# MrOlm/inStrain

Hardware: AMD Instinct MI355X
Metric: Gbp profiled/s (higher is better)
Workload: dtype u32

## Files before the change

### include/instrain_amd.h

```cpp
#ifndef INSTRAIN_AMD_H
#define INSTRAIN_AMD_H

#include <stdint.h>

#ifdef __cplusplus
extern "C" {
#endif

#define ISX_OK 0
#define ISX_ERR_ARG (-1)
#define ISX_ERR_HIP (-2)
#define ISX_ERR_CAPACITY (-3)
#define ISX_ERR_MM_RANGE (-4)
#define ISX_ERR_IO (-5)
#define ISX_ERR_STATE (-6)

#define ISX_ABI_VERSION 5


typedef struct isx_ctx isx_ctx;
typedef struct isx_batch isx_batch;
typedef struct isx_bam isx_bam;
struct isx_bam_params_s;
struct isx_bam_info_s;
// ... 250 lines not shown
    int32_t want_counts;
    int32_t ring_kib;
    int32_t stage_async;
    int32_t lean_output;
    int64_t max_segs;
} isx_pipe_params;

typedef struct {
    uint32_t gpos;
    float clon_rarefied;
} isx_rare;

typedef struct {
    uint32_t gpos;
    uint32_t coverage;
} isx_sat;

typedef struct {
    int64_t ticket;
    int64_t n_pos, n_obs;
    isx_sizes sizes;
    const uint16_t *coverage16;
    const float *clon;
    const isx_rare *rare;
    int64_t n_rare, n_saturated;
    const uint32_t *counts;
    const float *clon_rarefied;
    const isx_snv *snv;
    isx_batch *batch;
    float encode_ms;
    float h2d_ms, kernel_ms, d2h_ms;
    float collect_wait_ms;
    int32_t record_bytes;
    int32_t encode_passes;
    int64_t h2d_bytes, d2h_bytes;
    const isx_ld *ld;
    const uint8_t *coverage8;
    const isx_rare *clon_sparse;
    int64_t n_clon;
    const isx_sat *saturated;
    const uint8_t *coverage4;
    const uint16_t *cov_rows;
    const uint32_t *cov_row_window;
    int64_t n_cov_rows;
    int32_t cov_window, pad_cov;
    const void *lev_mask;
    const void *lev_cov;
    const uint32_t *lev_win_off;
    const isx_rare *lev_clon, *lev_rare;
    const isx_sat *lev_sat;
    int64_t n_lev, n_lev_clon, n_lev_rare, n_lev_sat;
    int32_t lev_mask_bytes, lev_cov_bytes, lev_window, n_lev_windows, lev_min_cov, pad_lev;
    uint64_t rows_checksum;
} isx_pipe_result;

int isx_levels_expand(const isx_pipe_result *r, int32_t host_threads, uint32_t *gpos, uint32_t *mm_cov, float *clon, float *clon_rarefied);

int isx_pipe_create(isx_ctx *ctx, const isx_params *params, const isx_pipe_params *pp, isx_pipe **out);
void isx_pipe_destroy(isx_pipe *p);
int isx_pipe_submit(isx_pipe *p, int64_t n_pos, const uint8_t *ref, int32_t n_splits, const int64_t *split_bounds,
                    int64_t n_obs, const isx_obs *obs, const uint32_t *pair, int64_t *ticket);
int isx_pipe_submit_bam(isx_pipe *p, isx_bam *bam, const struct isx_bam_params_s *bp, const int32_t *refs, int32_t n_refs,
                        const uint8_t *ref, int32_t n_splits, const int64_t *split_bounds, struct isx_bam_info_s *info,
                        int64_t *ticket);
int isx_pipe_collect(isx_pipe *p, int64_t ticket, isx_pipe_result *out);
int isx_pipe_release(isx_pipe *p, int64_t ticket);
int isx_pipe_fetch_entries(isx_pipe *p, int64_t ticket, isx_entry *out);
int isx_pipe_fetch_entries_shrunk(isx_pipe *p, int64_t ticket, uint32_t *gpos, uint32_t *mm_cov, float *clon, float *clon_rarefied);


#define ISX_SEG_BASES 150
#define ISX_SEG_WORDS 15
#define ISX_SEG_SKIP_WORD 0x24924924u
#define ISX_DREC_WORDS 8
#define ISX_DREC_EXC 6
#define ISX_DREC_EXC_FULL 3
#define ISX_DREC_DUAL 0x80000000u
#define ISX_DREC_NO_EXC 0x3FFFFFFFu

typedef struct {
    int64_t n_seg;
    const uint32_t *gpos;
    const uint8_t *len;
    const uint8_t *mm;
    const uint32_t *pair;
    const uint32_t *bases;
} isx_segs;

int isx_batch_create_reads(isx_ctx *ctx, const isx_params *params, int64_t n_pos, const uint8_t *ref, int32_t n_splits,
                           const int64_t *split_bounds, const isx_segs *segs, isx_batch **out);
int isx_pipe_submit_reads(isx_pipe *p, int64_t n_pos, const uint8_t *ref, int32_t n_splits, const int64_t *split_bounds,
                          const isx_segs *segs, int64_t *ticket);

typedef struct isx_wire isx_wire;
int isx_pipe_stage_reads(isx_pipe *p, int64_t n_pos, const uint8_t *ref, int32_t n_splits, const int64_t *split_bounds,
                         const isx_segs *segs, isx_wire **out);
int isx_pipe_submit_wire(isx_pipe *p, const isx_wire *wire, int64_t *ticket);
int64_t isx_wire_bytes(const isx_wire *wire);
void isx_wire_free(isx_wire *wire);
int isx_wire_keep_reference(isx_pipe *p, isx_wire *wire);

#define ISX_PLANE_WORDS 8
typedef struct {
    int64_t n_seg;
    const uint32_t *gpos;
    const uint8_t *len;
    const uint32_t *pair;
    const uint64_t *planes;
    const uint8_t *mm;
} isx_read_planes;

typedef struct {
    const uint8_t *plane2;
    const uint8_t *nplane;
    uint64_t key;
} isx_ref_planes;

int isx_pack_ref_planes(const uint8_t *ref, int64_t n_pos, int32_t host_threads, uint8_t *plane2, uint8_t *nplane, int32_t *has_n);
int isx_planes_from_segs(const isx_segs *segs, int32_t host_threads, uint64_t *planes);
int isx_pack_read_planes(int64_t n_reads, const int64_t *ref_start, const int64_t *clip_lo, const int64_t *clip_hi,
                         const uint32_t *cigar, const int64_t *cigar_off, const char *seq, const uint8_t *qual, const int64_t *seq_off,
                         const uint32_t *pair, int32_t min_base_quality, int64_t cap_seg, uint32_t *seg_gpos,
                         uint8_t *seg_len, uint32_t *seg_pair, uint64_t *seg_planes, int64_t *n_seg);
int isx_pipe_submit_planes(isx_pipe *p, int64_t n_pos, const isx_ref_planes *ref, int32_t n_splits, const int64_t *split_bounds,
                           const isx_read_planes *reads, int64_t *ticket);
int isx_pipe_stage_planes(isx_pipe *p, int64_t n_pos, const isx_ref_planes *ref, int32_t n_splits, const int64_t *split_bounds,
                          const isx_read_planes *reads, isx_wire **out);
int isx_pipe_set_reference_budget(isx_pipe *p, int64_t mib);
int isx_host_register(const void *ptr, int64_t bytes);
int isx_host_unregister(const void *ptr);
int isx_encode_planes(const isx_read_planes *reads, const isx_ref_planes *ref, int64_t n_pos, int32_t host_threads, int32_t slack_groups,
                      int64_t cap_rec, int64_t ring_records, uint32_t *rec, uint32_t *gbase, int64_t *n_rec, int64_t *need_slack);
int isx_encode_planes_mm(const isx_read_planes *reads, const isx_ref_planes *ref, int64_t n_pos, int32_t n_mm_bins, int32_t host_threads, int32_t slack_groups,
                         int64_t cap_rec, int64_t ring_records, uint32_t *rec, uint32_t *gbase, int64_t *n_rec, int64_t *need_slack);

int isx_count_read_segs(int64_t n_reads, const uint32_t *cigar, const int64_t *cigar_off, const int64_t *ref_start,
                        const int64_t *clip_lo, const int64_t *clip_hi, int64_t *n_seg);
int isx_pack_reads(int64_t n_reads, const int64_t *ref_start, const int64_t *clip_lo, const int64_t *clip_hi,
                   const uint32_t *cigar, const int64_t *cigar_off, const char *seq, const uint8_t *qual, const int64_t *seq_off,
                   const uint8_t *mm, const uint32_t *pair, int32_t min_base_quality, int64_t cap_seg, uint32_t *seg_gpos,
                   uint8_t *seg_len, uint8_t *seg_mm, uint32_t *seg_pair, uint32_t *seg_bases, int64_t *n_seg);

int isx_encode_segs(const isx_segs *segs, int64_t n_pos, int32_t n_mm_bins, int32_t host_threads, int64_t cap_rec, uint32_t *rec,
                    uint32_t *gbase, uint32_t *pair_out, int64_t *n_rec);
int64_t isx_seg_records_needed(const uint32_t *gpos, int64_t n_seg, int32_t host_threads);
int isx_encode_segs_ring(const isx_segs *segs, int64_t n_pos, int32_t n_mm_bins, int32_t host_threads, int64_t cap_rec, int64_t ring_records,
                         uint32_t *rec, uint32_t *gbase, uint32_t *pair_out, int64_t *n_rec);

int isx_encode_delta(const isx_segs *segs, const uint8_t *ref, int64_t n_pos, int32_t n_mm_bins, int32_t host_threads, int32_t slack_groups,
                     int64_t cap_rec, int64_t ring_records, uint32_t *rec, uint32_t *gbase, uint32_t *pair_out, int64_t *n_rec, int64_t *need_slack);
int64_t isx_delta_records_needed(const uint32_t *gpos, int64_t n_seg, int32_t host_threads, int32_t slack_groups);

int isx_encode_obs(const isx_obs *obs, const uint32_t *pair, int64_t n_obs, int64_t n_pos, int32_t record_bytes,
                   int32_t host_threads, double slack, int64_t cap_rec, void *rec, uint32_t *gbase, uint32_t *pair_out,
                   int64_t *n_rec, int32_t *passes);
int isx_encode_obs_ring(const isx_obs *obs, const uint32_t *pair, int64_t n_obs, int64_t n_pos, int32_t record_bytes,
                        int32_t host_threads, double slack, int64_t cap_rec, int64_t ring_records, void *rec,
                        uint32_t *gbase, uint32_t *pair_out, int64_t *n_rec, int32_t *passes);

typedef struct {
    int64_t in_off;
    int32_t in_len;
    int32_t out_len;
    int64_t out_off;
} isx_bgzf_block;
int isx_bgzf_index(const uint8_t *image, int64_t n_bytes, int64_t cap_blocks, isx_bgzf_block *blocks, int64_t *n_blocks, int64_t *out_bytes);
int isx_bgzf_inflate_device(isx_ctx *ctx, const uint8_t *image, int64_t n_bytes, const isx_bgzf_block *blocks, int64_t n_blocks,
                            uint8_t *out, int64_t out_bytes, float *kernel_ms);
int isx_bgzf_inflate_host(const uint8_t *image, int64_t n_bytes, const isx_bgzf_block *blocks, int64_t n_blocks, uint8_t *out, int64_t out_bytes);
int isx_bgzf_inflate_fast(const uint8_t *image, int64_t n_bytes, const isx_bgzf_block *blocks, int64_t n_blocks, uint8_t *out, int64_t out_bytes);

typedef struct isx_bam_params_s {
    double min_read_ani;
    int32_t min_mapq;
    double max_insert_relative;
    int32_t min_insert;
    int32_t min_base_quality;
    int32_t skip_mm;
    int32_t window_length;
    int32_t pairing_filter;
} isx_bam_params;

typedef struct isx_bam_info_s {
    int32_t n_refs;
    int32_t n_splits;
    int64_t n_reads;
    int64_t n_pos;
// ... 48 lines not shown
```

### instrain_amd/_lib.py

```python
import ctypes as C
import os

import numpy as np

_HERE = os.path.dirname(os.path.abspath(__file__))
LIB_PATH = os.path.join(_HERE, "libinstrain_amd.so")
if os.environ.get("ISX_LIB"):
    LIB_PATH = os.path.abspath(os.environ["ISX_LIB"])

BGZF_BLOCK_DT = np.dtype([("in_off", np.int64), ("in_len", np.int32), ("out_len", np.int32), ("out_off", np.int64)])
OBS_DT = np.dtype([("gpos", "<u4"), ("mm", "<u2"), ("base", "u1"), ("flags", "u1")])
ENTRY_DT = np.dtype([("gpos", "<u4"), ("mm", "<u2"), ("flags", "<u2"), ("cnt", "<u4", (4,)), ("clon", "<f4"),
                     ("clon_rarefied", "<f4")])
SNV_DT = np.dtype([("gpos", "<u4"), ("mm", "<u2"), ("con_base", "u1"), ("var_base", "u1"),
                   ("allele_count", "u1"), ("cls", "u1"), ("cryptic", "u1"), ("ref_base", "u1"),
                   ("cnt", "<u4", (4,))])
LD_DT = np.dtype([("gpos_a", "<u4"), ("gpos_b", "<u4"), ("mm", "<u2"), ("allele_A", "u1"), ("allele_a", "u1"),
                  ("allele_B", "u1"), ("allele_b", "u1"), ("pad", "<u2"), ("total", "<u4"), ("countAB", "<u4"),
                  ("countAb", "<u4"), ("countaB", "<u4"), ("countab", "<u4"), ("pad2", "<u4"),
                  ("r2", "<f8"), ("d_prime", "<f8"), ("r2_normalized", "<f8"), ("d_prime_normalized", "<f8")])
AO_DT = np.dtype([("pair", "<u4"), ("gpos", "<u4"), ("order", "<u4"), ("mm", "<u2"), ("base", "u1"), ("pad", "u1")])
assert AO_DT.itemsize == 16
assert OBS_DT.itemsize == 8 and ENTRY_DT.itemsize == 32 and SNV_DT.itemsize == 28 and LD_DT.itemsize == 72

# ... 19 lines not shown


class Segs(C.Structure):
    _fields_ = [("n_seg", C.c_int64), ("gpos", C.c_void_p), ("len", C.c_void_p), ("mm", C.c_void_p), ("pair", C.c_void_p),
                ("bases", C.c_void_p)]


PLANE_WORDS = 8
LAYOUT_MM_ENTRIES = 16
LAYOUT_MM_DELTA_RECORDS = 32
ABI_VERSION = 5


class ReadPlanes(C.Structure):
    _fields_ = [("n_seg", C.c_int64), ("gpos", C.c_void_p), ("len", C.c_void_p), ("pair", C.c_void_p), ("planes", C.c_void_p), ("mm", C.c_void_p)]


class RefPlanes(C.Structure):
    _fields_ = [("plane2", C.c_void_p), ("nplane", C.c_void_p), ("key", C.c_uint64)]


RARE_DT = np.dtype([("gpos", "<u4"), ("clon_rarefied", "<f4")])
CLON_DT = np.dtype([("gpos", "<u4"), ("clon", "<f4")])
SAT_DT = np.dtype([("gpos", "<u4"), ("coverage", "<u4")])


class Sizes(C.Structure):
    _fields_ = [(n, C.c_int64) for n in ("n_entries", "n_snv", "n_sites", "n_allele_obs", "n_increments",
                                         "n_edges", "n_ld")]


class Timings(C.Structure):
    _fields_ = [(n, C.c_float) for n in ("pileup_ms", "sites_ms", "allele_ms", "group_ms", "incr_ms", "ld_ms",
                                         "total_ms")] + \
               [(n, C.c_int32) for n in ("pileup_blocks", "pileup_threads", "pileup_lds_bytes", "pileup_window")] + \
               [("mfma_ms", C.c_float), ("dense_tiles", C.c_int32), ("dense_macs", C.c_int64), ("dense_bytes", C.c_int64),
                ("record_bytes", C.c_int32), ("pad", C.c_int32)]


class PipeResult(C.Structure):
    _fields_ = [("ticket", C.c_int64), ("n_pos", C.c_int64), ("n_obs", C.c_int64), ("sizes", Sizes),
                ("coverage16", C.c_void_p), ("clon", C.c_void_p), ("rare", C.c_void_p), ("n_rare", C.c_int64),
                ("n_saturated", C.c_int64), ("counts", C.c_void_p), ("clon_rarefied", C.c_void_p), ("snv", C.c_void_p),
                ("batch", C.c_void_p),
                ("encode_ms", C.c_float), ("h2d_ms", C.c_float), ("kernel_ms", C.c_float), ("d2h_ms", C.c_float),
                ("collect_wait_ms", C.c_float), ("record_bytes", C.c_int32), ("encode_passes", C.c_int32),
                ("h2d_bytes", C.c_int64), ("d2h_bytes", C.c_int64), ("ld", C.c_void_p),
                ("coverage8", C.c_void_p), ("clon_sparse", C.c_void_p), ("n_clon", C.c_int64), ("saturated", C.c_void_p),
                ("coverage4", C.c_void_p), ("cov_rows", C.c_void_p), ("cov_row_window", C.c_void_p), ("n_cov_rows", C.c_int64),
                ("cov_window", C.c_int32), ("pad_cov", C.c_int32),
                ("lev_mask", C.c_void_p), ("lev_cov", C.c_void_p), ("lev_win_off", C.c_void_p), ("lev_clon", C.c_void_p), ("lev_rare", C.c_void_p),
                ("lev_sat", C.c_void_p), ("n_lev", C.c_int64), ("n_lev_clon", C.c_int64), ("n_lev_rare", C.c_int64), ("n_lev_sat", C.c_int64),
                ("lev_mask_bytes", C.c_int32), ("lev_cov_bytes", C.c_int32), ("lev_window", C.c_int32), ("n_lev_windows", C.c_int32),
                ("lev_min_cov", C.c_int32), ("pad_lev", C.c_int32), ("rows_checksum", C.c_uint64)]


class BamParams(C.Structure):
    _fields_ = [("min_read_ani", C.c_double), ("min_mapq", C.c_int32), ("max_insert_relative", C.c_double),
                ("min_insert", C.c_int32), ("min_base_quality", C.c_int32), ("skip_mm", C.c_int32),
                ("window_length", C.c_int32), ("pairing_filter", C.c_int32)]


PAIRING_FILTERS = {"paired_only": 0, "non_discordant": 1, "all_reads": 2}


class BamInfo(C.Structure):
    _fields_ = [("n_refs", C.c_int32), ("n_splits", C.c_int32), ("n_reads", C.c_int64), ("n_pos", C.c_int64),
                ("n_obs", C.c_int64), ("n_pairs", C.c_int64), ("unfiltered_pairs", C.c_int64),
                ("filtered_pairs", C.c_int64), ("filtered_bases", C.c_int64), ("median_insert", C.c_double),
                ("max_mm", C.c_int32), ("pad", C.c_int32), ("unfiltered_reads", C.c_int64),
                ("unfiltered_singletons", C.c_int64), ("filtered_singletons", C.c_int64), ("n_segs", C.c_int64)]


SCAFFOLD_LEVEL_DT = np.dtype([("nonzero", "<i8"), ("sum_cov", "<u8"), ("sumsq_cov", "<u8"), ("median_cov", "<f8"),
                              ("counted", "<i8"), ("sum_clon", "<f8"), ("median_clon", "<f8"),
                              ("counted_rarefied", "<i8"), ("sum_clon_rarefied", "<f8"),
                              ("median_clon_rarefied", "<f8"), ("mm", "<i4"), ("present", "<i4")])
assert SCAFFOLD_LEVEL_DT.itemsize == 88
GENOME_LEVEL_DT = np.dtype([("n", "<i8"), ("sum_cov", "<u8"), ("sumsq_cov", "<u8"), ("median_cov", "<f8"), ("mm", "<i4"), ("pad", "<i4")])
assert GENOME_LEVEL_DT.itemsize == 40
GENOME_COV_DT = np.dtype([("n", "<i8"), ("sum_cov", "<u8"), ("sumsq_cov", "<u8"), ("max_cov", "<u4"), ("pad", "<u4")])
SNV_LEVEL_DT = np.dtype([(n, "<u4") for n in ("divergent", "sns", "snv", "con", "pop")])
LD_LEVEL_DT = np.dtype([("n", "<i8"), ("n_r2", "<i8"), ("n_dprime", "<i8"), ("sum_distance", "<i8"), ("sum_r2", "<f8"), ("sum_dprime", "<f8")])
assert GENOME_COV_DT.itemsize == 32 and SNV_LEVEL_DT.itemsize == 20 and LD_LEVEL_DT.itemsize == 48


COMPARE_LEVEL_DT = np.dtype([("both", "<i8"), ("either", "<i8"), ("mm", "<i4"), ("present_a", "<i4"),
                             ("present_b", "<i4"), ("pad", "<i4"), ("consensus_snps", "<i8"), ("population_snps", "<i8")])
assert COMPARE_LEVEL_DT.itemsize == 48
COMPARE_SNP_DT = np.dtype([("gpos", "<u4"), ("mm", "<u2"), ("consensus_snp", "u1"), ("population_snp", "u1"),
                           ("has_a", "u1"), ("has_b", "u1"), ("con_a", "u1"), ("ref_a", "u1"), ("var_a", "u1"),
                           ("con_b", "u1"), ("ref_b", "u1"), ("var_b", "u1"), ("cnt_a", "<u4", (4,)), ("cnt_b", "<u4", (4,))])
assert COMPARE_SNP_DT.itemsize == 48


GENE_DT = np.dtype([("start", "<i8"), ("end", "<i8"), ("seq_off", "<i8"), ("strand", "<i4"), ("pad", "<i4")])
GENE_COV_DT = np.dtype([("sum_cov", "<u8"), ("nonzero", "<u4"), ("counted", "<u4"), ("sum_clon", "<f8")])
GENE_SNV_COUNT_DT = np.dtype([(n, "<u4") for n in ("divergent", "sns", "sns_n", "sns_s", "snv", "snv_n", "snv_s")])
GENE_MUTATION_DT = np.dtype([("gene", "<i4"), ("k", "<i4"), ("type", "u1"), ("aa_old", "u1"), ("aa_new", "u1"), ("n_genes", "u1"),
                             ("pad", "<u4")])
assert GENE_DT.itemsize == 32 and GENE_COV_DT.itemsize == 24 and GENE_SNV_COUNT_DT.itemsize == 28 and GENE_MUTATION_DT.itemsize == 16
GENE_LEVEL_PRESENT, GENE_COV_ANY, GENE_CLON_ANY = 1, 2, 4


ERR_CAPACITY = -3


class IsxError(RuntimeError):
    def __init__(self, code, msg):
        super().__init__("libinstrain_amd error %d: %s" % (code, msg))
        self.code = code


SYMBOLS = ["isx_last_error", "isx_abi_version", "isx_ctx_create", "isx_ctx_destroy", "isx_ctx_reserve_cus", "isx_set_null_model",
           "isx_batch_create", "isx_batch_create_reads", "isx_batch_destroy", "isx_batch_run", "isx_batch_launch", "isx_batch_wait", "isx_batch_sizes", "isx_batch_timings",
           "isx_batch_fetch_entries", "isx_batch_fetch_dense", "isx_batch_fetch_snv", "isx_batch_fetch_ld", "isx_batch_fetch_allele_obs",
           "isx_batch_summarize", "isx_batch_summarize_genomes", "isx_batch_genome_coverage", "isx_snv_level_counts", "isx_ld_level_sums", "isx_compare_coverage", "isx_compare_scaffolds", "isx_compare_fetch_snps",
           "isx_genes_create", "isx_genes_destroy", "isx_genes_sites", "isx_batch_profile_genes", "isx_genes_profile_snvs",
           "isx_pipe_create", "isx_pipe_destroy", "isx_pipe_submit", "isx_pipe_submit_reads", "isx_pipe_stage_reads", "isx_pipe_submit_wire", "isx_wire_bytes", "isx_wire_free", "isx_wire_keep_reference", "isx_pipe_submit_bam", "isx_encode_segs", "isx_encode_segs_ring", "isx_seg_records_needed", "isx_encode_delta", "isx_delta_records_needed", "isx_count_read_segs", "isx_pack_reads", "isx_pipe_collect", "isx_pipe_release", "isx_pipe_fetch_entries", "isx_pipe_fetch_entries_shrunk", "isx_levels_expand", "isx_encode_obs", "isx_encode_obs_ring",
           "isx_pack_ref_planes", "isx_planes_from_segs", "isx_pack_read_planes", "isx_pipe_submit_planes", "isx_pipe_stage_planes", "isx_encode_planes", "isx_encode_planes_mm", "isx_pipe_set_reference_budget", "isx_host_register", "isx_host_unregister",
           "isx_bgzf_index", "isx_bgzf_inflate_device", "isx_bgzf_inflate_host", "isx_bgzf_inflate_fast",
           "isx_bam_open", "isx_bam_close", "isx_bam_close_wait", "isx_bam_set_threads", "isx_bam_ref", "isx_bam_set_priority_reads", "isx_bam_scan", "isx_bam_scan_part",
           "isx_bam_insert_sizes", "isx_bam_set_wanted_refs", "isx_bam_pair_keys", "isx_bam_set_cross_names", "isx_bam_filter_insert_sizes", "isx_bam_filter", "isx_bam_set_r2m", "isx_bam_r2m", "isx_bam_drop_names", "isx_bam_batch_pair_names", "isx_bam_set_mm_cap", "isx_bam_mm_levels", "isx_bam_set_mm_levels", "isx_bam_ref_counts",
           "isx_bam_expand_refs", "isx_bam_segment_refs", "isx_bam_copy_segs", "isx_bam_copy_read_planes", "isx_bam_expand_region", "isx_bam_expand", "isx_bam_copy", "isx_bam_view"]

_lib = None


def load():
    global _lib
    if _lib is not None:
        return _lib
    if not os.path.exists(LIB_PATH):
        raise IsxError(-2, "%s not built: run `python -c 'import __graft_entry__ as g; g.build()'` "
                           "(hipcc --offload-arch=gfx950)" % LIB_PATH)
    lib = C.CDLL(LIB_PATH)
    vp, i32, i64 = C.c_void_p, C.c_int32, C.c_int64
    lib.isx_last_error.restype = C.c_char_p
    lib.isx_abi_version.restype = C.c_int
    if lib.isx_abi_version() != ABI_VERSION:
        raise IsxError(-6, "%s has ABI version %d, this package binds version %d: rebuild it (python -c 'import __graft_entry__ as g; g.build()')"
                       % (LIB_PATH, lib.isx_abi_version(), ABI_VERSION))
    lib.isx_ctx_create.argtypes = [C.c_int, C.POINTER(vp)]
    lib.isx_ctx_destroy.argtypes = [vp]
    lib.isx_ctx_reserve_cus.argtypes = [vp, C.c_int]
    lib.isx_bgzf_index.argtypes = [vp, i64, i64, vp, C.POINTER(i64), C.POINTER(i64)]
    lib.isx_bgzf_inflate_device.argtypes = [vp, vp, i64, vp, i64, vp, i64, C.POINTER(C.c_float)]
    lib.isx_bgzf_inflate_host.argtypes = [vp, i64, vp, i64, vp, i64]
    lib.isx_bgzf_inflate_fast.argtypes = [vp, i64, vp, i64, vp, i64]
    lib.isx_ctx_destroy.restype = None
    lib.isx_set_null_model.argtypes = [vp, vp, i64, i32]
    lib.isx_batch_create.argtypes = [vp, C.POINTER(Params), i64, vp, i32, vp, i64, vp, vp, C.POINTER(vp)]
    lib.isx_batch_create_reads.argtypes = [vp, C.POINTER(Params), i64, vp, i32, vp, C.POINTER(Segs), C.POINTER(vp)]
    lib.isx_pipe_submit_reads.argtypes = [vp, i64, vp, i32, vp, C.POINTER(Segs), C.POINTER(i64)]
    lib.isx_pipe_stage_reads.argtypes = [vp, i64, vp, i32, vp, C.POINTER(Segs), C.POINTER(vp)]
    lib.isx_pipe_submit_wire.argtypes = [vp, vp, C.POINTER(i64)]
    lib.isx_wire_bytes.argtypes = [vp]
    lib.isx_wire_bytes.restype = i64
    lib.isx_wire_free.argtypes = [vp]
    lib.isx_wire_keep_reference.argtypes = [vp, vp]
    lib.isx_wire_free.restype = None
    lib.isx_encode_segs.argtypes = [C.POINTER(Segs), i64, i32, i32, i64, vp, vp, vp, C.POINTER(i64)]
    lib.isx_encode_segs_ring.argtypes = [C.POINTER(Segs), i64, i32, i32, i64, i64, vp, vp, vp, C.POINTER(i64)]
    lib.isx_encode_delta.argtypes = [C.POINTER(Segs), vp, i64, i32, i32, i32, i64, i64, vp, vp, vp, C.POINTER(i64), C.POINTER(i64)]
    lib.isx_delta_records_needed.argtypes = [vp, i64, i32, i32]
    lib.isx_delta_records_needed.restype = i64
    lib.isx_seg_records_needed.argtypes = [vp, i64, i32]
    lib.isx_seg_records_needed.restype = i64
    lib.isx_count_read_segs.argtypes = [i64, vp, vp, vp, vp, vp, C.POINTER(i64)]
    lib.isx_pack_reads.argtypes = [i64, vp, vp, vp, vp, vp, vp, vp, vp, vp, vp, i32, i64, vp, vp, vp, vp, vp, C.POINTER(i64)]
    lib.isx_batch_destroy.argtypes = [vp]
    lib.isx_batch_destroy.restype = None
    lib.isx_batch_run.argtypes = [vp]
# ... 18 lines not shown
    lib.isx_genes_sites.argtypes = [vp, vp, C.POINTER(C.c_float)]
    lib.isx_batch_profile_genes.argtypes = [vp, vp, i32, vp, vp, vp, vp, vp, C.POINTER(C.c_float)]
    lib.isx_genes_profile_snvs.argtypes = [vp, i32, vp, vp, vp, i64, vp, i32, vp, vp, C.POINTER(C.c_float)]
    lib.isx_pipe_create.argtypes = [vp, C.POINTER(Params), C.POINTER(PipeParams), C.POINTER(vp)]
    lib.isx_pipe_destroy.argtypes = [vp]
    lib.isx_pipe_destroy.restype = None
    lib.isx_pipe_submit.argtypes = [vp, i64, vp, i32, vp, i64, vp, vp, C.POINTER(i64)]
    lib.isx_pipe_submit_bam.argtypes = [vp, vp, C.POINTER(BamParams), vp, i32, vp, i32, vp, C.POINTER(BamInfo), C.POINTER(i64)]
    lib.isx_pipe_collect.argtypes = [vp, i64, C.POINTER(PipeResult)]
    lib.isx_pipe_release.argtypes = [vp, i64]
    lib.isx_pipe_fetch_entries.argtypes = [vp, i64, vp]
    lib.isx_pipe_fetch_entries_shrunk.argtypes = [vp, i64, vp, vp, vp, vp]
    lib.isx_levels_expand.argtypes = [C.POINTER(PipeResult), i32, vp, vp, vp, vp]
    lib.isx_encode_obs.argtypes = [vp, vp, i64, i64, i32, i32, C.c_double, i64, vp, vp, vp, C.POINTER(i64), C.POINTER(i32)]
    lib.isx_encode_obs_ring.argtypes = [vp, vp, i64, i64, i32, i32, C.c_double, i64, i64, vp, vp, vp, C.POINTER(i64), C.POINTER(i32)]
    lib.isx_bam_open.argtypes = [C.c_char_p, C.POINTER(vp)]
    lib.isx_bam_close.argtypes = [vp]
    lib.isx_bam_close.restype = None
    lib.isx_bam_close_wait.argtypes = [vp]
    lib.isx_bam_close_wait.restype = None
    lib.isx_bam_expand.argtypes = [vp, C.POINTER(BamParams), C.POINTER(BamInfo)]
    lib.isx_bam_set_threads.argtypes = [vp, i32]
    lib.isx_bam_set_priority_reads.argtypes = [vp, i64, C.c_char_p, vp]
    lib.isx_bam_scan.argtypes = [vp, C.POINTER(BamInfo)]
    lib.isx_bam_scan_part.argtypes = [vp, i32, i32, C.POINTER(BamInfo)]
    lib.isx_bam_set_wanted_refs.argtypes = [vp, vp, i32]
    lib.isx_bam_insert_sizes.argtypes = [vp, vp, i64, C.POINTER(i64)]
    lib.isx_bam_filter_insert_sizes.argtypes = [vp, vp, i64, C.POINTER(i64)]
    lib.isx_bam_pair_keys.argtypes = [vp, vp, vp, vp, vp, i64, C.POINTER(i64)]
    lib.isx_bam_set_cross_names.argtypes = [vp, i64, vp, vp, vp]
    lib.isx_bam_filter.argtypes = [vp, C.POINTER(BamParams), C.c_double, C.POINTER(BamInfo)]
    lib.isx_bam_set_r2m.argtypes = [vp, i32, i64, C.c_char_p, vp, vp]
    lib.isx_bam_drop_names.argtypes = [vp]
    lib.isx_bam_r2m.argtypes = [vp, i32, C.POINTER(i64), C.POINTER(i64), vp, vp, vp]
    lib.isx_bam_batch_pair_names.argtypes = [vp, C.POINTER(i64), C.POINTER(i64), vp, vp]
    lib.isx_bam_set_mm_cap.argtypes = [vp, i32]
    lib.isx_bam_mm_levels.argtypes = [vp, vp, i32, vp]
    lib.isx_bam_set_mm_levels.argtypes = [vp, vp, i32]
    lib.isx_bam_ref_counts.argtypes = [vp, vp, vp]
    lib.isx_bam_expand_region.argtypes = [vp, C.POINTER(BamParams), i32, i64, i64, C.POINTER(BamInfo)]
    lib.isx_bam_expand_refs.argtypes = [vp, C.POINTER(BamParams), vp, i32, C.POINTER(BamInfo)]
    lib.isx_bam_segment_refs.argtypes = [vp, C.POINTER(BamParams), vp, i32, C.POINTER(BamInfo), C.POINTER(i64)]
    lib.isx_bam_copy_segs.argtypes = [vp, vp, vp, vp, vp, vp, vp, vp]
    lib.isx_bam_copy_read_planes.argtypes = [vp, vp]
    lib.isx_pack_ref_planes.argtypes = [vp, i64, i32, vp, vp, C.POINTER(i32)]
    lib.isx_planes_from_segs.argtypes = [C.POINTER(Segs), i32, vp]
    lib.isx_pack_read_planes.argtypes = [i64, vp, vp, vp, vp, vp, vp, vp, vp, vp, i32, i64, vp, vp, vp, vp, C.POINTER(i64)]
    lib.isx_pipe_submit_planes.argtypes = [vp, i64, C.POINTER(RefPlanes), i32, vp, C.POINTER(ReadPlanes), C.POINTER(i64)]
    lib.isx_pipe_set_reference_budget.argtypes = [vp, i64]
    lib.isx_host_register.argtypes = [vp, i64]
    lib.isx_host_unregister.argtypes = [vp]
    lib.isx_pipe_stage_planes.argtypes = [vp, i64, C.POINTER(RefPlanes), i32, vp, C.POINTER(ReadPlanes), C.POINTER(vp)]
    lib.isx_encode_planes.argtypes = [C.POINTER(ReadPlanes), C.POINTER(RefPlanes), i64, i32, i32, i64, i64, vp, vp, C.POINTER(i64), C.POINTER(i64)]
    lib.isx_encode_planes_mm.argtypes = [C.POINTER(ReadPlanes), C.POINTER(RefPlanes), i64, i32, i32, i32, i64, i64, vp, vp, C.POINTER(i64), C.POINTER(i64)]
    lib.isx_bam_ref.argtypes = [vp, i32, C.POINTER(C.c_char_p), C.POINTER(i64), C.POINTER(i64)]
    lib.isx_bam_copy.argtypes = [vp, vp, vp, vp, vp]
    lib.isx_bam_view.argtypes = [vp, C.POINTER(vp), C.POINTER(vp)]
    _lib = lib
    return lib


def check(rc):
    if rc != 0:
        raise IsxError(rc, load().isx_last_error().decode(errors="replace"))
```

### instrain_amd/csrc/isx_internal.h

```cpp
#pragma once
#include <hip/hip_runtime.h>
#include <stdint.h>
#include <string>

#include "../../include/instrain_amd.h"

#define ISX_PAD32 0x0700FFFFu
#define ISX_GROUP16 512
#define ISX_GROUP 256
#define ISX_CHUNK 1024
#define ISX_DENSE_PAD 8
#define ISX_SEG_GROUP 16
#define ISX_SEG_PAD 32
#define ISX_SEG_LM 16
#define ISX_PK16_MAX_W 3264
#define ISX_PAD 2048
#define ISX_SENTINEL 0xFFFFFFFFu
#define ISX_TAIL_BYTES 65536
#define ISX_TAIL_GROUPS 256

void isx_set_error(const std::string &msg);

hipError_t isx_dev_malloc(void **p, size_t bytes);
void isx_dev_free(void *p);
// ... 140 lines not shown
    int32_t stripe;
    int32_t pad, lm;
    double min_freq;
    uint4 *counts;
    float *clon;
    float *clon_r;
    uint16_t *cov16;
    uint8_t *cov8;
    uint8_t *cov4;
    uint16_t *cov_rows;
    uint32_t *cov_row_win;
    uint32_t cap_cov_rows;
    uint2 *sat;
    uint32_t cap_sat, sat_thr;
    uint2 *clon_list;
    uint32_t cap_clon;
    uint2 *rare;
    uint32_t cap_rare;
    int32_t min_cov_r;
    uint32_t seed_lo, seed_hi;
    isx_entry *entries;
    uint32_t slab;
    uint32_t cap_ovf;
    uint64_t ovf0;
    uint32_t *win_nent;
    uint32_t *win_site_base, *win_site_cnt;
    isx_slev *slev;
    uint32_t cap_slev;
    isx_snv *snv;
    uint32_t cap_snv;
    isx_site *sites;
    uint32_t cap_sites;
    isx_ao *ao;
    uint32_t cap_ao;
    int32_t enable_linkage;
    uint32_t *win_rec;
    uint32_t *cursors;
    uint32_t *flags;
    uint32_t base[CUR_N];
    uint32_t *host_state;
    const uint32_t *pub_cursors;
    uint32_t *pub_host_state;
    uint32_t pub_epoch;
    void *lev_mask;
    void *lev_cov;
    uint32_t *lev_win_off;
    uint32_t cap_lev;
    int32_t lev_mask_bytes, lev_cov_bytes;
};

void launch_pileup(const PileupArgs &a, int block, size_t lds, int grid, int packed, hipStream_t s, hipEvent_t ev_start,
                   hipEvent_t ev_stop);
void launch_publish_state(const PileupArgs &a, uint32_t epoch, hipStream_t s);
void launch_win_order(const uint32_t *win_rec, uint32_t *win_out, int n_win, int W, const isx_snv *snv_raw, isx_snv *snv, const isx_site *sites_raw,
                      isx_site *sites, const uint2 *clon_raw, uint2 *clon, const uint2 *rare_raw, uint2 *rare, uint32_t *scan_state, uint32_t epoch, hipStream_t s);
void launch_extract_gpos(const uint2 *rec, const uint32_t *rec32, const uint32_t *gbase, uint32_t *gpos, uint16_t *gpos16,
                         const uint32_t *base16, uint32_t base16_records, uint64_t n_rec, hipStream_t s);
size_t pileup_lds_bytes(int W, int M, int qcap, int rqcap, int linkage, int packed, int block, int segs, int *stage_off, int *dlt_off = nullptr);

struct LinkageBuffers;
```

### instrain_amd/csrc/isx_pipe.hip

```cpp
#include <atomic>
#include <algorithm>
#include <chrono>
#include <cmath>
#include <condition_variable>
#include <cstring>
#include <deque>
#include <mutex>
#include <memory>
#include <string>
#include <thread>
#include <vector>

#include "bam_front.h"
#include "isx_batch.h"
#include "obs_encode.h"
#include "seg_encode.h"
#include "isx_summary.h"
#include <unordered_map>

namespace {

constexpr size_t ALIGN = 256;
inline size_t up(size_t v, size_t a = ALIGN) { return (v + a - 1) / a * a; }

// ... 10 lines not shown
    return ISX_OK;
}

void host_block_free(void *p, bool pinned)
{
    if (!p) return;
    if (pinned) isx_pin_free(p); else free(p);
}

static const bool pipe_timing = getenv("ISX_PIPE_TIMING") != nullptr;
#define H2D(p, s) ((s).h2d ? (s).h2d : (p)->s_h2d)
struct Slot {
    isx_batch *b = nullptr;
    hipStream_t h2d = nullptr;
    uint8_t *h_in = nullptr, *d_in = nullptr;
    size_t in_bytes = 0;
    size_t off_bounds = 0, off_win = 0, off_ref = 0, off_gbase = 0, off_ridx = 0, off_rec = 0;
    size_t off_pairs = 0;
    isxenc::PairRun *h_runs = nullptr;
    bool runs_pinned = true;
    uint2 *d_runs = nullptr;
    size_t cap_runs = 0;
    hipEvent_t ev_ring[2] = {nullptr, nullptr};
    bool ring_busy[2] = {false, false};
    uint8_t *h_out = nullptr;
    uint8_t *h_small = nullptr;
    size_t small_bytes = 0;
    bool out_pinned = true;
    size_t out_bytes = 0, o_counts = 0, o_clon = 0, o_clonr = 0, o_snv = 0, o_cov16 = 0, o_rare = 0;
    bool rare_dense = false;
    bool cov8 = false, clon_sparse = false;
    bool cov4 = false;
    size_t cov_rows_off = 0;
    int cov_window = 0;
    std::vector<uint32_t> cov_row_win;
    std::vector<isx_sat> sat_rows;
    bool sat_complete = true;
    void *sort_temp = nullptr;
    size_t sort_temp_bytes = 0;
    std::vector<float> clonr_big;
    std::vector<isx_rare> rare_big;
    std::vector<uint32_t> cmin, cmax, dir_pmax, dir_smin;
    std::vector<uint8_t> cany;
    std::vector<uint2> win;
    size_t o_lmask = 0, o_lwin = 0, o_lcov = 0, o_lclon = 0, o_lrare = 0;
    size_t lcov_room = 0, lclon_room = 0, lrare_room = 0;
    std::vector<uint8_t> lcov_big;
    std::vector<isx_rare> lclon_big, lrare_big;
    std::vector<isx_snv> snv_big;
    std::vector<isx_ld> ld_rows;
    uint64_t rows_checksum = 0;
    hipEvent_t ev_h2d0 = nullptr, ev_h2d1 = nullptr, ev_pass = nullptr, ev_d2h0 = nullptr, ev_d2h1 = nullptr;
    hipEvent_t ev_h2da = nullptr, ev_h2db = nullptr;
    bool h2d_split = false;
    int64_t ticket = -1;
    BamBatch *dead_batch = nullptr;
    bool ref_has_n = false;
    int state = 0;
    int rc = 0;
    std::string err;
    float finish_wait_ms = 0.f;
    float encode_ms = 0.f;
    int encode_passes = 0;
    int64_t h2d_bytes = 0, d2h_bytes = 0;
    uint16_t *d_gpos16 = nullptr;
};

static uint64_t bytes_checksum(const void *p, size_t bytes, uint64_t seed)
{
    const uint8_t *b = static_cast<const uint8_t *>(p);
    uint64_t a[4] = {seed ^ 0x9E3779B97F4A7C15ull, seed + 0xC2B2AE3D27D4EB4Full, seed ^ 0x165667B19E3779F9ull, seed + 0x27D4EB2F165667C5ull};
    const size_t n8 = bytes / 8;
    size_t i = 0;
    for (; i + 4 <= n8; i += 4) {
        uint64_t w[4];
        memcpy(w, b + 8 * i, 32);
        for (int k = 0; k < 4; k++) a[k] = a[k] * 0x100000001B3ull + w[k];
    }
    uint64_t h = (uint64_t)bytes;
    for (; i < n8; i++) { uint64_t w; memcpy(&w, b + 8 * i, 8); h = h * 0x100000001B3ull + w; }
    for (size_t j = n8 * 8; j < bytes; j++) h = h * 0x100000001B3ull + b[j];
    for (int k = 0; k < 4; k++) { h ^= a[k]; h *= 0xFF51AFD7ED558CCDull; h ^= h >> 33; }
    return h;
}

static inline size_t ref2_bytes(int64_t n_pos) { return (((size_t)n_pos + 3) / 4 + 15) & ~(size_t)15; }
static inline size_t refn_bytes(int64_t n_pos) { return (((size_t)n_pos + 7) / 8 + 15) & ~(size_t)15; }

static bool copy_ref_planes(isxenc::HostPool &pool, const isx_ref_planes *rp, int64_t n_pos, uint8_t *plane2, uint8_t *nplane)
{
    const size_t b2 = ((size_t)n_pos + 3) / 4, bn = ((size_t)n_pos + 7) / 8;
    const size_t piece = (size_t)1 << 20;
    const int t2 = (int)((b2 + piece - 1) / piece), tn = rp->nplane ? (int)((bn + piece - 1) / piece) : 0;
    std::atomic<int> any{0};
    pool.run(t2 + tn, [&](int t) {
        if (t < t2) { const size_t a = (size_t)t * piece; memcpy(plane2 + a, rp->plane2 + a, std::min(piece, b2 - a)); return; }
        const size_t a = (size_t)(t - t2) * piece, n = std::min(piece, bn - a);
        const uint8_t *src = rp->nplane + a;
        uint8_t acc = 0;
        for (size_t i = 0; i < n; i++) acc |= src[i];
        memcpy(nplane + a, src, n);
        if (acc) any.store(1, std::memory_order_relaxed);
    });
    return any.load() != 0;
}

static bool plane_any(isxenc::HostPool &pool, const uint8_t *pl, size_t bytes)
{
    const size_t piece = (size_t)1 << 20;
    const int nt = (int)((bytes + piece - 1) / piece);
    std::atomic<int> any{0};
    pool.run(nt, [&](int t) {
        const size_t a = (size_t)t * piece, n = std::min(piece, bytes - a);
        uint64_t acc = 0;
        size_t i = 0;
        for (; i + 8 <= n; i += 8) { uint64_t v; memcpy(&v, pl + a + i, 8); acc |= v; }
        for (; i < n; i++) acc |= pl[a + i];
        if (acc) any.store(1, std::memory_order_relaxed);
// ... 10 lines not shown
    for (size_t k = 0; k < n_s; k++) {
        uint64_t w;
        memcpy(&w, plane2 + 8 * (k * step), 8);
        h = (h ^ w) * 0x100000001B3ull;
        h ^= h >> 29;
    }
    return h;
}

int cgroup_cpus()
{
    if (FILE *f = fopen("/sys/fs/cgroup/cpu.max", "r")) {
        char q[64] = {0};
        long period = 0;
        const int n = fscanf(f, "%63s %ld", q, &period);
        fclose(f);
        if (n == 2 && period > 0 && strcmp(q, "max") != 0) return (int)std::max<long>(1, atol(q) / period);
    }
    return 0;
}

int gpu_numa_node(int device)
{
    char bus[64] = {0};
    if (hipDeviceGetPCIBusId(bus, sizeof bus, device) != hipSuccess) return -1;
    std::string id(bus);
    std::transform(id.begin(), id.end(), id.begin(), [](unsigned char ch) { return (char)std::tolower(ch); });
    int node = -1;
    if (FILE *f = fopen(("/sys/bus/pci/devices/" + id + "/numa_node").c_str(), "r")) {
        if (fscanf(f, "%d", &node) != 1) node = -1;
        fclose(f);
    }
    return node;
}

}

struct isx_pipe {
    isx_ctx *ctx = nullptr;
    isx_params prm{};
    isx_pipe_params pp{};
    std::unique_ptr<isxenc::HostPool> pool;
    std::vector<Slot> slots;
    hipStream_t s_h2d = nullptr, s_d2h = nullptr;
    hipStream_t s_h2d2 = nullptr;
    hipStream_t s_fin = nullptr;
    hipStream_t s_fin2 = nullptr;
    int64_t next_ticket = 0;
    int64_t cap_rec = 0;
    int64_t ring_half = 0;
    int rb = 2;
    bool segs = false;
    bool drec = false;
    int64_t dslack = 1;
    uint32_t G = ISX_GROUP16;
    size_t snv_prefix = 0;
    size_t rare_prefix = 0, cap_rare = 0;
    double slack = 0.0;
    std::thread finisher;
    std::thread finisher2;
    std::vector<std::thread> more_finishers;
    std::vector<hipStream_t> extra_fin;
    std::mutex bounce_mu;
    std::mutex mu;
    std::condition_variable cv_work, cv_done;
    std::deque<int64_t> work;
    bool stop = false;
    std::mutex launch_mu;
    uint8_t *bounce[2] = {nullptr, nullptr};
    hipEvent_t bounce_ev[2] = {nullptr, nullptr};
    size_t bounce_bytes = 0;
    std::unique_ptr<isxenc::HostPool> fin_pool;
    struct StageJob {
        int64_t ticket, n_pos;
        const uint8_t *ref;
        std::vector<int64_t> bounds;
        isx_segs segs;
        bool planes = false;
        isx_read_planes reads{};
        isx_ref_planes rp{};
    };
    struct RefEntry { uint8_t *d = nullptr; size_t bytes = 0; int64_t n_pos = 0; bool has_n = false; hipEvent_t ready = nullptr; uint64_t sum = 0; };
    std::unordered_map<uint64_t, RefEntry> ref_cache;
    size_t ref_cache_bytes = 0;
    std::atomic<size_t> ref_cache_budget{(size_t)4096 << 20};
    std::thread stager;
    std::deque<StageJob> stage_q;
    std::condition_variable cv_stage;
    int64_t next_promise = 0;
    bool stage_stop = false;
};

static int bounce_d2h(isx_pipe *p, void *hdst, const void *dsrc, size_t bytes, hipStream_t st)
{
    if (!bytes) return ISX_OK;
    std::lock_guard<std::mutex> bounce_lk(p->bounce_mu);
    const size_t piece = p->bounce_bytes;
    const size_t n_pieces = (bytes + piece - 1) / piece;
    auto issue = [&](size_t k) -> hipError_t {
        const size_t off = k * piece, len = std::min(piece, bytes - off);
        hipError_t e = isx_copy_to_host(p->bounce[k & 1], static_cast<const uint8_t *>(dsrc) + off, len, st);
        return e == hipSuccess ? hipEventRecord(p->bounce_ev[k & 1], st) : e;
    };
    HIP_TRY(issue(0));
    for (size_t k = 0; k < n_pieces; k++) {
        if (k + 1 < n_pieces) HIP_TRY(issue(k + 1));
        HIP_TRY(isx_wait_event(p->bounce_ev[k & 1]));
        const size_t off = k * piece, len = std::min(piece, bytes - off);
        const size_t sub = (size_t)1 << 20;
        const uint8_t *src = p->bounce[k & 1];
        uint8_t *dst = static_cast<uint8_t *>(hdst) + off;
        p->fin_pool->run((int)((len + sub - 1) / sub), [&](int t) {
            const size_t a = (size_t)t * sub;
            memcpy(dst + a, src + a, std::min(sub, len - a));
        });
    }
    return ISX_OK;
}

static void pipe_free(isx_pipe *p)
{
    if (!p) return;
    if (p->stager.joinable()) {
        { std::lock_guard<std::mutex> lk(p->mu); p->stage_stop = true; }
        p->cv_stage.notify_all();
        p->stager.join();
    }
    if (p->finisher.joinable()) {
        { std::lock_guard<std::mutex> lk(p->mu); p->stop = true; }
        p->cv_work.notify_all();
        p->finisher.join();
        if (p->finisher2.joinable()) p->finisher2.join();
        for (auto &t : p->more_finishers) if (t.joinable()) t.join();
    }
    (void)hipSetDevice(p->ctx->device);
    if (p->s_h2d) (void)isx_wait_stream(p->s_h2d);
    if (p->s_h2d2) (void)isx_wait_stream(p->s_h2d2);
    if (p->s_d2h) (void)isx_wait_stream(p->s_d2h);
    if (p->s_fin) (void)isx_wait_stream(p->s_fin);
    if (p->s_fin2) (void)isx_wait_stream(p->s_fin2);
    for (hipStream_t st : p->extra_fin) (void)isx_wait_stream(st);
    for (int i = 0; i < 2; i++) if (p->ctx->pstream[i]) (void)isx_wait_stream(p->ctx->pstream[i]);
    const double t_f0 = now_ms();
    double t_batch = 0, t_dev = 0, t_pin = 0;
    for (Slot &s : p->slots) {
        double t_x = now_ms();
        if (s.b) {
            isx_batch *b = s.b;
            b->d_seg = nullptr; b->d_drec = nullptr;
            b->d_rec = nullptr; b->d_rec32 = nullptr; b->d_rec16 = nullptr; b->d_gbase = nullptr; b->d_pair = nullptr;
            b->d_pair_runs = nullptr; b->d_run_index = nullptr;
            b->d_gpos = nullptr; b->d_gpos16 = nullptr; b->d_cbase = nullptr; b->d_ref = nullptr; b->d_win = nullptr;
            b->d_bounds = nullptr;
            isx_batch_destroy(b);
        }
        t_batch += now_ms() - t_x; t_x = now_ms();
        if (s.sort_temp) isx_dev_free(s.sort_temp);
        if (s.d_gpos16) isx_dev_free(s.d_gpos16);
        if (s.d_in) isx_dev_free(s.d_in);
        if (s.d_runs) isx_dev_free(s.d_runs);
        t_dev += now_ms() - t_x; t_x = now_ms();
        if (s.h_in) isx_pin_free(s.h_in);
        host_block_free(s.h_runs, s.runs_pinned);
        for (hipEvent_t e : s.ev_ring) if (e) (void)hipEventDestroy(e);
        host_block_free(s.h_out, s.out_pinned);
        if (s.h_small) isx_pin_free(s.h_small);
        t_pin += now_ms() - t_x;
        for (hipEvent_t e : {s.ev_h2d0, s.ev_h2d1, s.ev_pass, s.ev_d2h0, s.ev_d2h1, s.ev_h2da, s.ev_h2db}) if (e) (void)hipEventDestroy(e);
    }
    if (pipe_timing)
        fprintf(stderr, "[isx_pipe_destroy] device tables %.1f ms, device arena %.1f ms, pinned staging %.1f ms, total %.1f ms\n", t_batch, t_dev, t_pin, now_ms() - t_f0);
    for (auto &kv : p->ref_cache) { if (kv.second.d) isx_dev_free(kv.second.d); if (kv.second.ready) (void)hipEventDestroy(kv.second.ready); }
    for (int i = 0; i < 2; i++) {
        if (p->bounce[i]) isx_pin_free(p->bounce[i]);
        if (p->bounce_ev[i]) (void)hipEventDestroy(p->bounce_ev[i]);
    }
    if (p->s_h2d) (void)hipStreamDestroy(p->s_h2d);
    if (p->s_h2d2) (void)hipStreamDestroy(p->s_h2d2);
    if (p->s_d2h) (void)hipStreamDestroy(p->s_d2h);
    if (p->s_fin) (void)hipStreamDestroy(p->s_fin);
    if (p->s_fin2) (void)hipStreamDestroy(p->s_fin2);
    for (hipStream_t st : p->extra_fin) (void)hipStreamDestroy(st);
    delete p;
}

static int slot_batch_create(isx_pipe *p, Slot &s, int index)
{
    isx_ctx *c = p->ctx;
    const isx_params *prm = &p->prm;
    const double t_s0 = now_ms();
    isx_batch *b = new isx_batch();
    s.b = b;
    b->ctx = c; b->prm = *prm; b->M = prm->n_mm_bins;
    b->ps = getenv("ISX_ONE_PASS_QUEUE") ? 0 : (index & 1);
    b->cap_pos = p->pp.max_pos; b->cap_obs = p->pp.max_obs; b->arena = true; b->ref_packed = 2;
    b->n_pos = p->pp.max_pos; b->n_obs = p->pp.max_obs;
    b->segs = p->segs; b->drec = p->drec;
    b->lean = p->pp.lean_output != 0 && !p->pp.want_counts;
    b->lev_sparse = b->M > 1 && b->M <= 32 && p->segs && !p->pp.want_counts && !(prm->layout & ISX_LAYOUT_MM_ENTRIES);
    b->spin_us = (p->pp.host_threads > 0 && p->pp.host_threads < 8) ? 200 : 2000;
    const bool dense = b->M == 1;
    batch_pick_block(b);
    const int64_t cap_pos = p->pp.max_pos;
    for (auto &e : b->ev) HIP_TRY(hipEventCreate(&e));
    for (auto &e : b->ev_sum) HIP_TRY(hipEventCreate(&e));
    HIP_TRY(isx_dev_malloc(reinterpret_cast<void **>(&b->d_cursors), (CUR_N + 4) * sizeof(uint32_t)));
    b->d_flags = b->d_cursors + CUR_N;
    HIP_TRY(hipHostMalloc(&b->h_state, (CUR_N + 8) * sizeof(uint32_t), hipHostMallocMapped | hipHostMallocCoherent));
    memset(b->h_state, 0, (CUR_N + 8) * sizeof(uint32_t));
    HIP_TRY(hipHostGetDevicePointer(reinterpret_cast<void **>(&b->d_host_state), b->h_state, 0));
    HIP_TRY(hipMemset(b->d_cursors, 0, (CUR_N + 4) * sizeof(uint32_t)));
    {
        std::vector<uint16_t> thr = build_thresholds(c->h_lut, c->fallback, prm->min_freq);
        HIP_TRY(isx_dev_malloc(reinterpret_cast<void **>(&b->d_thr), thr.size() * sizeof(uint16_t)));
        HIP_TRY(hipMemcpy(b->d_thr, thr.data(), thr.size() * sizeof(uint16_t), hipMemcpyHostToDevice));
    }
    const uint64_t npm = (uint64_t)cap_pos * b->M;
    const uint64_t cap_obs = (uint64_t)std::max<int64_t>(p->pp.max_obs, 1);
    if (dense) {
        if (p->pp.want_counts) HIP_TRY(isx_dev_malloc(reinterpret_cast<void **>(&b->d_counts), (size_t)cap_pos * sizeof(uint4)));
        else {
// ... 25 lines not shown
            b->cap_entries = b->cap_lev;
            HIP_TRY(isx_dev_malloc(reinterpret_cast<void **>(&b->d_entries), b->cap_entries * sizeof(isx_entry)));
        }
        b->cap_clon = (size_t)cap_pos / 4 + 65536;
        HIP_TRY(isx_dev_malloc(reinterpret_cast<void **>(&b->d_clon_list), b->cap_clon * sizeof(uint2)));
        b->cap_sat = (size_t)cap_pos / 16 + 65536;
        HIP_TRY(isx_dev_malloc(reinterpret_cast<void **>(&b->d_sat), b->cap_sat * sizeof(uint2)));
        if (prm->rarefied_coverage > 0) {
            b->cap_rare = p->cap_rare;
            HIP_TRY(isx_dev_malloc(reinterpret_cast<void **>(&b->d_rare), b->cap_rare * sizeof(uint2)));
        }
    } else {
        b->slab_region = (size_t)(cap_pos + 2 * b->block) * (size_t)std::min(b->M, 4);
        const size_t ovf = b->M <= 4 ? 16 : (size_t)std::max<uint64_t>(1u << 20, std::min<uint64_t>(cap_obs, npm) / 4);
        if (b->slab_region + ovf >= 0xFFFFFFFFull) { isx_set_error("mm path: more than 2^32 entry slots in one batch"); return ISX_ERR_ARG; }
        b->cap_entries = b->slab_region + ovf;
        HIP_TRY(isx_dev_malloc(reinterpret_cast<void **>(&b->d_entries), b->cap_entries * sizeof(isx_entry)));
        HIP_TRY(isx_dev_malloc(reinterpret_cast<void **>(&b->d_win_nent), ((size_t)cap_pos / 64 + 2) * sizeof(uint32_t)));
    }
    b->cap_snv = (size_t)std::min<uint64_t>(npm, std::max<uint64_t>((uint64_t)cap_pos / 2, 1u << 20));
    b->cap_sites = (size_t)std::min<uint64_t>((uint64_t)cap_pos, std::max<uint64_t>((uint64_t)cap_pos / 4, 1u << 20));
    b->cap_ao = (size_t)std::max<uint64_t>(1, std::min<uint64_t>(cap_obs, std::max<uint64_t>(cap_obs / 4, 1u << 20)));
    HIP_TRY(isx_dev_malloc(reinterpret_cast<void **>(&b->d_snv), b->cap_snv * sizeof(isx_snv)));
    HIP_TRY(isx_dev_malloc(reinterpret_cast<void **>(&b->d_sites), b->cap_sites * sizeof(isx_site)));
    if (prm->enable_linkage) HIP_TRY(isx_dev_malloc(reinterpret_cast<void **>(&b->d_ao), b->cap_ao * sizeof(isx_ao)));
    if (!dense) {
        b->cap_slev = b->cap_sites * (size_t)std::min(b->M, 8);
        HIP_TRY(isx_dev_malloc(reinterpret_cast<void **>(&b->d_slev), b->cap_slev * sizeof(isx_slev)));
    }
    size_t o = 0;
    s.off_bounds = o; o = up(o + (size_t)(p->pp.max_splits + 1) * sizeof(int64_t));
    s.off_win = o; o = up(o + ((size_t)cap_pos / 64 + 2) * sizeof(uint2));
    s.off_ref = o; o = up(o + ref2_bytes(cap_pos) + refn_bytes(cap_pos));
    s.off_gbase = o; o = up(o + ((size_t)(p->cap_rec / p->G) + ISX_TAIL_GROUPS) * sizeof(uint32_t));
    s.off_ridx = o; if (prm->enable_linkage && !p->segs) o = up(o + ((size_t)p->cap_rec / ISX_CHUNK + 2) * sizeof(uint32_t));
    s.off_pairs = o; if (prm->enable_linkage && p->segs && !p->drec) o = up(o + (size_t)p->cap_rec * sizeof(uint32_t));
    s.off_rec = o;
    s.in_bytes = up(o + (size_t)p->cap_rec * p->rb + ISX_TAIL_BYTES);
    const size_t host_bytes = p->ring_half ? up(o + 2 * (size_t)p->ring_half * p->rb) : s.in_bytes;
    const double t_a0 = now_ms();
    HIP_TRY(isx_pin_malloc(reinterpret_cast<void **>(&s.h_in), host_bytes));
    const double t_a1 = now_ms();
    HIP_TRY(isx_dev_malloc(reinterpret_cast<void **>(&s.d_in), s.in_bytes));
    if (pipe_timing)
        fprintf(stderr, "[isx_pipe_create] slot %d: device tables %.1f ms, pinned input %.1f MB %.1f ms, device arena %.1f MB %.1f ms\n", index,
                t_a0 - t_s0, host_bytes / 1e6, t_a1 - t_a0, s.in_bytes / 1e6, now_ms() - t_a1);
    if (prm->enable_linkage && !p->segs) {
        s.cap_runs = (size_t)p->cap_rec / 64 + 4096;
        s.runs_pinned = p->pp.depth > 1;
        { const int hrc = host_block_alloc(reinterpret_cast<void **>(&s.h_runs), s.cap_runs * sizeof(isxenc::PairRun), s.runs_pinned); if (hrc != ISX_OK) return hrc; }
        HIP_TRY(isx_dev_malloc(reinterpret_cast<void **>(&s.d_runs), s.cap_runs * sizeof(uint2)));
    }
    if (p->ring_half) for (hipEvent_t &e : s.ev_ring) HIP_TRY(hipEventCreateWithFlags(&e, hipEventDisableTiming));
    if (prm->enable_linkage && p->rb == 4) HIP_TRY(isx_dev_malloc(reinterpret_cast<void **>(&s.d_gpos16), (size_t)p->cap_rec * sizeof(uint16_t)));
    o = 0;
    s.o_snv = o; o = up(o + p->snv_prefix * sizeof(isx_snv));
    s.o_rare = o; if (dense && prm->rarefied_coverage > 0) o = up(o + p->rare_prefix * sizeof(isx_rare));
    s.small_bytes = o;
    HIP_TRY(isx_pin_malloc(reinterpret_cast<void **>(&s.h_small), std::max<size_t>(s.small_bytes, 1)));
    o = 0;
    if (dense) {
        s.o_cov16 = o; o = up(o + (size_t)cap_pos * 2);
        s.o_clon = o; o = up(o + (size_t)cap_pos * 4);
        if (p->pp.want_counts) {
            s.o_counts = o; o = up(o + (size_t)cap_pos * 16);
            s.o_clonr = o; if (prm->rarefied_coverage > 0) o = up(o + (size_t)cap_pos * 4);
        }
    }
    if (b->lev_sparse) {
        s.o_lmask = o; o = up(o + (size_t)cap_pos * b->lev_mask_bytes);
        s.o_lwin = o; o = up(o + ((size_t)cap_pos / 64 + 2) * sizeof(uint32_t));
        s.lcov_room = (size_t)cap_pos * (size_t)std::min(b->M, 4);
        s.o_lcov = o; o = up(o + s.lcov_room);
        s.lclon_room = (size_t)cap_pos;
        s.o_lclon = o; o = up(o + s.lclon_room);
        s.lrare_room = prm->rarefied_coverage > 0 ? (size_t)cap_pos / 2 : 0;
        s.o_lrare = o; o = up(o + s.lrare_room);
    }
    s.out_bytes = o;
    const double t_o0 = now_ms();
    s.out_pinned = s.out_bytes <= ((size_t)64 << 20) || p->pp.depth > 2;
    { const int hrc = host_block_alloc(reinterpret_cast<void **>(&s.h_out), s.out_bytes, s.out_pinned); if (hrc != ISX_OK) return hrc; }
    if (pipe_timing) fprintf(stderr, "[isx_pipe_create] slot %d: %s results %.1f MB %.1f ms\n", index, s.out_pinned ? "pinned" : "pageable", s.out_bytes / 1e6, now_ms() - t_o0);
    for (hipEvent_t *e : {&s.ev_h2d0, &s.ev_h2d1, &s.ev_pass, &s.ev_d2h0, &s.ev_d2h1, &s.ev_h2da, &s.ev_h2db}) HIP_TRY(hipEventCreate(e));
    const size_t n_chunks = (size_t)(p->cap_rec / (p->segs ? (int64_t)p->G : (int64_t)ISX_CHUNK)) + 2;
    s.cmin.resize(n_chunks); s.cmax.resize(n_chunks); s.cany.resize(n_chunks);
    return ISX_OK;
}

static int finish_slot(isx_pipe *p, Slot &s, hipStream_t sfin)
{
    isx_ctx *c = p->ctx;
    isx_batch *b = s.b;
    const bool dense = b->M == 1;
    const double t0 = now_ms();
    HIP_TRY(isx_wait_event(s.ev_d2h1));
    s.finish_wait_ms = (float)(now_ms() - t0);
    const double t_c0 = now_ms();
    double t_fin = 0, t_rare = 0;
    hipStream_t ps = c->pstream[b->ps];
    bool redo = false;
    for (int attempt = 0;; attempt++) {
        uint32_t cf = 0;
        int rc = finish_pass_sizes(b, &cf, sfin);
        if (rc != ISX_OK) return rc;
        const bool cov8_overflow = !cf && dense && b->sparse_out && b->cov8_out && !b->nib_pass && (size_t)b->n_sat > b->cap_sat;
        const bool nib_overflow = !cf && dense && b->nib_pass &&
                                  ((size_t)b->n_pos / 2 + 128 + (size_t)b->n_cov_rows * (size_t)b->W * 2 > (size_t)b->n_pos * 2 ||
                                   ((size_t)b->n_cov_rows + 1) * (size_t)b->W > (size_t)(b->cap_pos ? b->cap_pos : b->n_pos));
        const bool clon_overflow = !cf && dense && b->sparse_out && b->lean && !b->clon_dense &&
                                   ((size_t)b->n_clon > b->cap_clon || (size_t)b->n_clon * 2 > (size_t)b->n_pos);
        const bool rare_overflow = !cf && dense && p->prm.rarefied_coverage > 0 && !b->rare_dense &&
                                   ((size_t)b->n_rare > p->cap_rare || (size_t)b->n_rare * 8 > (size_t)b->n_pos);
        const bool lev_overflow = !cf && b->lev_sparse && ((size_t)b->n_clon > b->cap_clon || (size_t)b->n_sat > b->cap_sat ||
                                                           (p->prm.rarefied_coverage > 0 && (size_t)b->n_rare > b->cap_rare));
        if (!cf && !cov8_overflow && !clon_overflow && !nib_overflow && !rare_overflow && !lev_overflow) break;
        if (attempt == 7) { isx_set_error("output tables still too small after 8 growth steps"); return ISX_ERR_CAPACITY; }
        if (cov8_overflow) b->cov8_out = false;
        if (nib_overflow) b->nib_out = false;
        if (clon_overflow) b->clon_dense = true;
        if (rare_overflow) b->rare_dense = true;
        if (cf && (rc = batch_grow_tables(b, cf)) != ISX_OK) return rc;
        if (lev_overflow) {
            auto regrow_list = [&](uint2 **lp, size_t *cap, size_t need) -> int {
                if (need <= *cap) return ISX_OK;
                HIP_TRY(isx_wait_stream(ps));
                if (*lp) isx_dev_free(*lp);
                *lp = nullptr;
                const size_t want = need + need / 4 + 65536;
                HIP_TRY(isx_dev_malloc(reinterpret_cast<void **>(lp), want * sizeof(uint2)));
                *cap = want;
                return ISX_OK;
            };
            if ((rc = regrow_list(&b->d_clon_list, &b->cap_clon, b->n_clon)) != ISX_OK) return rc;
            if ((rc = regrow_list(&b->d_sat, &b->cap_sat, b->n_sat)) != ISX_OK) return rc;
            if (p->prm.rarefied_coverage > 0 && (rc = regrow_list(&b->d_rare, &b->cap_rare, b->n_rare)) != ISX_OK) return rc;
        }
// ... 125 lines not shown
            }
            if (!b->ordered) std::sort(rr, rr + n_rare, [](const isx_rare &x, const isx_rare &y) { return x.gpos < y.gpos; });
        }
    }
    t_rare = now_ms();
    const size_t n_snv = (size_t)b->sizes.n_snv;
    isx_snv *rows = reinterpret_cast<isx_snv *>(s.h_small + s.o_snv);
    if (n_snv > p->snv_prefix || redo) {
        if (n_snv > p->snv_prefix) { s.snv_big.resize(n_snv); rows = s.snv_big.data(); }
        { const int prc = pull(rows, b->d_snv, n_snv * sizeof(isx_snv)); if (prc != ISX_OK) return prc; }
    }
    if (!b->ordered) std::sort(rows, rows + n_snv, [](const isx_snv &x, const isx_snv &y) { return x.gpos != y.gpos ? x.gpos < y.gpos : x.mm < y.mm; });
    if (p->prm.enable_linkage) {
        s.ld_rows.resize((size_t)b->sizes.n_ld);
        if (!s.ld_rows.empty() && b->ld_host && s.ld_rows.size() <= b->n_ld_host) memcpy(s.ld_rows.data(), b->ld_host, s.ld_rows.size() * sizeof(isx_ld));
        else if (!s.ld_rows.empty()) { const int rc = pull(s.ld_rows.data(), b->L.ld.p, s.ld_rows.size() * sizeof(isx_ld)); if (rc != ISX_OK) return rc; }
    }
    s.rows_checksum = bytes_checksum(s.ld_rows.data(), p->prm.enable_linkage ? s.ld_rows.size() * sizeof(isx_ld) : 0, bytes_checksum(rows, n_snv * sizeof(isx_snv), 0));
    if (pipe_timing)
        fprintf(stderr, "[isx_pipe finisher] wait %.2f ms, finish (sizes, linkage) %.2f ms [device: sites %.2f allele %.2f group %.2f incr %.2f ld %.2f; %lld ao, %lld incr, %lld ld], clonTR list (%u) %.2f ms, snv rows (%zu) %.2f ms\n",
                s.finish_wait_ms, t_fin - t_c0, b->tim.sites_ms, b->tim.allele_ms, b->tim.group_ms, b->tim.incr_ms, b->tim.ld_ms,
                (long long)b->sizes.n_allele_obs, (long long)b->sizes.n_increments, (long long)b->sizes.n_ld, b->n_rare, t_rare - t_fin, n_snv, now_ms() - t_rare);
    return ISX_OK;
}

static void finisher_main(isx_pipe *p, hipStream_t sfin)
{
    (void)hipSetDevice(p->ctx->device);
    for (;;) {
        int64_t ticket;
        {
            std::unique_lock<std::mutex> lk(p->mu);
            p->cv_work.wait(lk, [&] { return p->stop || !p->work.empty(); });
            if (p->work.empty()) return;
            ticket = p->work.front();
            p->work.pop_front();
        }
        Slot &s = p->slots[(size_t)(ticket % (int64_t)p->slots.size())];
        const int rc = finish_slot(p, s, sfin);
        std::string err = rc == ISX_OK ? std::string() : std::string(isx_last_error());
        BamBatch *dead = nullptr;
        {
            std::lock_guard<std::mutex> lk(p->mu);
            s.rc = rc; s.err.swap(err);
            dead = s.dead_batch; s.dead_batch = nullptr;
            s.state = 2;
        }
        p->cv_done.notify_all();
        if (dead) bam_batch_retire(dead);
    }
}

static int submit_segs_common(isx_pipe *p, int64_t n_pos, const uint8_t *ref, int32_t n_splits, const int64_t *split_bounds,
                              isxenc::SegJob &J, int64_t *ticket, const isx_ref_planes *rp = nullptr);

static void stager_main(isx_pipe *p)
{
    for (;;) {
        isx_pipe::StageJob job;
        {
            std::unique_lock<std::mutex> lk(p->mu);
            p->cv_stage.wait(lk, [&] { return p->stage_stop || !p->stage_q.empty(); });
            if (p->stage_q.empty()) return;
            job = std::move(p->stage_q.front());
            p->stage_q.pop_front();
        }
        isxenc::SegJob J;
        if (job.planes) { J.in2 = job.reads; J.n_seg = job.reads.n_seg; }
        else { J.in = job.segs; J.n_seg = job.segs.n_seg; }
        int64_t got = -1;
        const int rc = submit_segs_common(p, job.n_pos, job.ref, (int32_t)job.bounds.size() - 1, job.bounds.data(), J, &got, job.planes ? &job.rp : nullptr);
        if (rc != ISX_OK) {
            Slot &s = p->slots[(size_t)(job.ticket % (int64_t)p->slots.size())];
            std::string err(isx_last_error());
            std::lock_guard<std::mutex> lk(p->mu);
            s.ticket = job.ticket; s.rc = rc; s.err.swap(err); s.state = 2;
            p->next_ticket = job.ticket + 1;
        }
        p->cv_done.notify_all();
    }
}

static void drain_stager(isx_pipe *p)
{
    if (!p->stager.joinable()) return;
    std::unique_lock<std::mutex> lk(p->mu);
    p->cv_done.wait(lk, [&] { return p->next_ticket == p->next_promise; });
}

extern "C" {

int isx_pipe_create(isx_ctx *c, const isx_params *prm, const isx_pipe_params *pp, isx_pipe **out)
{
    if (!c || !prm || !pp || !out) { isx_set_error("isx_pipe_create: bad argument"); return ISX_ERR_ARG; }
    *out = nullptr;
    if (!c->d_lut) { isx_set_error("isx_pipe_create: call isx_set_null_model first"); return ISX_ERR_STATE; }
    if (prm->n_mm_bins < 1 || prm->n_mm_bins > 128) { isx_set_error("n_mm_bins must be in [1, 128]"); return ISX_ERR_ARG; }
    if (pp->max_pos <= 0 || pp->max_obs < 0 || pp->max_splits <= 0 || pp->depth < 1 || pp->depth > 64 || pp->max_segs < 0) {
        isx_set_error("isx_pipe_create: max_pos > 0, max_obs >= 0, max_segs >= 0, max_splits > 0, 1 <= depth <= 64");
        return ISX_ERR_ARG;
    }
    if (pp->max_segs > 0 && prm->linkage_mode == 2) { isx_set_error("isx_pipe_create: the dense MFMA linkage path takes observation batches only"); return ISX_ERR_ARG; }
    if (pp->max_pos >= (int64_t)0xFFFF0000ll) { isx_set_error("flat position space must be < 2^32 - 65536"); return ISX_ERR_ARG; }
    if (prm->window && (prm->window < 64 || (prm->window & 63) || prm->window > 8192)) { isx_set_error("window must be a multiple of 64 in [64, 8192]"); return ISX_ERR_ARG; }
    if (prm->layout & ISX_LAYOUT_WIDE_RECORDS) { isx_set_error("a pipe streams 2- / 4-byte records only"); return ISX_ERR_ARG; }
    HIP_TRY(hipSetDevice(c->device));
    isx_pipe *p = new isx_pipe();
    p->ctx = c; p->prm = *prm; p->pp = *pp;
    p->segs = pp->max_segs > 0;
    p->drec = p->segs && !(prm->layout & ISX_LAYOUT_SEG64_RECORDS) && (prm->n_mm_bins == 1 || (prm->layout & ISX_LAYOUT_MM_DELTA_RECORDS));
    p->rb = p->segs ? (p->drec ? 32 : 64) : ((prm->n_mm_bins == 1 && !(prm->layout & ISX_LAYOUT_NO_SHORT_RECORDS)) ? 2 : 4);
    p->G = p->segs ? (p->drec ? ISX_DREC_GROUP : ISX_SEG_GROUP) : (p->rb == 2 ? ISX_GROUP16 : ISX_GROUP);
    const double js = pp->jump_slack > 0 ? pp->jump_slack : 0.25;
    if (p->segs) {
        if (p->pp.max_obs == 0) p->pp.max_obs = pp->max_segs * ISX_SEG_BASES;
        const uint64_t G = p->G;
        const uint64_t groups = (uint64_t)(pp->max_segs + G - 1) / G + (uint64_t)pp->max_segs / 4096 * (p->drec ? 3 : 1) + (uint64_t)pp->max_pos / 65536 +
                                (uint64_t)pp->max_splits + 64 + (uint64_t)((double)pp->max_segs / G * js * (p->drec ? 1.0 : 0.25));
        p->cap_rec = (int64_t)(groups * G);
        if ((uint64_t)p->cap_rec >= (1ull << 26)) { delete p; isx_set_error("more than 2^26 segment records in one batch (4 GiB of records)"); return ISX_ERR_ARG; }
        const size_t rec_bytes = (size_t)p->cap_rec * (size_t)p->rb;
        size_t ring = 0;
        if (pp->ring_kib > 0) ring = (size_t)pp->ring_kib << 10;
        else if (pp->ring_kib == 0 && rec_bytes > ((size_t)(pp->depth == 1 ? 96 : 256) << 20)) ring = (size_t)64 << 20;
        if (ring && ring < rec_bytes) {
            p->ring_half = (int64_t)(ring / 2 / (size_t)p->rb) / (int64_t)p->G * (int64_t)p->G;
            if (p->ring_half * p->rb < (4096 + 16 * ISX_SEG_GROUP) * 64) { delete p; isx_set_error("isx_pipe_create: ring_kib too small for a read-level pipe (at least 1024)"); return ISX_ERR_ARG; }
        }
    } else {
        const uint64_t want = (uint64_t)((double)pp->max_obs * (1.0 + js)) + 4 * ISX_PAD;
        p->cap_rec = (int64_t)((want + ISX_PAD - 1) / ISX_PAD * ISX_PAD);
        if ((uint64_t)p->cap_rec >= 0xFFFFFFFFull) { delete p; isx_set_error("more than 2^32 records in one batch"); return ISX_ERR_ARG; }
    }
    if (!p->segs) {
        const size_t rec_bytes = (size_t)p->cap_rec * p->rb;
        size_t ring = 0;
        if (pp->ring_kib > 0) ring = (size_t)pp->ring_kib << 10;
        else if (pp->ring_kib == 0 && pp->depth == 1 && rec_bytes > ((size_t)128 << 20)) ring = (size_t)64 << 20;
        else if (pp->ring_kib == 0 && rec_bytes > ((size_t)512 << 20)) ring = (size_t)256 << 20;
        if (ring && ring < rec_bytes) {
            p->ring_half = (int64_t)(ring / 2 / p->rb) / ISX_PAD * ISX_PAD;
            if (p->ring_half < 2 * ISX_PAD) { delete p; isx_set_error("isx_pipe_create: ring_kib too small (at least 32)"); return ISX_ERR_ARG; }
        }
    }
    p->snv_prefix = (size_t)std::min<int64_t>(std::max<int64_t>(pp->max_pos / 64, 1 << 16), 1 << 22);
    p->cap_rare = (size_t)std::max<int64_t>(pp->max_pos, 1 << 16);
    p->rare_prefix = (size_t)std::max<int64_t>(pp->max_pos / 16, 1 << 16);
    int nt = pp->host_threads;
    if (nt <= 0) {
        const int q = cgroup_cpus();
        nt = q > 0 ? q : (int)std::thread::hardware_concurrency();
        nt = std::max(1, std::min(nt, 32));
    }
    c->n_pipes++;
    const double t_c0 = now_ms();
    p->pool.reset(new isxenc::HostPool(nt, gpu_numa_node(c->device), pp->pin_threads != 0));
    const double t_c1 = now_ms();
    int rc = ISX_OK;
    hipError_t e;
    if ((e = isx_side_stream_create(c, &p->s_h2d)) != hipSuccess ||
        (e = isx_side_stream_create(c, &p->s_fin)) != hipSuccess ||
        (e = isx_side_stream_create(c, &p->s_fin2)) != hipSuccess ||
        (e = isx_side_stream_create(c, &p->s_d2h)) != hipSuccess) {
        isx_set_error(std::string("isx_pipe_create: ") + hipGetErrorString(e));
        pipe_free(p);
        return ISX_ERR_HIP;
    }
    p->slots.resize((size_t)pp->depth);
    {
        const char *e2 = getenv("ISX_PIPE_H2D_STREAMS");
        if (e2 && atoi(e2) >= 2 && pp->depth >= 2 && isx_side_stream_create(c, &p->s_h2d2) != hipSuccess) { p->s_h2d2 = nullptr; (void)hipGetLastError(); }
    }
    for (int i = 0; i < pp->depth && rc == ISX_OK; i++) {
        rc = slot_batch_create(p, p->slots[(size_t)i], i);
        if ((i & 1) && p->s_h2d2) p->slots[(size_t)i].h2d = p->s_h2d2;
    }
    if (rc != ISX_OK) { pipe_free(p); return rc; }
    if (!p->slots[0].out_pinned) {
        p->bounce_bytes = (size_t)16 << 20;
        for (int i = 0; i < 2 && rc == ISX_OK; i++) {
            if (isx_pin_malloc(reinterpret_cast<void **>(&p->bounce[i]), p->bounce_bytes) != hipSuccess ||
                hipEventCreateWithFlags(&p->bounce_ev[i], hipEventDisableTiming) != hipSuccess) rc = ISX_ERR_HIP;
        }
        if (rc != ISX_OK) { isx_set_error("isx_pipe_create: bounce buffers"); pipe_free(p); return rc; }
        p->fin_pool.reset(new isxenc::HostPool(std::max(1, std::min(nt, 6)), -1, false));
    }
    p->finisher = std::thread(finisher_main, p, p->s_fin);
    if (pp->depth >= 2) p->finisher2 = std::thread(finisher_main, p, p->s_fin2);
    {
        int want = pp->depth >= 4 ? 4 : 2;
        if (const char *e = getenv("ISX_PIPE_FINISHERS")) want = std::max(1, atoi(e));
        want = std::min(want, pp->depth);
        for (int i = 2; i < want; i++) {
            hipStream_t st = nullptr;
            if (isx_side_stream_create(c, &st) != hipSuccess) break;
            p->extra_fin.push_back(st);
            p->more_finishers.emplace_back(finisher_main, p, st);
        }
    }
    if (pipe_timing)
        fprintf(stderr, "[isx_pipe_create] thread pool %.1f ms, %d slot(s) %.1f ms\n", t_c1 - t_c0, pp->depth, now_ms() - t_c1);
    if (pp->stage_async && p->segs) p->stager = std::thread(stager_main, p);
    *out = p;
    return ISX_OK;
}

void isx_pipe_destroy(isx_pipe *p) { pipe_free(p); }

static int enqueue_pass_impl(isx_pipe *p, Slot &s, int64_t n_pos, int64_t *ticket);

static int enqueue_pass(isx_pipe *p, Slot &s, int64_t n_pos, int64_t *ticket)
{
    const int rc = enqueue_pass_impl(p, s, n_pos, ticket);
    if (rc != ISX_OK) {
        const std::string why(isx_last_error());
        (void)isx_wait_stream(H2D(p, s));
        (void)isx_wait_stream(p->ctx->pstream[s.b->ps]);
        (void)isx_wait_stream(p->s_d2h);
        isx_set_error(why);
    }
    return rc;
}

static int enqueue_pass_impl(isx_pipe *p, Slot &s, int64_t n_pos, int64_t *ticket)
{
    isx_ctx *c = p->ctx;
    isx_batch *b = s.b;
    const bool dense = b->M == 1, linkage = p->prm.enable_linkage != 0;
    hipStream_t ps = c->pstream[b->ps];
    int rc = ISX_OK;
    std::unique_lock<std::mutex> launch_lk(p->launch_mu);
    HIP_TRY(hipStreamWaitEvent(ps, s.ev_h2d1, 0));
    if (dense && p->prm.rarefied_coverage > 0 && b->rare_dense)
        HIP_TRY(hipMemsetD32Async(reinterpret_cast<hipDeviceptr_t>(b->d_clon_r), 0x7FC00000, (size_t)n_pos, ps));
    if (linkage && p->rb == 4)
        launch_extract_gpos(nullptr, b->d_rec32, b->d_gbase, nullptr, b->d_gpos16, b->d_gbase, ISX_GROUP, b->n_rec, ps);
    if ((rc = launch_pass(b)) != ISX_OK) return rc;
    {
        PileupArgs pa{};
        pa.cursors = b->d_cursors; pa.host_state = b->d_host_state;
        launch_publish_state(pa, b->epoch, ps);
        b->publish_enqueued = true;
        if (c->unpublished[b->ps] == b) c->unpublished[b->ps] = nullptr;
    }
    HIP_TRY(hipEventRecord(s.ev_pass, ps));

    HIP_TRY(hipStreamWaitEvent(p->s_d2h, s.ev_pass, 0));
    HIP_TRY(hipEventRecord(s.ev_d2h0, p->s_d2h));
    const size_t snv_rows = std::min(p->snv_prefix, b->cap_snv);
    HIP_TRY(isx_copy_rows_to_host(s.h_small + s.o_snv, b->d_snv, b->d_cursors + CUR_SNV, b->base[CUR_SNV], (uint32_t)sizeof(isx_snv), snv_rows, p->s_d2h));
    s.d2h_bytes = 0;
    if (dense) {
        if (p->prm.rarefied_coverage > 0) {
            const size_t n = std::min(p->rare_prefix, std::min(p->cap_rare, (size_t)n_pos));
// ... 182 lines not shown
static int stage_reference(isx_pipe *p, Slot &s, int64_t n_pos, const uint8_t *ref, const isx_ref_planes *rp, isxenc::SegJob &J, RefStage *out)
{
    const bool ring = p->ring_half > 0;
    const double t_r = now_ms();
    const size_t b2 = ((size_t)n_pos + 3) / 4, bn = ((size_t)n_pos + 7) / 8;
    hipStream_t st = H2D(p, s);

    const auto hit = rp && rp->key ? p->ref_cache.find(rp->key) : p->ref_cache.end();
    if (hit != p->ref_cache.end()) {
        const isx_pipe::RefEntry &e = hit->second;
        if (e.n_pos != n_pos || e.has_n != (rp->nplane != nullptr && e.has_n) || e.sum != ref_plane_checksum(rp->plane2, n_pos)) {
            isx_set_error("isx_pipe_submit_planes: the reference key stands for other planes (positions / non-ACGT plane / content differ)");
            return ISX_ERR_ARG;
        }
        s.ref_has_n = e.has_n;
        J.ref2 = rp->plane2; J.refn = e.has_n ? rp->nplane : nullptr;
        out->resident = e.d;
        HIP_TRY(hipStreamWaitEvent(st, e.ready, 0));
        if (!ring) HIP_TRY(hipEventRecord(s.ev_h2d0, st));
        HIP_TRY(hipEventRecord(s.ev_h2da, st));
        out->early = true;
        out->host_ms = now_ms() - t_r;
        return ISX_OK;
    }

    const bool first_trip = rp && rp->key && p->ref_cache_budget.load(std::memory_order_relaxed) > 0;
    if (rp && !first_trip && isx_host_is_registered(rp->plane2, b2) && (!rp->nplane || isx_host_is_registered(rp->nplane, bn))) {
        const bool any_n = rp->nplane && plane_any(*p->pool, rp->nplane, bn);
        s.ref_has_n = any_n;
        J.ref2 = rp->plane2; J.refn = any_n ? rp->nplane : nullptr;
        out->host_ms = now_ms() - t_r;
        if (!ring) HIP_TRY(hipEventRecord(s.ev_h2d0, st));
        HIP_TRY(hipMemcpyAsync(s.d_in + s.off_ref, rp->plane2, b2, hipMemcpyHostToDevice, st));
        if (any_n) HIP_TRY(hipMemcpyAsync(s.d_in + s.off_ref + ref2_bytes(n_pos), rp->nplane, bn, hipMemcpyHostToDevice, st));
        if (!ring) HIP_TRY(hipEventRecord(s.ev_h2da, st));
        out->early = true;
        return ISX_OK;
    }

    uint8_t *h2 = s.h_in + s.off_ref, *hn = h2 + ref2_bytes(n_pos);
    s.ref_has_n = rp ? copy_ref_planes(*p->pool, rp, n_pos, h2, hn) : isxenc::pack_ref_planes(*p->pool, ref, n_pos, h2, hn);
    J.ref2 = h2; J.refn = s.ref_has_n ? hn : nullptr;
    out->host_ms = now_ms() - t_r;
    static const bool late_dma = getenv("ISX_PIPE_LATE_DMA") != nullptr;
    if (late_dma) return ISX_OK;
    if (!ring) HIP_TRY(hipEventRecord(s.ev_h2d0, st));
    HIP_TRY(hipMemcpyAsync(s.d_in + s.off_ref, h2, ref2_bytes(n_pos) + (s.ref_has_n ? refn_bytes(n_pos) : 0), hipMemcpyHostToDevice, st));
    if (!ring) HIP_TRY(hipEventRecord(s.ev_h2da, st));
    out->early = true;
    if (rp && rp->key) ref_cache_insert(p, s, rp, n_pos);
    return ISX_OK;
}

static int submit_common(isx_pipe *p, int64_t n_pos, const uint8_t *ref, int32_t n_splits, const int64_t *split_bounds,
                         int64_t n_obs, isxenc::EncodeJob &J, int64_t *ticket)
{
    static const char who[] = "isx_pipe_submit";
    int rc;
    if ((rc = check_capacity(p, who, n_pos, n_obs, p->pp.max_obs, n_splits)) != ISX_OK) return rc;
    if ((rc = check_split_bounds(n_pos, n_splits, split_bounds)) != ISX_OK) return rc;
    Slot *slot = nullptr;
    if ((rc = slot_acquire(p, who, &slot)) != ISX_OK) return rc;
    Slot &s = *slot;
    isx_batch *b = s.b;
    const bool linkage = p->prm.enable_linkage != 0;

    const double t0 = now_ms();
    const bool ring = p->ring_half > 0;
    uint8_t *d_rec = s.d_in + s.off_rec;
    RingFeed feed;
    J.n_obs = n_obs; J.n_pos = n_pos; J.record_bytes = p->rb;
    J.rec = s.h_in + s.off_rec; J.gbase = reinterpret_cast<uint32_t *>(s.h_in + s.off_gbase);
    J.pair_out = nullptr;
    J.cmin = s.cmin.data(); J.cmax = s.cmax.data(); J.cany = s.cany.data();
    J.cap_rec = p->cap_rec;
    if ((rc = ring_feed_install(p, s, feed, J.ring_groups, J.wave_begin, J.wave_flush)) != ISX_OK) return rc;
    int erc = 0;
    for (int attempt = 0;; attempt++) {
        if (linkage) {
            J.runs_out = s.h_runs; J.cap_runs = s.cap_runs;
            J.run_index_out = reinterpret_cast<uint32_t *>(s.h_in + s.off_ridx);
        }
        J.slack = p->slack;
        feed.bytes = 0;
        erc = isxenc::encode_obs(*p->pool, J);
        if (erc != isxenc::ENC_OK || !linkage || J.n_runs <= s.cap_runs || attempt == 1) break;
        HIP_TRY(isx_wait_stream(H2D(p, s)));
        host_block_free(s.h_runs, s.runs_pinned); s.h_runs = nullptr;
        isx_dev_free(s.d_runs); s.d_runs = nullptr;
        s.cap_runs = J.n_runs + J.n_runs / 4 + 4096;
        { const int hrc = host_block_alloc(reinterpret_cast<void **>(&s.h_runs), s.cap_runs * sizeof(isxenc::PairRun), s.runs_pinned); if (hrc != ISX_OK) return hrc; }
        HIP_TRY(isx_dev_malloc(reinterpret_cast<void **>(&s.d_runs), s.cap_runs * sizeof(uint2)));
    }
    const double t_enc = now_ms();
    if (feed.err != hipSuccess) { isx_set_error(std::string("isx_pipe_submit: staging ring: ") + hipGetErrorString(feed.err)); return ISX_ERR_HIP; }
    if (erc == isxenc::ENC_CAPACITY) { isx_set_error("isx_pipe_submit: the stream jumps too often for the pipe's record capacity (raise jump_slack)"); return ISX_ERR_CAPACITY; }
    if (erc == isxenc::ENC_MM_RANGE) { isx_set_error("an observation has mm >= 256"); return ISX_ERR_MM_RANGE; }
    if (erc == isxenc::ENC_BAD_POS) { isx_set_error("observation gpos >= n_pos"); return ISX_ERR_ARG; }
    if (linkage) {
        if (J.n_runs > s.cap_runs) { isx_set_error("isx_pipe_submit: internal: pair-id run table did not fit after growing it"); return ISX_ERR_STATE; }
        b->n_runs = (uint32_t)J.n_runs;
    }
    if (J.passes > 1 && J.n_groups_in > 0)
        p->slack = std::max(p->slack, 1.25 * ((double)J.n_groups_real / (double)J.n_groups_in - 1.0) + 0.01);
    s.ref_has_n = isxenc::pack_ref_planes(*p->pool, ref, n_pos, s.h_in + s.off_ref, s.h_in + s.off_ref + ref2_bytes(n_pos));
    memcpy(s.h_in + s.off_bounds, split_bounds, (size_t)(n_splits + 1) * sizeof(int64_t));

    b->n_pos = n_pos; b->n_obs = n_obs; b->n_splits = n_splits; b->n_rec = (uint64_t)J.n_rec;
    b->n_pairs = (uint64_t)J.max_pair + 1;
    if ((rc = slot_choose_windows(p, s, ISX_CHUNK, false)) != ISX_OK) return rc;
    if ((rc = slot_shape_pass(p, s)) != ISX_OK) return rc;
    slot_bind_inputs(p, s, nullptr);
    s.encode_ms = (float)(now_ms() - t0);
    s.encode_passes = J.passes;
    if (pipe_timing)
        fprintf(stderr, "[isx_pipe_submit] records %.2f ms (%d pass), reference + bounds + windows %.2f ms; %lld obs, %lld runs\n",
                t_enc - t0, J.passes, now_ms() - t_enc, (long long)n_obs, (long long)J.n_runs);

    if (!ring) HIP_TRY(hipEventRecord(s.ev_h2d0, H2D(p, s)));
    const size_t ref_bytes = ref2_bytes(n_pos) + (s.ref_has_n ? refn_bytes(n_pos) : 0);
    const size_t head = (size_t)(n_splits + 1) * sizeof(int64_t) + s.win.size() * sizeof(uint2) + ref_bytes;
    memset(s.h_in + s.off_gbase + (size_t)(b->n_rec / p->G) * sizeof(uint32_t), 0, ISX_TAIL_GROUPS * sizeof(uint32_t));
    const size_t gb_bytes = ((size_t)(b->n_rec / p->G) + ISX_TAIL_GROUPS) * sizeof(uint32_t), rec_bytes = (size_t)b->n_rec * p->rb + ISX_TAIL_BYTES;
    HIP_TRY(hipMemcpyAsync(s.d_in + s.off_bounds, s.h_in + s.off_bounds, (size_t)(n_splits + 1) * sizeof(int64_t), hipMemcpyHostToDevice, H2D(p, s)));
    HIP_TRY(hipMemcpyAsync(s.d_in + s.off_win, s.h_in + s.off_win, s.win.size() * sizeof(uint2), hipMemcpyHostToDevice, H2D(p, s)));
    HIP_TRY(hipMemcpyAsync(s.d_in + s.off_ref, s.h_in + s.off_ref, ref_bytes, hipMemcpyHostToDevice, H2D(p, s)));
    HIP_TRY(hipMemcpyAsync(s.d_in + s.off_gbase, s.h_in + s.off_gbase, gb_bytes, hipMemcpyHostToDevice, H2D(p, s)));
    if (ring) {
        if (p->rb == 2) HIP_TRY(hipMemsetD8Async(reinterpret_cast<hipDeviceptr_t>(d_rec + (size_t)b->n_rec * 2), 0xFF, ISX_TAIL_BYTES, H2D(p, s)));
        else HIP_TRY(hipMemsetD32Async(reinterpret_cast<hipDeviceptr_t>(d_rec + (size_t)b->n_rec * 4), (int)ISX_PAD32, ISX_TAIL_BYTES / 4, H2D(p, s)));
        if (feed.bytes != (size_t)b->n_rec * p->rb) { isx_set_error("internal: the staging ring did not carry the whole stream"); return ISX_ERR_STATE; }
    } else {
        if (p->rb == 2) memset(s.h_in + s.off_rec + (size_t)b->n_rec * 2, 0xFF, ISX_TAIL_BYTES);
        else std::fill_n(reinterpret_cast<uint32_t *>(s.h_in + s.off_rec + (size_t)b->n_rec * 4), ISX_TAIL_BYTES / 4, (uint32_t)ISX_PAD32);
        HIP_TRY(hipMemcpyAsync(d_rec, s.h_in + s.off_rec, rec_bytes, hipMemcpyHostToDevice, H2D(p, s)));
    }
    s.h2d_bytes = (int64_t)(head + gb_bytes + rec_bytes);
    if (linkage) {
        const size_t rb = (size_t)b->n_runs * sizeof(isxenc::PairRun), ib = (size_t)(b->n_rec / ISX_CHUNK) * sizeof(uint32_t);
        HIP_TRY(hipMemcpyAsync(s.d_runs, s.h_runs, rb, hipMemcpyHostToDevice, H2D(p, s)));
        HIP_TRY(hipMemcpyAsync(s.d_in + s.off_ridx, s.h_in + s.off_ridx, ib, hipMemcpyHostToDevice, H2D(p, s)));
        s.h2d_bytes += (int64_t)(rb + ib);
    }
    HIP_TRY(hipEventRecord(s.ev_h2d1, H2D(p, s)));
    s.h2d_split = false;

    return enqueue_pass(p, s, n_pos, ticket);
}

static int encode_reads(isx_pipe *p, Slot &s, isxenc::SegJob &J, bool planes_in, RingFeed &feed)
{
    s.encode_passes = 1;
    if (!p->drec) return isxenc::encode_segs(*p->pool, J);
    std::vector<int64_t> exact;
    for (int attempt = 0;; attempt++) {
        J.slack_groups = p->dslack;
        J.task_groups = exact.empty() ? nullptr : exact.data();
        feed.bytes = 0;
        const int erc = planes_in ? isxenc::encode_planes(*p->pool, J) : isxenc::encode_delta(*p->pool, J);
        if (erc != isxenc::SEG_CAPACITY || J.need_slack <= p->dslack || attempt != 0) return erc;
        exact = J.task_need;
        int64_t tot = 0;
        for (int64_t v : exact) tot += v;
        const int64_t n_t = (int64_t)exact.size(), base_tot = J.n_rec / ISX_DREC_GROUP - n_t * p->dslack;
        p->dslack = std::max<int64_t>(p->dslack, 1 + (tot - base_tot + n_t - 1) / std::max<int64_t>(n_t, 1));
        s.encode_passes = 2;
    }
}

static int submit_segs_common(isx_pipe *p, int64_t n_pos, const uint8_t *ref, int32_t n_splits, const int64_t *split_bounds,
                              isxenc::SegJob &J, int64_t *ticket, const isx_ref_planes *rp)
{
    static const char who[] = "isx_pipe_submit_reads";
    const bool planes_in = J.in2.planes != nullptr || (bool)J.produce_planes || (J.n_seg == 0 && rp != nullptr);
    int rc;
    if ((rc = check_capacity(p, who, n_pos, J.n_seg, p->pp.max_segs, n_splits)) != ISX_OK) return rc;
    if ((rc = check_split_bounds(n_pos, n_splits, split_bounds)) != ISX_OK) return rc;
    Slot *slot = nullptr;
    if ((rc = slot_acquire(p, who, &slot)) != ISX_OK) return rc;
    Slot &s = *slot;
    isx_batch *b = s.b;
    const bool linkage = p->prm.enable_linkage != 0;

    const double t0 = now_ms();
    J.n_pos = n_pos; J.n_mm_bins = b->M;
    J.rec = reinterpret_cast<uint32_t *>(s.h_in + s.off_rec);
    J.gbase = reinterpret_cast<uint32_t *>(s.h_in + s.off_gbase);
    J.pair_out = linkage && !p->drec ? reinterpret_cast<uint32_t *>(s.h_in + s.off_pairs) : nullptr;
    J.cmin = s.cmin.data(); J.cmax = s.cmax.data(); J.cany = s.cany.data();
    J.cap_rec = p->cap_rec;
    const bool ring = p->ring_half > 0;
    RingFeed feed;
    if ((rc = ring_feed_install(p, s, feed, J.ring_groups, J.wave_begin, J.wave_flush)) != ISX_OK) return rc;
    RefStage rs;
    if (planes_in) {
        if (!p->drec) { isx_set_error("bit-plane reads need a pipe whose batches travel as reference-delta records (one mm bin, or ISX_LAYOUT_MM_DELTA_RECORDS)"); return ISX_ERR_STATE; }
        if ((rc = stage_reference(p, s, n_pos, ref, rp, J, &rs)) != ISX_OK) return rc;
    }
    if (p->drec) J.ref = ref;
    const int erc = encode_reads(p, s, J, planes_in, feed);
    const double t_enc = now_ms();
    if (feed.err != hipSuccess) { isx_set_error(std::string("isx_pipe_submit_reads: staging ring: ") + hipGetErrorString(feed.err)); return ISX_ERR_HIP; }
    if ((rc = seg_status_error(erc, "isx_pipe_submit_reads: the stream jumps too often for the pipe's record capacity (raise jump_slack)", ISX_ERR_CAPACITY)) != ISX_OK) return rc;
    if (J.n_bases > p->pp.max_obs) { isx_set_error("isx_pipe_submit_reads: more bases than the pipe's max_obs"); return ISX_ERR_CAPACITY; }
    bool early_rec = false;
    if (rs.early && !ring) {
        const size_t gb_bytes0 = (size_t)(J.n_rec / (int64_t)p->G) * sizeof(uint32_t), rec_bytes0 = (size_t)J.n_rec * (size_t)p->rb;
        HIP_TRY(hipEventRecord(s.ev_h2db, H2D(p, s)));
        if (s.off_pairs == s.off_rec && s.off_ridx == s.off_rec && s.off_rec - s.off_gbase < ((size_t)2 << 20)) {
            HIP_TRY(hipMemcpyAsync(s.d_in + s.off_gbase, s.h_in + s.off_gbase, (s.off_rec - s.off_gbase) + rec_bytes0, hipMemcpyHostToDevice, H2D(p, s)));
        } else {
            HIP_TRY(hipMemcpyAsync(s.d_in + s.off_gbase, s.h_in + s.off_gbase, gb_bytes0, hipMemcpyHostToDevice, H2D(p, s)));
            HIP_TRY(hipMemcpyAsync(s.d_in + s.off_rec, s.h_in + s.off_rec, rec_bytes0, hipMemcpyHostToDevice, H2D(p, s)));
        }
        early_rec = true;
    }
    if (!planes_in) s.ref_has_n = isxenc::pack_ref_planes(*p->pool, ref, n_pos, s.h_in + s.off_ref, s.h_in + s.off_ref + ref2_bytes(n_pos));
    const double t_ref = now_ms();
    memcpy(s.h_in + s.off_bounds, split_bounds, (size_t)(n_splits + 1) * sizeof(int64_t));

    b->n_pos = n_pos; b->n_obs = J.n_bases; b->n_splits = n_splits; b->n_rec = (uint64_t)J.n_rec;
    b->n_pairs = (uint64_t)J.max_pair + 1;
    if ((rc = slot_choose_windows(p, s, p->G, true)) != ISX_OK) return rc;
    if ((rc = slot_shape_pass(p, s)) != ISX_OK) return rc;
    slot_bind_inputs(p, s, rs.resident);
    s.encode_ms = (float)(now_ms() - t0);
    if (pipe_timing)
        fprintf(stderr, "[isx_pipe_submit_reads] records %.2f ms, reference %.2f ms, bounds + windows %.2f ms; %lld segments, %lld records%s\n",
                t_enc - t0 - rs.host_ms, t_ref - t_enc + rs.host_ms, now_ms() - t_ref, (long long)J.n_seg, (long long)J.n_rec, planes_in ? " (bit planes)" : "");
    const double t_q0 = now_ms();

    if (!ring && !rs.early) HIP_TRY(hipEventRecord(s.ev_h2d0, H2D(p, s)));
    const size_t ref_bytes = ref2_bytes(n_pos) + (s.ref_has_n ? refn_bytes(n_pos) : 0);
    const size_t head = (size_t)(n_splits + 1) * sizeof(int64_t) + s.win.size() * sizeof(uint2) + ref_bytes;
    const size_t gb_bytes = (size_t)(b->n_rec / p->G) * sizeof(uint32_t), rec_bytes = (size_t)b->n_rec * (size_t)p->rb;
    if (s.off_win - s.off_bounds < ((size_t)1 << 20)) {
        HIP_TRY(hipMemcpyAsync(s.d_in + s.off_bounds, s.h_in + s.off_bounds, (s.off_win - s.off_bounds) + s.win.size() * sizeof(uint2), hipMemcpyHostToDevice, H2D(p, s)));
    } else {
        HIP_TRY(hipMemcpyAsync(s.d_in + s.off_bounds, s.h_in + s.off_bounds, (size_t)(n_splits + 1) * sizeof(int64_t), hipMemcpyHostToDevice, H2D(p, s)));
        HIP_TRY(hipMemcpyAsync(s.d_in + s.off_win, s.h_in + s.off_win, s.win.size() * sizeof(uint2), hipMemcpyHostToDevice, H2D(p, s)));
    }
    if (!rs.early) HIP_TRY(hipMemcpyAsync(s.d_in + s.off_ref, s.h_in + s.off_ref, ref_bytes, hipMemcpyHostToDevice, H2D(p, s)));
    if (!early_rec) HIP_TRY(hipMemcpyAsync(s.d_in + s.off_gbase, s.h_in + s.off_gbase, gb_bytes, hipMemcpyHostToDevice, H2D(p, s)));
    if (ring) { if (feed.bytes != rec_bytes) { isx_set_error("internal: the staging ring did not carry the whole stream"); return ISX_ERR_STATE; } }
    else if (!early_rec) HIP_TRY(hipMemcpyAsync(s.d_in + s.off_rec, s.h_in + s.off_rec, rec_bytes, hipMemcpyHostToDevice, H2D(p, s)));
    s.h2d_bytes = (int64_t)(head + gb_bytes + rec_bytes) - (rs.resident ? (int64_t)ref_bytes : 0);
    if (linkage && !p->drec) {
        HIP_TRY(hipMemcpyAsync(s.d_in + s.off_pairs, s.h_in + s.off_pairs, (size_t)b->n_rec * sizeof(uint32_t), hipMemcpyHostToDevice, H2D(p, s)));
        s.h2d_bytes += (int64_t)b->n_rec * 4;
    }
    HIP_TRY(hipEventRecord(s.ev_h2d1, H2D(p, s)));
    s.h2d_split = early_rec;
    const double t_q1 = now_ms();
    rc = enqueue_pass(p, s, n_pos, ticket);
    if (pipe_timing) fprintf(stderr, "[isx_pipe_submit_reads] copy-in queue %.2f ms, pass + copy-out queue %.2f ms\n", t_q1 - t_q0, now_ms() - t_q1);
    return rc;
}

struct isx_wire {
    isx_pipe *pipe = nullptr;
    uint8_t *h = nullptr;
    size_t bytes = 0;
    size_t o_bounds = 0, o_win = 0, o_ref = 0, o_gbase = 0, o_pairs = 0, o_rec = 0;
    size_t bounds_bytes = 0, win_bytes = 0, ref_bytes = 0, gbase_bytes = 0, pairs_bytes = 0, rec_bytes = 0;
    int64_t n_pos = 0, n_bases = 0, n_rec = 0, n_seg = 0;
    int32_t n_splits = 0;
    uint64_t n_pairs = 0;
    int W = 0, packed = 0;
    bool ref_has_n = false;
    float stage_ms = 0.f;
    int encode_passes = 1;
    uint8_t *d_ref = nullptr;
    int device = 0;
};

static int stage_common(isx_pipe *p, int64_t n_pos, const uint8_t *ref, const isx_ref_planes *rp, int32_t n_splits, const int64_t *split_bounds,
                        const isx_segs *segs, const isx_read_planes *reads, isx_wire **out)
{
    isx_segs as_segs{};
    if (reads) { as_segs.n_seg = reads->n_seg; as_segs.gpos = reads->gpos; as_segs.len = reads->len; as_segs.pair = reads->pair; segs = &as_segs; }
    *out = nullptr;
    if (!p->segs) { isx_set_error("isx_pipe_stage_reads: not a read-level pipe (isx_pipe_params.max_segs == 0)"); return ISX_ERR_STATE; }
    const bool linkage = p->prm.enable_linkage != 0;
    if (linkage && segs->n_seg && !segs->pair) { isx_set_error("linkage needs the pair array"); return ISX_ERR_ARG; }
    int rc;
    if ((rc = check_capacity(p, "isx_pipe_stage_reads", n_pos, segs->n_seg, p->pp.max_segs, n_splits)) != ISX_OK) return rc;
    if ((rc = check_split_bounds(n_pos, n_splits, split_bounds)) != ISX_OK) return rc;
    HIP_TRY(hipSetDevice(p->ctx->device));
    const double t0 = now_ms();
    std::unique_ptr<isx_wire, void (*)(isx_wire *)> w(new isx_wire(), isx_wire_free);
    w->pipe = p; w->n_pos = n_pos; w->n_splits = n_splits; w->n_seg = segs->n_seg;
    const isx_batch *b0 = p->slots[0].b;
    const int M = b0->M;
    const size_t G = p->G, rb = (size_t)p->rb;
    auto up = [](size_t v) { return (v + 255) & ~(size_t)255; };
    isxenc::SegJob J;
    std::vector<uint32_t> cmin, cmax;
    std::vector<uint8_t> cany;
    std::vector<int64_t> exact;
    for (int attempt = 0;; attempt++) {
        int64_t cap = p->drec ? isxenc::delta_groups_needed(*p->pool, segs->gpos, segs->n_seg, p->dslack) * ISX_DREC_GROUP
                              : isxenc::seg_groups_needed(*p->pool, segs->gpos, segs->n_seg) * ISX_SEG_GROUP;
        if (!exact.empty()) { cap = 0; for (int64_t v : exact) cap += std::max<int64_t>(v, 1) * ISX_DREC_GROUP; }
        if (cap > p->cap_rec) { isx_set_error("isx_pipe_stage_reads: the stream needs more records than the pipe's capacity (raise jump_slack)"); return ISX_ERR_CAPACITY; }
        const size_t n_groups = (size_t)cap / G;
        w->bounds_bytes = (size_t)(n_splits + 1) * sizeof(int64_t);
        w->ref_bytes = ref2_bytes(n_pos) + refn_bytes(n_pos);
        const size_t win_cap = ((size_t)n_pos / 64 + 2) * sizeof(uint2);
// ... 77 lines not shown
    return stage_common(p, n_pos, nullptr, ref, n_splits, split_bounds, nullptr, reads, out);
}

void isx_wire_free(isx_wire *w)
{
    if (!w) return;
    if (w->h) isx_pin_free(w->h);
    if (w->d_ref) { (void)hipSetDevice(w->device); isx_dev_free(w->d_ref); }
    delete w;
}

int isx_wire_keep_reference(isx_pipe *p, isx_wire *w)
{
    if (!p || !w || w->pipe != p) { isx_set_error("isx_wire_keep_reference: bad argument"); return ISX_ERR_ARG; }
    if (w->d_ref || !w->ref_bytes) return ISX_OK;
    isx_ctx *c = p->ctx;
    HIP_TRY(hipSetDevice(c->device));
    uint8_t *d = nullptr;
    HIP_TRY(isx_dev_malloc(reinterpret_cast<void **>(&d), w->ref_bytes + 64));
    const hipError_t e = hipMemcpy(d, w->h + w->o_ref, w->ref_bytes, hipMemcpyHostToDevice);
    if (e != hipSuccess) { isx_dev_free(d); isx_set_error(std::string("isx_wire_keep_reference: ") + hipGetErrorString(e)); return ISX_ERR_HIP; }
    w->d_ref = d; w->device = c->device;
    return ISX_OK;
}

int64_t isx_wire_bytes(const isx_wire *w) { return w ? (int64_t)(w->bounds_bytes + w->win_bytes + (w->d_ref ? 0 : w->ref_bytes) + w->gbase_bytes + w->pairs_bytes + w->rec_bytes) : 0; }

int isx_pipe_submit_wire(isx_pipe *p, const isx_wire *w, int64_t *ticket)
{
    if (!p || !w || !ticket) { isx_set_error("isx_pipe_submit_wire: bad argument"); return ISX_ERR_ARG; }
    if (w->pipe != p) { isx_set_error("isx_pipe_submit_wire: the batch was staged for another pipe"); return ISX_ERR_ARG; }
    drain_stager(p);
    Slot *slot = nullptr;
    int rc = slot_acquire(p, "isx_pipe_submit_wire", &slot);
    if (rc != ISX_OK) return rc;
    Slot &s = *slot;
    isx_batch *b = s.b;
    const double t0 = now_ms();
    b->n_pos = w->n_pos; b->n_obs = w->n_bases; b->n_splits = w->n_splits; b->n_rec = (uint64_t)w->n_rec;
    b->n_pairs = w->n_pairs;
    s.ref_has_n = w->ref_has_n;
    b->packed = w->packed; b->W = w->W;
    b->n_win = (int)(w->win_bytes / sizeof(uint2));
    if ((rc = slot_shape_pass(p, s)) != ISX_OK) return rc;
    slot_bind_inputs(p, s, w->d_ref);
    HIP_TRY(hipEventRecord(s.ev_h2d0, H2D(p, s)));
    HIP_TRY(hipMemcpyAsync(s.d_in + s.off_bounds, w->h + w->o_bounds, w->bounds_bytes, hipMemcpyHostToDevice, H2D(p, s)));
    HIP_TRY(hipMemcpyAsync(s.d_in + s.off_win, w->h + w->o_win, w->win_bytes, hipMemcpyHostToDevice, H2D(p, s)));
    if (!w->d_ref) HIP_TRY(hipMemcpyAsync(s.d_in + s.off_ref, w->h + w->o_ref, w->ref_bytes, hipMemcpyHostToDevice, H2D(p, s)));
    HIP_TRY(hipMemcpyAsync(s.d_in + s.off_gbase, w->h + w->o_gbase, w->gbase_bytes, hipMemcpyHostToDevice, H2D(p, s)));
    if (w->pairs_bytes) HIP_TRY(hipMemcpyAsync(s.d_in + s.off_pairs, w->h + w->o_pairs, w->pairs_bytes, hipMemcpyHostToDevice, H2D(p, s)));
    HIP_TRY(hipMemcpyAsync(s.d_in + s.off_rec, w->h + w->o_rec, w->rec_bytes, hipMemcpyHostToDevice, H2D(p, s)));
    HIP_TRY(hipEventRecord(s.ev_h2d1, H2D(p, s)));
    s.h2d_split = false;
    s.h2d_bytes = isx_wire_bytes(w);
    s.encode_ms = (float)(now_ms() - t0);
    s.encode_passes = 0;
    return enqueue_pass(p, s, w->n_pos, ticket);
}

int isx_pipe_submit_reads(isx_pipe *p, int64_t n_pos, const uint8_t *ref, int32_t n_splits, const int64_t *split_bounds,
                          const isx_segs *segs, int64_t *ticket)
{
    if (!p || !ref || !split_bounds || !ticket || n_pos <= 0 || n_splits <= 0 || !segs || segs->n_seg < 0 ||
        (segs->n_seg && (!segs->gpos || !segs->len || !segs->bases))) {
        isx_set_error("isx_pipe_submit_reads: bad argument");
        return ISX_ERR_ARG;
    }
    if (!p->segs) { isx_set_error("isx_pipe_submit_reads: not a read-level pipe (isx_pipe_params.max_segs == 0)"); return ISX_ERR_STATE; }
    if (p->prm.enable_linkage && segs->n_seg && !segs->pair) { isx_set_error("linkage needs the pair array"); return ISX_ERR_ARG; }
    if (p->stager.joinable()) {
        isx_pipe::StageJob job;
        job.n_pos = n_pos; job.ref = ref; job.segs = *segs;
        if (!p->prm.enable_linkage) job.segs.pair = nullptr;
        job.bounds.assign(split_bounds, split_bounds + n_splits + 1);
        return queue_for_stager(p, std::move(job), "isx_pipe_submit_reads", ticket);
    }
    isxenc::SegJob J;
    J.in = *segs; J.n_seg = segs->n_seg;
    if (!p->prm.enable_linkage) J.in.pair = nullptr;
    return submit_segs_common(p, n_pos, ref, n_splits, split_bounds, J, ticket);
}

int isx_pipe_submit_planes(isx_pipe *p, int64_t n_pos, const isx_ref_planes *ref, int32_t n_splits, const int64_t *split_bounds,
                           const isx_read_planes *reads, int64_t *ticket)
{
    if (!p || !ref || !ref->plane2 || !split_bounds || !ticket || n_pos <= 0 || n_splits <= 0 || !reads || reads->n_seg < 0 ||
        (reads->n_seg && (!reads->gpos || !reads->len || !reads->planes))) {
        isx_set_error("isx_pipe_submit_planes: bad argument");
        return ISX_ERR_ARG;
    }
    if (!p->segs || !p->drec) { isx_set_error("isx_pipe_submit_planes: bit-plane reads need a read-level pipe (max_segs > 0) with one mm bin (n_mm_bins == 1) or ISX_LAYOUT_MM_DELTA_RECORDS"); return ISX_ERR_STATE; }
    if (p->prm.enable_linkage && reads->n_seg && !reads->pair) { isx_set_error("linkage needs the pair array"); return ISX_ERR_ARG; }
    if (p->stager.joinable()) {
        isx_pipe::StageJob job;
        job.n_pos = n_pos; job.ref = nullptr; job.planes = true; job.reads = *reads; job.rp = *ref;
        if (!p->prm.enable_linkage) job.reads.pair = nullptr;
        job.bounds.assign(split_bounds, split_bounds + n_splits + 1);
        return queue_for_stager(p, std::move(job), "isx_pipe_submit_planes", ticket);
    }
    isxenc::SegJob J;
    J.in2 = *reads; J.n_seg = reads->n_seg;
    if (!p->prm.enable_linkage) J.in2.pair = nullptr;
    return submit_segs_common(p, n_pos, nullptr, n_splits, split_bounds, J, ticket, ref);
}

int isx_pipe_set_reference_budget(isx_pipe *p, int64_t mib)
{
    if (!p) { isx_set_error("isx_pipe_set_reference_budget: bad argument"); return ISX_ERR_ARG; }
    p->ref_cache_budget.store(mib < 0 ? 0 : (size_t)(mib ? mib : 4096) << 20, std::memory_order_relaxed);
    return ISX_OK;
}

int isx_pipe_submit(isx_pipe *p, int64_t n_pos, const uint8_t *ref, int32_t n_splits, const int64_t *split_bounds,
                    int64_t n_obs, const isx_obs *obs, const uint32_t *pair, int64_t *ticket)
{
    if (!p || !ref || !split_bounds || !ticket || n_pos <= 0 || n_splits <= 0 || n_obs < 0 || (n_obs && !obs)) {
        isx_set_error("isx_pipe_submit: bad argument");
        return ISX_ERR_ARG;
    }
    if (p->prm.enable_linkage && n_obs && !pair) { isx_set_error("linkage needs the pair array"); return ISX_ERR_ARG; }
    if (p->segs) { isx_set_error("isx_pipe_submit: a read-level pipe takes isx_pipe_submit_reads / isx_pipe_submit_bam"); return ISX_ERR_STATE; }
    isxenc::EncodeJob J;
    J.obs = obs; J.pair = p->prm.enable_linkage ? pair : nullptr;
    static const isx_obs none{};
    if (!n_obs) J.obs = &none;
    return submit_common(p, n_pos, ref, n_splits, split_bounds, n_obs, J, ticket);
}

int isx_pipe_submit_bam(isx_pipe *p, isx_bam *bam, const struct isx_bam_params_s *bp, const int32_t *refs, int32_t n_refs,
                        const uint8_t *ref, int32_t n_splits, const int64_t *split_bounds, struct isx_bam_info_s *info, int64_t *ticket)
{
    if (!p || !bam || !bp || !refs || n_refs <= 0 || !ref || !ticket) { isx_set_error("isx_pipe_submit_bam: bad argument"); return ISX_ERR_ARG; }
    BamBatch *q = nullptr;
    const double t_in = now_ms();
    drain_stager(p);
    int rc = bam_batch_prepare(bam, bp, refs, n_refs, &q, 0, -1, p->segs);
    if (rc != ISX_OK) return rc;
    const double t_prep = now_ms();
    std::unique_ptr<BamBatch, void (*)(BamBatch *)> Q(q, bam_batch_free);
    const int64_t n_pos = bam_batch_n_pos(q), n_obs = p->segs ? bam_batch_seg_bases(q) : bam_batch_n_obs(q);
    const std::vector<int64_t> &own = bam_batch_bounds(q);
    if (!split_bounds) { split_bounds = own.data(); n_splits = (int32_t)own.size() - 1; }
    if (n_splits <= 0) { isx_set_error("isx_pipe_submit_bam: no splits"); return ISX_ERR_ARG; }
    if (info) bam_batch_info(q, n_refs, info);
    if (p->segs) {
        isxenc::SegJob J;
        J.n_seg = bam_batch_n_segs(q);
        J.gpos_all = bam_batch_seg_gpos(q);
        J.want_pairs = p->prm.enable_linkage != 0;
        if (p->drec && !getenv("ISX_BAM_SEG_WORDS")) J.produce_planes = [q](int64_t first, int64_t count, uint32_t *g, uint8_t *l, uint8_t *m, uint32_t *pr, uint64_t *pl) { bam_batch_emit_planes(q, first, count, g, l, m, pr, pl); };
        else J.produce = [q](int64_t first, int64_t count, uint32_t *g, uint8_t *l, uint8_t *m, uint32_t *pr, uint32_t *b) { bam_batch_emit_segs(q, first, count, g, l, m, pr, b); };
        rc = submit_segs_common(p, n_pos, ref, n_splits, split_bounds, J, ticket);
    } else {
        isxenc::EncodeJob J;
        J.obs = nullptr;
        J.want_pairs = p->prm.enable_linkage != 0;
        J.produce = [q](int64_t first, uint32_t count, isx_obs *o, uint32_t *pr) { bam_batch_emit(q, first, count, o, pr); };
        rc = submit_common(p, n_pos, ref, n_splits, split_bounds, n_obs, J, ticket);
    }
    const double t_sub = now_ms();
    if (rc == ISX_OK) {
        std::lock_guard<std::mutex> lk(p->mu);
        Slot &s = p->slots[(size_t)(*ticket % (int64_t)p->slots.size())];
        if (s.ticket == *ticket && s.state == 1) s.dead_batch = Q.release();
    }
    if (Q) bam_batch_retire(Q.release());
    if (pipe_timing)
        fprintf(stderr, "[isx_pipe_submit_bam] prepare %.1f ms, encode + enqueue %.1f ms, free %.1f ms\n", t_prep - t_in, t_sub - t_prep, now_ms() - t_sub);
    return rc;
}

int isx_pipe_collect(isx_pipe *p, int64_t ticket, isx_pipe_result *out)
{
    if (!p || !out || ticket < 0) { isx_set_error("isx_pipe_collect: bad argument"); return ISX_ERR_ARG; }
    Slot &s = p->slots[(size_t)(ticket % (int64_t)p->slots.size())];
    isx_ctx *c = p->ctx;
    isx_batch *b = s.b;
    const bool dense = b->M == 1;
    *out = isx_pipe_result{};
    {
        const double t0 = now_ms();
        std::unique_lock<std::mutex> lk(p->mu);
        if (ticket < p->next_promise) p->cv_done.wait(lk, [&] { return p->next_ticket > ticket; });
        if (s.ticket != ticket || s.state == 0) { isx_set_error("isx_pipe_collect: unknown or already released ticket"); return ISX_ERR_STATE; }
        p->cv_done.wait(lk, [&] { return s.state == 2; });
        out->collect_wait_ms = (float)(now_ms() - t0);
        if (s.rc != ISX_OK) { isx_set_error(s.err); return s.rc; }
    }
    HIP_TRY(hipSetDevice(c->device));
    out->ticket = ticket;
    out->n_pos = b->n_pos; out->n_obs = b->n_obs;
    out->sizes = b->sizes;
    out->snv = (size_t)b->sizes.n_snv > p->snv_prefix ? s.snv_big.data() : reinterpret_cast<const isx_snv *>(s.h_small + s.o_snv);
    if (dense) {
        if (s.cov4) {
            out->coverage4 = s.h_out + s.o_cov16;
            out->cov_rows = reinterpret_cast<const uint16_t *>(s.h_out + s.o_cov16 + s.cov_rows_off);
            out->cov_row_window = s.cov_row_win.data();
            out->n_cov_rows = (int64_t)s.cov_row_win.size();
            out->cov_window = s.cov_window;
        } else if (s.cov8) out->coverage8 = s.h_out + s.o_cov16;
        else out->coverage16 = reinterpret_cast<const uint16_t *>(s.h_out + s.o_cov16);
        if (s.clon_sparse) { out->clon_sparse = reinterpret_cast<const isx_rare *>(s.h_out + s.o_clon); out->n_clon = (int64_t)b->n_clon; }
        else out->clon = reinterpret_cast<const float *>(s.h_out + s.o_clon);
        out->n_saturated = b->n_sat;
        out->saturated = s.sat_complete ? s.sat_rows.data() : nullptr;
        if (p->prm.rarefied_coverage > 0) {
            out->n_rare = (int64_t)b->n_rare;
            if (!s.rare_dense) out->rare = s.rare_big.empty() ? reinterpret_cast<const isx_rare *>(s.h_small + s.o_rare) : s.rare_big.data();
            if (p->pp.want_counts) out->clon_rarefied = reinterpret_cast<const float *>(s.h_out + s.o_clonr);
            else if (s.rare_dense) out->clon_rarefied = s.clonr_big.data();
        }
        if (p->pp.want_counts) out->counts = reinterpret_cast<const uint32_t *>(s.h_out + s.o_counts);
    }
    if (b->lev_sparse) {
        out->lev_mask = s.h_out + s.o_lmask;
        out->lev_win_off = reinterpret_cast<const uint32_t *>(s.h_out + s.o_lwin);
        out->lev_cov = s.lcov_big.empty() ? s.h_out + s.o_lcov : s.lcov_big.data();
        out->lev_clon = s.lclon_big.empty() ? reinterpret_cast<const isx_rare *>(s.h_out + s.o_lclon) : s.lclon_big.data();
        out->lev_rare = s.lrare_big.empty() ? reinterpret_cast<const isx_rare *>(s.h_out + s.o_lrare) : s.lrare_big.data();
        out->lev_sat = s.sat_rows.data();
        out->n_lev = b->sizes.n_entries; out->n_lev_clon = (int64_t)b->n_clon; out->n_lev_sat = (int64_t)b->n_sat;
        out->n_lev_rare = p->prm.rarefied_coverage > 0 ? (int64_t)b->n_rare : 0;
        out->lev_mask_bytes = b->lev_mask_bytes; out->lev_cov_bytes = b->lev_cov_bytes;
        out->lev_window = b->W; out->n_lev_windows = b->n_win; out->lev_min_cov = p->prm.min_cov;
    }
    out->batch = b;
    out->encode_ms = s.encode_ms;
    out->encode_passes = s.encode_passes;
    out->record_bytes = p->rb;
    out->h2d_bytes = s.h2d_bytes; out->d2h_bytes = s.d2h_bytes;
    out->ld = p->prm.enable_linkage ? s.ld_rows.data() : nullptr;
    out->rows_checksum = s.rows_checksum;
    float ms = 0.f;
    if (s.h2d_split) {
        float m1 = 0.f, m2 = 0.f;
        if (hipEventElapsedTime(&m1, s.ev_h2d0, s.ev_h2da) == hipSuccess && hipEventElapsedTime(&m2, s.ev_h2db, s.ev_h2d1) == hipSuccess) out->h2d_ms = m1 + m2;
    } else if (hipEventElapsedTime(&ms, s.ev_h2d0, s.ev_h2d1) == hipSuccess) out->h2d_ms = ms;
    if (hipEventElapsedTime(&ms, s.ev_d2h0, s.ev_d2h1) == hipSuccess) out->d2h_ms = ms;
    isx_timings t{};
    if (isx_batch_timings(b, &t) == ISX_OK) out->kernel_ms = t.pileup_ms;
    return ISX_OK;
}

static int pipe_fetch_entries(isx_pipe *p, int64_t ticket, isx_entry *out, const EntrySoa *soa);

int isx_pipe_fetch_entries(isx_pipe *p, int64_t ticket, isx_entry *out)
{
    if (!out) { isx_set_error("isx_pipe_fetch_entries: bad argument"); return ISX_ERR_ARG; }
    return pipe_fetch_entries(p, ticket, out, nullptr);
}

int isx_pipe_fetch_entries_shrunk(isx_pipe *p, int64_t ticket, uint32_t *gpos, uint32_t *mm_cov, float *clon, float *clon_rarefied)
{
    if (!gpos || !mm_cov || !clon || !clon_rarefied) { isx_set_error("isx_pipe_fetch_entries_shrunk: bad argument"); return ISX_ERR_ARG; }
    const EntrySoa soa{gpos, mm_cov, clon, clon_rarefied};
    return pipe_fetch_entries(p, ticket, nullptr, &soa);
}

static int pipe_fetch_entries(isx_pipe *p, int64_t ticket, isx_entry *out, const EntrySoa *soa)
{
    if (!p || ticket < 0) { isx_set_error("isx_pipe_fetch_entries: bad argument"); return ISX_ERR_ARG; }
    Slot &s = p->slots[(size_t)(ticket % (int64_t)p->slots.size())];
    {
        std::lock_guard<std::mutex> lk(p->mu);
        if (s.ticket != ticket || s.state != 2 || s.rc != ISX_OK) { isx_set_error("isx_pipe_fetch_entries: collect the batch first"); return ISX_ERR_STATE; }
    }
    isx_batch *b = s.b;
    if (b->M == 1) { isx_set_error("n_mm_bins == 1: the dense tables come with isx_pipe_collect"); return ISX_ERR_STATE; }
    HIP_TRY(hipSetDevice(p->ctx->device));
    const size_t n = (size_t)b->sizes.n_entries;
    if (!n) return ISX_OK;
    if (b->lev_sparse && soa) {
        isx_pipe_result r;
        const int rc = isx_pipe_collect(p, ticket, &r);
        if (rc != ISX_OK) return rc;
        return isx_levels_expand(&r, std::max(1, std::min(p->pool ? p->pool->size() : 1, 16)), soa->gpos, soa->mm_cov, soa->clon, soa->clon_rarefied);
    }
    if (b->lev_sparse && !b->d_entries) {
        isx_set_error("isx_pipe_fetch_entries: a lean slot keeps no 32-byte entries (the levels come with isx_pipe_collect: isx_pipe_result.lev_*, isx_levels_expand)");
        return ISX_ERR_STATE;
    }
    const size_t region = p->ring_half ? 2 * (size_t)p->ring_half * p->rb : (size_t)p->cap_rec * p->rb;
    const size_t piece = std::min<size_t>((size_t)32 << 20, region / 2 / 4096 * 4096);
    if (piece < ((size_t)1 << 20))
        return fetch_entries_sorted(p->ctx->stream, b->d_entries, b->d_win_nent, (uint32_t)b->slab, entry_wins(b), b->n_ovf, n, out, nullptr, soa);
    uint8_t *bounce[2] = {s.h_in + s.off_rec, s.h_in + s.off_rec + piece};
    hipEvent_t ev[2] = {nullptr, nullptr};
    for (hipEvent_t &e : ev) HIP_TRY(hipEventCreateWithFlags(&e, hipEventDisableTiming));
    const EntryCopier copier = [&](const void *dsrc, void *hdst, size_t bytes, hipStream_t st) -> int {
// ... 89 lines not shown
```

### instrain_amd/csrc/seg_encode.cpp

```cpp
#include "seg_encode.h"

#include <immintrin.h>

#include <algorithm>
#include <atomic>
#include <cstdlib>
#include <cstring>
#include <string>
#include <vector>

void isx_set_error(const std::string &msg);

namespace isxenc {

namespace {

constexpr int64_t TASK = 4096;
constexpr uint32_t SPAN = 65535u;

inline int64_t count_groups(const uint32_t *gpos, int64_t a, int64_t e, int64_t group = ISX_SEG_GROUP)
{
    int64_t n = 0;
    for (int64_t i = a; i < e;) {
        uint32_t lo = gpos[i], hi = gpos[i];
// ... 650 lines not shown
                S.gpos.resize((size_t)TASK); S.pair.resize((size_t)TASK); S.len.resize((size_t)TASK); S.mm.resize((size_t)TASK);
                S.planes.resize((size_t)TASK * ISX_PLANE_WORDS + 8);
                S.pl = reinterpret_cast<uint64_t *>((reinterpret_cast<uintptr_t>(S.planes.data()) + 63) & ~(uintptr_t)63);
            }
            J.produce_planes(a, e - a, S.gpos.data(), S.len.data(), J.n_mm_bins > 1 ? S.mm.data() : nullptr, pairs ? S.pair.data() : nullptr, S.pl);
            gp = S.gpos.data() - a; ln = S.len.data() - a; pr = pairs ? S.pair.data() - a : nullptr;
            if (J.n_mm_bins > 1) mmv = S.mm.data() - a;
            pl = S.pl - (size_t)a * ISX_PLANE_WORDS;
        } else {
            gp = J.in2.gpos; ln = J.in2.len; pr = pairs ? J.in2.pair : nullptr; pl = J.in2.planes;
            if (J.n_mm_bins > 1) mmv = J.in2.mm;
        }
        PlaneTask K;
        K.a = a; K.e = e; K.gp = gp; K.ln = ln; K.mm = mmv; K.pr = pr; K.pl = pl; K.gpos_all = gpos_all;
        K.rec0 = RG ? J.rec + (size_t)((int64_t)half * RG) * group_words : J.rec;
        K.g0 = RG ? wave_g0 : 0; K.ga = g_at[(size_t)t]; K.ge = g_at[(size_t)t + 1]; K.fast_store = fast_store;
        if (variant == 2) planes_task_avx512(J, err, K);
        else if (variant == 1) planes_task_bmi2(J, err, K);
        else planes_task_portable(J, err, K);
        if (err.load(std::memory_order_relaxed) != SEG_OK) return;
        need_of[(size_t)t] = K.used;
        bases_of[(size_t)t] = K.nb; maxp_of[(size_t)t] = K.maxp; pieces_of[(size_t)t] = K.np;
    };
    if (!RG) pool.run(n_tasks, [&](int t) { run_task(t, 0, 0); });
    else {
        int half = 0;
        for (int t0 = 0; t0 < n_tasks && err.load() == SEG_OK;) {
            int t1 = t0 + 1;
            while (t1 < n_tasks && g_at[(size_t)t1 + 1] - g_at[(size_t)t0] <= RG) t1++;
            if (g_at[(size_t)t1] - g_at[(size_t)t0] > RG) return SEG_CAPACITY;
            J.wave_begin(half);
            const int64_t wg0 = g_at[(size_t)t0];
            pool.run(t1 - t0, [&](int k) { run_task(t0 + k, wg0, half); });
            if (err.load() == SEG_OK) J.wave_flush(half, wg0, g_at[(size_t)t1]);
            t0 = t1; half ^= 1;
        }
    }
    if (err.load() != SEG_OK) return err.load();
    J.n_bases = 0; J.max_pair = 0; J.n_pieces = 0;
    int64_t worst = 0;
    bool fits = true;
    J.task_need.assign(need_of.begin(), need_of.begin() + n_tasks);
    for (int t = 0; t < n_tasks; t++) {
        J.n_bases += bases_of[(size_t)t]; J.max_pair = std::max(J.max_pair, maxp_of[(size_t)t]); J.n_pieces += pieces_of[(size_t)t];
        const int64_t region = g_at[(size_t)t + 1] - g_at[(size_t)t];
        if (need_of[(size_t)t] > region) fits = false;
        worst = std::max(worst, need_of[(size_t)t] - (region - (J.task_groups ? 0 : slack)));
    }
    J.need_slack = fits ? slack : std::max<int64_t>(worst, slack + 1);
    if (!fits) return SEG_CAPACITY;
    return SEG_OK;
}


namespace {
__attribute__((target("bmi2")))
inline void pack_ref_piece_bmi2(const uint8_t *r, int64_t n, uint8_t *o2, uint8_t *on, bool &seen)
{
    int64_t i = 0;
    uint64_t any = 0;
    for (; i + 8 <= n; i += 8) {
        uint64_t x;
        memcpy(&x, r + i, 8);
        const uint64_t bad = x & 0xFCFCFCFCFCFCFCFCull;
        if (__builtin_expect(bad == 0, 1)) {
            const uint16_t v = (uint16_t)_pext_u64(x, 0x0303030303030303ull);
            memcpy(o2 + (i >> 2), &v, 2);
            on[i >> 3] = 0;
            continue;
        }
        uint64_t t = bad | (bad >> 4);
        t |= t >> 2; t |= t >> 1;
        const uint64_t nb = t & 0x0101010101010101ull;
        const uint64_t keep = ~(nb * 0xFFull);
        const uint16_t v = (uint16_t)_pext_u64(x & keep, 0x0303030303030303ull);
        memcpy(o2 + (i >> 2), &v, 2);
        on[i >> 3] = (uint8_t)_pext_u64(nb, 0x0101010101010101ull);
        any |= nb;
    }
    for (; i < n; i += 8) {
        uint32_t lo = 0, hi = 0, nbits = 0;
        const int64_t m = std::min<int64_t>(8, n - i);
        for (int64_t k = 0; k < m; k++) {
            const uint32_t c = r[i + k];
            const uint32_t b = c > 3u;
            nbits |= b << k;
            const uint32_t v = b ? 0u : c;
            if (k < 4) lo |= v << (2 * k); else hi |= v << (2 * (k - 4));
        }
        o2[i >> 2] = (uint8_t)lo;
        if (m > 4) o2[(i >> 2) + 1] = (uint8_t)hi;
        on[i >> 3] = (uint8_t)nbits;
        any |= nbits;
    }
    seen = any != 0;
}

inline void pack_ref_piece_scalar(const uint8_t *r, int64_t n, uint8_t *o2, uint8_t *on, bool &seen)
{
    seen = false;
    for (int64_t i = 0; i < n; i += 8) {
        uint32_t lo = 0, hi = 0, nb = 0;
        const int64_t m = std::min<int64_t>(8, n - i);
        for (int64_t k = 0; k < m; k++) {
            const uint32_t c = r[i + k];
            const uint32_t bad = c > 3u;
// ... 265 lines not shown
    if (bad.load()) { isx_set_error("a segment's length is not in [1, 150]"); return ISX_ERR_ARG; }
    return ISX_OK;
}

int isx_encode_planes(const isx_read_planes *reads, const isx_ref_planes *ref, int64_t n_pos, int32_t host_threads, int32_t slack_groups,
                      int64_t cap_rec, int64_t ring_records, uint32_t *rec, uint32_t *gbase, int64_t *n_rec, int64_t *need_slack)
{
    return isx_encode_planes_mm(reads, ref, n_pos, 1, host_threads, slack_groups, cap_rec, ring_records, rec, gbase, n_rec, need_slack);
}

int isx_encode_planes_mm(const isx_read_planes *reads, const isx_ref_planes *ref, int64_t n_pos, int32_t n_mm_bins, int32_t host_threads, int32_t slack_groups,
                         int64_t cap_rec, int64_t ring_records, uint32_t *rec, uint32_t *gbase, int64_t *n_rec, int64_t *need_slack)
{
    if (n_mm_bins < 1 || n_mm_bins > 128) { isx_set_error("isx_encode_planes: n_mm_bins must be in [1, 128]"); return ISX_ERR_ARG; }
    if (!reads || !ref || !ref->plane2 || !rec || !gbase || !n_rec || reads->n_seg < 0 || cap_rec < ISX_DREC_GROUP || (cap_rec % ISX_DREC_GROUP) || n_pos <= 0 ||
        (reads->n_seg && (!reads->gpos || !reads->len || !reads->planes)) || ring_records < 0 ||
        (ring_records % (2 * ISX_DREC_GROUP)) || slack_groups < 0) {
        isx_set_error("isx_encode_planes: bad argument");
        return ISX_ERR_ARG;
    }
    std::vector<uint32_t> ring;
    isxenc::HostPool pool(std::max(1, host_threads), -1, false);
    std::vector<uint32_t> cmin((size_t)(cap_rec / ISX_DREC_GROUP)), cmax(cmin.size());
    std::vector<uint8_t> cany(cmin.size());
    isxenc::SegJob J;
    J.in2 = *reads; J.n_seg = reads->n_seg; J.n_pos = n_pos; J.n_mm_bins = n_mm_bins;
    J.ref2 = ref->plane2; J.refn = ref->nplane; J.slack_groups = std::max(1, slack_groups);
    J.rec = rec; J.gbase = gbase; J.pair_out = nullptr;
    J.cmin = cmin.data(); J.cmax = cmax.data(); J.cany = cany.data(); J.cap_rec = cap_rec;
    if (ring_records) {
        const int64_t half = ring_records / 2;
        ring.assign((size_t)ring_records * ISX_DREC_WORDS + 16, 0xABABABABu);
        uint32_t *r0 = reinterpret_cast<uint32_t *>((reinterpret_cast<uintptr_t>(ring.data()) + 63) & ~(uintptr_t)63);
        J.rec = r0;
        J.ring_groups = half / ISX_DREC_GROUP;
        J.wave_begin = [](int) {};
        J.wave_flush = [&, r0](int h, int64_t g0, int64_t g1) {
            const size_t gw = (size_t)ISX_DREC_GROUP * ISX_DREC_WORDS;
            memcpy(rec + (size_t)g0 * gw, r0 + (size_t)h * half * ISX_DREC_WORDS, (size_t)(g1 - g0) * gw * 4);
            std::fill_n(r0 + (size_t)h * half * ISX_DREC_WORDS, (size_t)half * ISX_DREC_WORDS, 0xABABABABu);
        };
    }
    const int rc = isxenc::encode_planes(pool, J);
    if (need_slack) *need_slack = J.need_slack;
    *n_rec = J.n_rec;
    if (rc == isxenc::SEG_CAPACITY) {
        isx_set_error(J.need_slack > J.slack_groups ? "isx_encode_planes: a task needs more spare groups than slack_groups (see *need_slack)"
                                                    : "isx_encode_planes: the stream does not fit cap_rec records");
        return ISX_ERR_CAPACITY;
    }
    if (rc == isxenc::SEG_BAD_POS) { isx_set_error("a segment reaches beyond n_pos"); return ISX_ERR_ARG; }
    if (rc == isxenc::SEG_BAD_LEN) { isx_set_error("a segment's length is not in [1, 150]"); return ISX_ERR_ARG; }
    if (rc == isxenc::SEG_MM_RANGE) { isx_set_error("a segment has mm >= n_mm_bins"); return ISX_ERR_MM_RANGE; }
    return ISX_OK;
}

int isx_pack_read_planes(int64_t n_reads, const int64_t *ref_start, const int64_t *clip_lo, const int64_t *clip_hi,
                         const uint32_t *cigar, const int64_t *cigar_off, const char *seq, const uint8_t *qual, const int64_t *seq_off,
                         const uint32_t *pair, int32_t min_base_quality, int64_t cap_seg, uint32_t *seg_gpos,
                         uint8_t *seg_len, uint32_t *seg_pair, uint64_t *seg_planes, int64_t *n_seg)
{
    if (n_reads < 0 || !n_seg || cap_seg < 0 || (n_reads && (!ref_start || !clip_lo || !clip_hi || !cigar || !cigar_off || !seq || !qual || !seq_off)) ||
        (cap_seg && (!seg_gpos || !seg_len || !seg_planes)) || (pair && cap_seg && !seg_pair)) {
        isx_set_error("isx_pack_read_planes: bad argument");
        return ISX_ERR_ARG;
    }
    int64_t n = 0;
    bool full = false, bad = false;
    for (int64_t r = 0; r < n_reads && !full && !bad; r++) {
        const char *sq = seq + seq_off[r];
        const uint8_t *ql = qual + seq_off[r];
        const int64_t q_len = seq_off[r + 1] - seq_off[r];
        const bool ok = for_runs(cigar + cigar_off[r], cigar_off[r + 1] - cigar_off[r], ref_start[r], clip_lo[r], clip_hi[r],
                                 [&](int64_t pos, int64_t q0, int64_t cols) {
            if (q0 + cols > q_len || pos < 0 || pos + cols > (int64_t)0xFFFFFFFFll) { bad = true; return; }
            for (int64_t c0 = 0; c0 < cols && !full; c0 += ISX_SEG_BASES) {
                const int L = (int)std::min<int64_t>(ISX_SEG_BASES, cols - c0);
                if (n >= cap_seg) { full = true; return; }
                uint64_t *P = seg_planes + (size_t)n * ISX_PLANE_WORDS;
                for (int k = 0; k < ISX_PLANE_WORDS; k++) P[k] = 0;
                for (int j = 0; j < L; j++) {
                    const int64_t qi = q0 + c0 + j;
                    const uint32_t code = (int)ql[qi] >= min_base_quality ? ascii_code(sq[qi]) : 4u;
                    if (code >= 4) {
                        P[5 + (j >> 6)] |= (uint64_t)1 << (j & 63);
                        if (code == 5) { P[j >> 5] |= (uint64_t)1 << (2 * (j & 31)); P[7] |= (uint64_t)1 << 63; }
                    } else P[j >> 5] |= (uint64_t)code << (2 * (j & 31));
                }
                seg_gpos[n] = (uint32_t)(pos + c0); seg_len[n] = (uint8_t)L;
                if (seg_pair) seg_pair[n] = pair ? pair[r] : 0u;
                n++;
            }
        });
        if (!ok) { isx_set_error("isx_pack_read_planes: unknown CIGAR operator"); return ISX_ERR_ARG; }
    }
    if (bad) { isx_set_error("isx_pack_read_planes: a CIGAR reaches beyond its read's bases or the flat space"); return ISX_ERR_ARG; }
    if (full) { isx_set_error("isx_pack_read_planes: more segments than cap_seg (isx_count_read_segs gives the number)"); return ISX_ERR_CAPACITY; }
    *n_seg = n;
    return ISX_OK;
}

}
```

### instrain_amd/csrc/seg_encode.h

```cpp
#pragma once
#include <stdint.h>

#include <functional>
#include <vector>

#include "../../include/instrain_amd.h"
#include "obs_encode.h"

#define ISX_SEG_GROUP 16
#define ISX_SEG_REC_WORDS 16
#define ISX_DREC_GROUP 32

namespace isxenc {

struct SegJob {
    isx_segs in{};
    std::function<void(int64_t first, int64_t count, uint32_t *gpos, uint8_t *len, uint8_t *mm, uint32_t *pair, uint32_t *bases)> produce;
    const uint32_t *gpos_all = nullptr;
    isx_read_planes in2{};
    std::function<void(int64_t first, int64_t count, uint32_t *gpos, uint8_t *len, uint8_t *mm, uint32_t *pair, uint64_t *planes)> produce_planes;
    const uint8_t *ref2 = nullptr, *refn = nullptr;
    int64_t n_seg = 0, n_pos = 0;
    int n_mm_bins = 1;
    bool want_pairs = false;
    uint32_t *rec = nullptr;
    uint32_t *gbase = nullptr;
    uint32_t *pair_out = nullptr;
    uint32_t *cmin = nullptr, *cmax = nullptr;
    uint8_t *cany = nullptr;
    int64_t cap_rec = 0;
    int64_t ring_groups = 0;
    std::function<void(int half)> wave_begin;
    std::function<void(int half, int64_t g0, int64_t g1)> wave_flush;
    const uint8_t *ref = nullptr;
    int64_t slack_groups = 1;
    int64_t need_slack = 0;
    std::vector<int64_t> task_need;
    const int64_t *task_groups = nullptr;
    int64_t n_pieces = 0;
    int64_t n_rec = 0;
    int64_t n_bases = 0;
    uint32_t max_pair = 0;
};

enum { SEG_OK = 0, SEG_CAPACITY = 1, SEG_MM_RANGE = 2, SEG_BAD_POS = 3, SEG_BAD_LEN = 4 };

int encode_segs(HostPool &pool, SegJob &job);
int encode_delta(HostPool &pool, SegJob &job);
int encode_planes(HostPool &pool, SegJob &job);
int64_t delta_groups_needed(HostPool &pool, const uint32_t *gpos, int64_t n, int64_t slack_groups);
int64_t seg_groups_needed(HostPool &pool, const uint32_t *gpos, int64_t n);
bool pack_ref_planes(HostPool &pool, const uint8_t *ref, int64_t n_pos, uint8_t *plane2, uint8_t *nplane);
void planes_from_words(const uint32_t *words, uint32_t len, uint64_t *planes);

}
```

### instrain_amd/csrc/seg_planes.inc

```

#if ISX_PLANES_VARIANT == 2
static inline __attribute__((always_inline)) __m256i ISX_DIFFERS_FN(const uint8_t *q, uint32_t sh, __m512i P)
{
    const __m512i lo = _mm512_maskz_loadu_epi64((__mmask8)0x1F, q), hi = _mm512_maskz_loadu_epi64((__mmask8)0x1F, q + 8);
    const __m512i r = _mm512_shrdv_epi64(lo, hi, _mm512_set1_epi64((long long)sh));
    const __m512i x = _mm512_xor_si512(r, P);
    const __m512i m = _mm512_or_si512(x, _mm512_srli_epi64(x, 1));
    const __m512i nib = _mm512_gf2p8affine_epi64_epi8(m, _mm512_set1_epi64((long long)0x0104104000000000ull), 0);
    const __m512i t = _mm512_or_si512(nib, _mm512_srli_epi16(nib, 4));
    return _mm512_cvtepi16_epi8(t);
}
#else
static inline __attribute__((always_inline)) void ISX_DIFFERS_FN(const uint8_t *q, uint32_t sh, const uint64_t *P, uint64_t d[3])
{
    uint64_t w[6];
    memcpy(w, q, 48);
    uint64_t e[5];
    for (int i = 0; i < 5; i++) {
        const uint64_t r = (w[i] >> sh) | ((w[i + 1] << 1) << (63 - sh));
        const uint64_t x = r ^ P[i];
        const uint64_t m = x | (x >> 1);
#if ISX_PLANES_VARIANT == 1
        e[i] = _pext_u64(m, 0x5555555555555555ull);
#else
        e[i] = even_bits_portable(m);
#endif
    }
    d[0] = e[0] | (e[1] << 32);
    d[1] = e[2] | (e[3] << 32);
    d[2] = e[4];
}
#endif

static __attribute__((noinline)) void ISX_CLOSE_FN(SegJob &J, const PlaneTask &K, PlaneGroup &G)
{
    if (!G.n) return;
    if (G.g < K.ge) {
        for (int r = G.n; r < ISX_DREC_GROUP; r++) put_empty_drec(G.rec[r]);
        uint32_t *o = K.rec0 + (size_t)(G.g - K.g0) * (size_t)ISX_DREC_GROUP * ISX_DREC_WORDS;
        if (!K.fast_store) memcpy(o, G.rec, sizeof G.rec);
        else {
#if ISX_PLANES_VARIANT == 2
            for (int r = 0; r < ISX_DREC_GROUP; r += 2) _mm512_stream_si512(reinterpret_cast<__m512i *>(o + (size_t)r * ISX_DREC_WORDS), _mm512_load_si512(G.rec[r]));
#else
            const __m128i *src = reinterpret_cast<const __m128i *>(G.rec);
            __m128i *dst = reinterpret_cast<__m128i *>(o);
            for (int i = 0; i < ISX_DREC_GROUP * ISX_DREC_WORDS / 4; i++) _mm_stream_si128(dst + i, _mm_load_si128(src + i));
#endif
        }
        J.gbase[G.g] = G.lo; J.cmin[G.g] = G.lo; J.cmax[G.g] = G.last; J.cany[G.g] = 1;
        G.g++;
    }
    G.used++;
    G.n = 0; G.open = -1;
}

#if ISX_PLANES_VARIANT == 0
#define ISX_TZ64(x) ((x) ? (uint32_t)__builtin_ctzll(x) : 64u)
#else
#define ISX_TZ64(x) ((uint32_t)_tzcnt_u64(x))
#endif
static void ISX_PLANES_FN(SegJob &J, std::atomic<int> &err, PlaneTask &K)
{
    static const LenMasks LM;
    PlaneGroup G;
    G.g = K.ga;
    const uint8_t *const ref2 = J.ref2, *const refn = J.refn;
    const int64_t n_pos = J.n_pos;
    const int64_t safe_pos = n_pos - 200;
    const uint32_t *const gp = K.gp, *const pr = K.pr, *const ga = K.gpos_all;
    const uint8_t *const ln = K.ln;
    int64_t nb = 0, np = 0;
    uint32_t maxp = 0;
    auto place = [&](uint32_t start, uint32_t len, bool plain, bool &fill) __attribute__((always_inline)) -> uint32_t * {
        fill = plain && G.open >= 0;
        if (G.n) {
            const uint32_t nlo = std::min(G.lo, start), nhi = std::max(G.hi, start);
            if (__builtin_expect(nhi - nlo > SPAN || (!fill && G.n == ISX_DREC_GROUP), 0)) { ISX_CLOSE_FN(J, K, G); fill = false; }
        }
        if (!G.n) { G.lo = G.hi = start; G.last = start + len - 1; }
        else {
            if (__builtin_expect(start < G.lo, 0)) rebase_drecs(G, start);
            G.hi = std::max(G.hi, start); G.last = std::max(G.last, start + len - 1);
        }
        np++;
        if (fill) { uint32_t *o = G.rec[G.open] + 4; G.open = -1; return o; }
        uint32_t *o = G.rec[G.n];
        G.open = plain ? G.n : -1;
        G.n++;
        return o;
    };
    uint32_t hdr_hi = 0;
    auto add_full = [&](uint32_t start, uint32_t len, uint32_t pid, uint64_t s0, uint64_t s1, uint64_t s2, uint32_t exc) __attribute__((always_inline)) {
        bool fill;
        uint32_t *o = place(start, len, false, fill);
        const uint64_t v0 = (uint64_t)((start - G.lo) | (len << 16) | hdr_hi) | (s0 << 32), v1 = (s0 >> 32) | ((uint64_t)exc << 32);
        const uint64_t v3 = (s2 & 0xFFFFFFFFull) | ((uint64_t)pid << 32);
        memcpy(o, &v0, 8); memcpy(o + 2, &v1, 8); memcpy(o + 4, &s1, 8); memcpy(o + 6, &v3, 8);
    };
    auto add_plain = [&](uint32_t start, uint32_t len, uint32_t pid, uint32_t exc0, uint32_t exc1) __attribute__((always_inline)) {
        bool fill;
        uint32_t *o = place(start, len, true, fill);
        const uint64_t v0 = (uint64_t)((start - G.lo) | (len << 16) | hdr_hi | ISX_DREC_DUAL) | ((uint64_t)pid << 32), v1 = (uint64_t)exc0 | ((uint64_t)exc1 << 32);
        memcpy(o, &v0, 8); memcpy(o + 2, &v1, 8);
        if (!fill) {
            const uint64_t v2 = (uint64_t)ISX_DREC_DUAL, v3 = (uint64_t)ISX_DREC_NO_EXC | ((uint64_t)ISX_DREC_NO_EXC << 32);
            memcpy(o + 4, &v2, 8); memcpy(o + 6, &v3, 8);
        }
    };
#if ISX_PLANES_VARIANT == 2
    const __m256i rec_idx = _mm256_setr_epi32(8, 0, 1, 8, 2, 3, 4, 8);
#endif
    const bool mm_on = J.n_mm_bins > 1;
    const int64_t pf_end = K.e - PLANES_PREFETCH;
    for (int64_t s = K.a; s < K.e; s++) {
        const uint32_t L = ln[s], p = gp[s];
        const uint64_t *P = K.pl + (size_t)s * ISX_PLANE_WORDS;
        if (s < pf_end) {
            _mm_prefetch(reinterpret_cast<const char *>(P + (size_t)PLANES_PREFETCH * ISX_PLANE_WORDS), _MM_HINT_T0);
            _mm_prefetch(reinterpret_cast<const char *>(ref2 + (gp[s + PLANES_PREFETCH] >> 2) + 40), _MM_HINT_T0);
// ... 24 lines not shown
            alignas(32) uint64_t t[8];
            _mm256_store_si256(reinterpret_cast<__m256i *>(t), skv);
            _mm256_store_si256(reinterpret_cast<__m256i *>(t + 4), exv);
            s0 = t[0]; s1 = t[1]; s2 = t[2];
            ex[0] = t[4]; ex[1] = t[5]; ex[2] = t[6];
        } else
#endif
        {
            s0 = P[5] & lm[0]; s1 = P[6] & lm[1]; s2 = P[7] & lm[2];
            uint64_t d[3];
#if ISX_PLANES_VARIANT == 2
            alignas(32) uint64_t dq[4];
#define ISX_DIFFERS_AT(q_, sh_) do { _mm256_store_si256(reinterpret_cast<__m256i *>(dq), ISX_DIFFERS_FN((q_), (sh_), _mm512_loadu_si512(P))); d[0] = dq[0]; d[1] = dq[1]; d[2] = dq[2]; } while (0)
#else
#define ISX_DIFFERS_AT(q_, sh_) ISX_DIFFERS_FN((q_), (sh_), P, d)
#endif
            if (__builtin_expect((int64_t)p < safe_pos, 1)) {
                ISX_DIFFERS_AT(ref2 + (p >> 2), (p & 3u) * 2u);
                if (refn) {
                    uint64_t nn[3];
                    if (__builtin_expect((int64_t)p + 264 <= n_pos, 1)) bits160(refn + (p >> 3), p & 7u, nn);
                    else {
                        uint8_t bn[32] = {0};
                        const int64_t haven = (n_pos + 7) / 8 - (int64_t)(p >> 3);
                        memcpy(bn, refn + (p >> 3), (size_t)std::min<int64_t>(32, haven));
                        bits160(bn, p & 7u, nn);
                    }
                    d[0] |= nn[0]; d[1] |= nn[1]; d[2] |= nn[2];
                }
            } else {
                alignas(64) uint8_t buf[64] = {0};
                const int64_t have2 = (n_pos + 3) / 4 - (int64_t)(p >> 2);
                memcpy(buf, ref2 + (p >> 2), (size_t)std::min<int64_t>(48, have2));
                ISX_DIFFERS_AT(buf, (p & 3u) * 2u);
                if (refn) {
                    uint8_t bn[32] = {0};
                    const int64_t haven = (n_pos + 7) / 8 - (int64_t)(p >> 3);
                    memcpy(bn, refn + (p >> 3), (size_t)std::min<int64_t>(32, haven));
                    uint64_t nn[3];
                    bits160(bn, p & 7u, nn);
                    d[0] |= nn[0]; d[1] |= nn[1]; d[2] |= nn[2];
                }
            }
#undef ISX_DIFFERS_AT
            ex[0] = d[0] & (lm[0] ^ s0); ex[1] = d[1] & (lm[1] ^ s1); ex[2] = d[2] & (lm[2] ^ s2);
            if (__builtin_expect(n_marked, 0)) {
                ex[0] |= (even_bits_portable(P[0]) | (even_bits_portable(P[1]) << 32)) & s0;
                ex[1] |= (even_bits_portable(P[2]) | (even_bits_portable(P[3]) << 32)) & s1;
                ex[2] |= even_bits_portable(P[4]) & s2;
            }
        }
        const bool plain = (s0 | s1 | s2) == 0;
        const uint32_t n_exc = (uint32_t)(__builtin_popcountll(ex[0]) + __builtin_popcountll(ex[1]) + __builtin_popcountll(ex[2]));
        if (__builtin_expect(n_exc <= 1, 1)) {
            const uint32_t t0 = ISX_TZ64(ex[0]), t1 = ISX_TZ64(ex[1]), t2 = ISX_TZ64(ex[2] | ((uint64_t)1 << 63));
            const uint32_t m0 = 0u - (uint32_t)(ex[0] == 0), m01 = m0 & (0u - (uint32_t)(ex[1] == 0));
            const uint32_t col = t0 + (t1 & m0) + (t2 & m01);
            const uint32_t code = (uint32_t)(P[col >> 5] >> (2 * (col & 31u))) & 3u;
            const uint32_t w0 = 0x3FFFFC00u | ((col | (code << 8) | (0u - (uint32_t)(n_exc == 0))) & 0x3FFu);
            if (__builtin_expect(plain, 0)) { add_plain(p, L, pid, w0, ISX_DREC_NO_EXC); continue; }
#if ISX_PLANES_VARIANT == 2
            if (__builtin_expect(in_regs, 1)) {
                bool fill;
                uint32_t *o = place(p, L, false, fill);
                __m256i v = _mm256_permutex2var_epi32(skv, rec_idx, _mm256_set1_epi32((int)w0));
                v = _mm256_mask_set1_epi32(v, (__mmask8)0x01, (int)((p - G.lo) | (L << 16) | hdr_hi));
                v = _mm256_mask_set1_epi32(v, (__mmask8)0x80, (int)pid);
                _mm256_store_si256(reinterpret_cast<__m256i *>(o), v);
                continue;
            }
#endif
            add_full(p, L, pid, s0, s1, s2, w0);
            continue;
        }
        const uint32_t max_exc = plain ? ISX_DREC_EXC : ISX_DREC_EXC_FULL;
        if (__builtin_expect(n_exc <= max_exc, 1)) {
            uint64_t fields = 0;
            for (uint32_t i = 0; i < n_exc; i++) {
                const int k = ex[0] ? 0 : (ex[1] ? 1 : 2);
                const uint32_t col = (uint32_t)(64 * k + __builtin_ctzll(ex[k]));
                ex[k] &= ex[k] - 1;
                const uint64_t code = (P[col >> 5] >> (2 * (col & 31u))) & 3u;
                fields |= ((uint64_t)col | (code << 8)) << (10 * i);
            }
            const uint64_t all = (fields | (0x0FFFFFFFFFFFFFFFull << (10 * n_exc))) & 0x0FFFFFFFFFFFFFFFull;
            const uint32_t w0 = (uint32_t)all & ISX_DREC_NO_EXC, w1 = (uint32_t)(all >> 30) & ISX_DREC_NO_EXC;
            if (plain) add_plain(p, L, pid, w0, w1);
            else add_full(p, L, pid, s0, s1, s2, w0);
            continue;
        }
        const uint64_t sk[3] = {s0, s1, s2};
        uint32_t b = 0;
        while (b < L) {
            uint32_t w[2] = {ISX_DREC_NO_EXC, ISX_DREC_NO_EXC};
            uint32_t nf = 0, end = L;
            for (int k = 0; k < 3; k++) {
                while (ex[k]) {
                    const uint32_t col = (uint32_t)(64 * k + __builtin_ctzll(ex[k]));
                    if (nf == max_exc) { end = col; goto cut; }
                    ex[k] &= ex[k] - 1;
                    const uint32_t code = (uint32_t)(P[col >> 5] >> (2 * (col & 31u))) & 3u;
                    const uint32_t f = ((col - b) & 0xFFu) | (code << 8);
                    const int wi = (int)(nf / 3), shf = 10 * (int)(nf % 3);
                    w[wi] = (w[wi] & ~(0x3FFu << shf)) | (f << shf);
                    nf++;
                }
// ... 23 lines not shown
```

### instrain_amd/engine.py

```python
import ctypes as C
import os

import numpy as np

from . import _lib
from ._lib import (ENTRY_DT, LD_DT, OBS_DT, SNV_DT, BamInfo, BamParams, IsxError, Params, Sizes,
                   Timings, check)


def pack_obs(gpos, base, mm):
    o = np.empty(len(gpos), dtype=OBS_DT)
    o["gpos"] = gpos
    o["mm"] = mm
    o["base"] = base
    o["flags"] = 0
    return o


class SegBatch:

    def __init__(self, gpos, length, bases, mm=None, pair=None):
        self.gpos = np.ascontiguousarray(gpos, dtype=np.uint32)
        self.len = np.ascontiguousarray(length, dtype=np.uint8)
        self.bases = np.ascontiguousarray(bases, dtype=np.uint32).reshape(-1, _lib.SEG_WORDS)
# ... 479 lines not shown
                                            C.byref(cs), C.byref(h)))
        w = Wire(self, h)
        self._wires.append(w)
        return w

    def submit_planes(self, ref_planes, split_bounds, reads, keyed=True):
        split_bounds = np.ascontiguousarray(split_bounds, dtype=np.int64)
        cr, cf = reads.c(with_pair=self.enable_linkage), ref_planes.c(keyed)
        t = C.c_int64(-1)
        check(self.lib.isx_pipe_submit_planes(self.h, ref_planes.n_pos, C.byref(cf), len(split_bounds) - 1, split_bounds.ctypes.data,
                                              C.byref(cr), C.byref(t)))
        if self.stage_async:
            self._held[t.value] = (ref_planes, reads, cr, cf)
        return t.value

    def set_reference_budget(self, mib):
        check(self.lib.isx_pipe_set_reference_budget(self.h, int(mib)))

    def stage_planes(self, ref_planes, split_bounds, reads):
        split_bounds = np.ascontiguousarray(split_bounds, dtype=np.int64)
        cr, cf = reads.c(with_pair=self.enable_linkage), ref_planes.c()
        h = C.c_void_p()
        check(self.lib.isx_pipe_stage_planes(self.h, ref_planes.n_pos, C.byref(cf), len(split_bounds) - 1, split_bounds.ctypes.data,
                                             C.byref(cr), C.byref(h)))
        w = Wire(self, h)
        self._wires.append(w)
        return w

    def submit_wire(self, wire):
        t = C.c_int64(-1)
        check(self.lib.isx_pipe_submit_wire(self.h, wire.h, C.byref(t)))
        return t.value

    def submit_bam(self, bamfile, refs, ref_codes, split_bounds=None, **kw):
        refs = np.ascontiguousarray(refs, dtype=np.int32)
        ref_codes = np.ascontiguousarray(ref_codes, dtype=np.uint8)
        sb = None if split_bounds is None else np.ascontiguousarray(split_bounds, dtype=np.int64)
        p = BamFile._params(**kw)
        info = BamInfo()
        t = C.c_int64(-1)
        rc = self.lib.isx_pipe_submit_bam(self.h, bamfile.h, C.byref(p), refs.ctypes.data, len(refs), ref_codes.ctypes.data,
                                          0 if sb is None else len(sb) - 1, None if sb is None else sb.ctypes.data,
                                          C.byref(info), C.byref(t))
        bamfile._info(info)
        check(rc)
        return t.value

    def collect(self, ticket, want_ld=True, rare_list=True, densify=True, shrunk_entries=False):
        r = _lib.PipeResult()
        check(self.lib.isx_pipe_collect(self.h, int(ticket), C.byref(r)))
        sz = {n: getattr(r.sizes, n) for n, _ in Sizes._fields_}
        out = {"sizes": sz, "ticket": r.ticket, "rows_checksum": int(r.rows_checksum),
               "stats": {k: getattr(r, k) for k in ("encode_ms", "h2d_ms", "kernel_ms", "d2h_ms", "collect_wait_ms",
                                                    "record_bytes", "encode_passes", "h2d_bytes", "d2h_bytes")}}
        n_pos = int(r.n_pos)

        def view(addr, dtype, n):
            if not n:
                return np.empty(0, dtype=dtype)
            return np.frombuffer((C.c_uint8 * (n * np.dtype(dtype).itemsize)).from_address(addr), dtype=dtype)

        slot = _SlotBatch(self.ctx, r.batch, n_pos, r.n_obs, self.n_mm_bins)
        if self.n_mm_bins == 1:
            if r.coverage16:
                out["cov16"] = view(r.coverage16, np.uint16, n_pos)
            elif r.coverage4:
                out["cov4"] = view(r.coverage4, np.uint8, (n_pos + 1) // 2)
                out["cov_window"] = int(r.cov_window)
                out["cov_row_win"] = view(r.cov_row_window, np.uint32, int(r.n_cov_rows)).copy()
                out["cov_rows"] = view(r.cov_rows, np.uint16, int(r.n_cov_rows) * int(r.cov_window)).reshape(-1, int(r.cov_window))
            else:
                out["cov8"] = view(r.coverage8, np.uint8, n_pos)
            if r.clon:
                out["clon"] = view(r.clon, np.float32, n_pos)
            else:
                out["clon_sparse"] = view(r.clon_sparse, _lib.CLON_DT, int(r.n_clon))
            if r.n_saturated and r.saturated:
                out["saturated"] = view(r.saturated, _lib.SAT_DT, int(r.n_saturated)).copy()
            if densify and ("cov8" in out or "cov4" in out):
                out["cov16"] = dense_cov(out, n_pos)
                for k in ("cov8", "cov4", "cov_rows", "cov_row_win", "cov_window"):
                    out.pop(k, None)
            if densify and "clon_sparse" in out:
                out["clon"] = dense_clon(out["cov16"], out.pop("clon_sparse"), self.min_cov)
            if r.clon_rarefied:
                out["clon_r"] = view(r.clon_rarefied, np.float32, n_pos)
            if r.rare:
                out["rare"] = view(r.rare, _lib.RARE_DT, int(r.n_rare))
            elif r.clon_rarefied and not rare_list:
                pass
            elif r.clon_rarefied:
                k = np.flatnonzero(~np.isnan(out["clon_r"]))
                out["rare"] = np.empty(len(k), dtype=_lib.RARE_DT)
                out["rare"]["gpos"] = k
                out["rare"]["clon_rarefied"] = out["clon_r"][k]
            else:
                out["rare"] = np.empty(0, dtype=_lib.RARE_DT)
            out["n_saturated"] = int(r.n_saturated)
            if r.counts:
                out["counts"] = view(r.counts, np.uint32, n_pos * 4).reshape(n_pos, 4)
                if "clon_r" not in out:
                    out["clon_r"] = np.full(n_pos, np.nan, np.float32)
        else:
            n_e = sz["n_entries"]
            got = False
            if r.lev_mask:
                out["levels"] = {"mask": view(r.lev_mask, {1: np.uint8, 2: np.uint16, 4: np.uint32}[int(r.lev_mask_bytes)], n_pos),
# ... 167 lines not shown

def encode_segs(segs, n_pos, n_mm_bins=1, threads=1, cap_rec=None, ring_records=0):
    lib = _lib.load()
    if cap_rec is None:
        cap_rec = int(lib.isx_seg_records_needed(segs.gpos.ctypes.data if segs.n_seg else None, segs.n_seg, int(threads)))
    rec = np.empty((cap_rec, 16), dtype=np.uint32)
    gbase = np.empty(cap_rec // 16, dtype=np.uint32)
    pout = np.empty(cap_rec, dtype=np.uint32) if segs.pair is not None else None
    n_rec = C.c_int64(0)
    cs = segs.c()
    check(lib.isx_encode_segs_ring(C.byref(cs), int(n_pos), int(n_mm_bins), int(threads), int(cap_rec), int(ring_records), rec.ctypes.data,
                                   gbase.ctypes.data, pout.ctypes.data if pout is not None else None, C.byref(n_rec)))
    n = n_rec.value
    return rec[:n], gbase[:n // 16], (pout[:n] if pout is not None else None)


def encode_delta(segs, ref_codes, n_mm_bins=1, threads=1, slack_groups=1, cap_rec=None, ring_records=0, retry=True):
    lib = _lib.load()
    ref = np.ascontiguousarray(ref_codes, dtype=np.uint8)
    while True:
        cap = cap_rec if cap_rec is not None else int(lib.isx_delta_records_needed(segs.gpos.ctypes.data if segs.n_seg else None, segs.n_seg, int(threads), int(slack_groups)))
        rec = np.empty((cap, 8), dtype=np.uint32)
        gbase = np.empty(cap // 32, dtype=np.uint32)
        n_rec, need = C.c_int64(0), C.c_int64(0)
        cs = segs.c()
        rc = lib.isx_encode_delta(C.byref(cs), ref.ctypes.data, len(ref), int(n_mm_bins), int(threads), int(slack_groups), cap, int(ring_records),
                                  rec.ctypes.data, gbase.ctypes.data, None, C.byref(n_rec), C.byref(need))
        if rc == _lib.ERR_CAPACITY and retry and need.value > slack_groups and cap_rec is None:
            slack_groups = int(need.value)
            continue
        check(rc)
        n = n_rec.value
        return rec[:n], gbase[:n // 32], None, slack_groups


def encode_planes(reads, ref_planes, threads=1, slack_groups=1, cap_rec=None, ring_records=0, retry=True, n_mm_bins=1):
    lib = _lib.load()
    while True:
        cap = cap_rec if cap_rec is not None else int(lib.isx_delta_records_needed(reads.gpos.ctypes.data if reads.n_seg else None, reads.n_seg, int(threads), int(slack_groups)))
        rec = _aligned((cap, 8), np.uint32)
        gbase = np.empty(cap // 32, dtype=np.uint32)
        n_rec, need = C.c_int64(0), C.c_int64(0)
        cr, cf = reads.c(), ref_planes.c()
        rc = lib.isx_encode_planes_mm(C.byref(cr), C.byref(cf), ref_planes.n_pos, int(n_mm_bins), int(threads), int(slack_groups), cap, int(ring_records),
                                      rec.ctypes.data, gbase.ctypes.data, C.byref(n_rec), C.byref(need))
        if rc == _lib.ERR_CAPACITY and retry and need.value > slack_groups and cap_rec is None:
            slack_groups = int(need.value)
            continue
        check(rc)
        n = n_rec.value
        return rec[:n], gbase[:n // 32], None, slack_groups


def dense_cov(res, n_pos=None):
    if "cov16" in res:
        return res["cov16"]
    if "cov8" in res:
        cov = res["cov8"].astype(np.uint16)
    else:
        nib = res["cov4"]
        n_pos = 2 * len(nib) if n_pos is None else int(n_pos)
        cov = np.empty(2 * len(nib), dtype=np.uint16)
        cov[0::2] = nib & 15
        cov[1::2] = nib >> 4
        cov = cov[:n_pos]
        W = int(res["cov_window"])
        for k, w in enumerate(res["cov_row_win"].tolist()):
            lo = w * W
            hi = min(lo + W, n_pos)
            cov[lo:hi] = res["cov_rows"][k, :hi - lo]
    if "saturated" in res:
        cov[res["saturated"]["gpos"]] = np.minimum(res["saturated"]["coverage"], 65535)
    return cov


DREC_DUAL = 0x80000000
DREC_NO_EXC = 0x3FFFFFFF


def decode_delta(rec, gbase, ref_codes):
    rec = np.asarray(rec, dtype=np.uint32).reshape(-1, 8)
    ref = np.asarray(ref_codes, dtype=np.uint8)
    n = len(rec)
    dual = (rec[:, 0] >> 31) == 1
    assert ((rec[dual, 4] >> 31) == 1).all(), "a dual record's second half carries the flag too"
    zero = np.zeros(n, dtype=np.uint32)
    none = np.full(n, DREC_NO_EXC, dtype=np.uint32)
    hdr = np.stack([rec[:, 0], np.where(dual, rec[:, 4], zero)], axis=1)
    pair = np.stack([np.where(dual, rec[:, 1], rec[:, 7]), np.where(dual, rec[:, 5], zero)], axis=1)
    e0 = np.stack([np.where(dual, rec[:, 2], rec[:, 3]), np.where(dual, rec[:, 6], none)], axis=1)
    e1 = np.stack([np.where(dual, rec[:, 3], none), np.where(dual, rec[:, 7], none)], axis=1)
    skw = [np.stack([np.where(dual, zero, rec[:, k]), zero], axis=1) for k in (1, 2, 4, 5, 6)]
    gb = np.repeat(np.asarray(gbase, dtype=np.uint32), 32)[:n]
    start = (gb[:, None] + (hdr & 0xFFFF)).astype(np.int64)
    ln = ((hdr >> 16) & 0xFF).astype(np.int64)
    lvl = ((hdr >> 24) & 0x7F).astype(np.uint8)
    full = np.stack([~dual, np.zeros(n, dtype=bool)], axis=1)
    real = (ln > 0).reshape(-1)
    flat = lambda x: x.reshape(-1)[real]
    st, ln, pr, e0, e1, fl, lvl = flat(start), flat(ln), flat(pair), flat(e0), flat(e1), flat(full), flat(lvl)
    words = np.stack([flat(w) for w in skw], axis=1)
    m = len(st)
    j = np.arange(160, dtype=np.int64)[None, :]
    skip = ((words[:, :, None] >> np.arange(32, dtype=np.uint32)[None, None, :]) & 1).reshape(m, 160).astype(bool)
    assert not (skip & (j >= ln[:, None])).any(), "skip bits beyond a piece's length"
    assert skip[fl].any(axis=1).all() or True
# ... 346 lines not shown
```

Baseline: 151.3.

## Send sparse reference words and move submit tail to a launcher thread

```diff
diff --git a/include/instrain_amd.h b/include/instrain_amd.h
--- a/include/instrain_amd.h
+++ b/include/instrain_amd.h
@@ -326,6 +326,8 @@
     int64_t n_lev, n_lev_clon, n_lev_rare, n_lev_sat;
     int32_t lev_mask_bytes, lev_cov_bytes, lev_window, n_lev_windows, lev_min_cov, pad_lev;
     uint64_t rows_checksum;
+    float tail_ms;
+    int32_t pad_tail;
 } isx_pipe_result;
 
 int isx_levels_expand(const isx_pipe_result *r, int32_t host_threads, uint32_t *gpos, uint32_t *mm_cov, float *clon, float *clon_rarefied);
@@ -407,6 +409,8 @@
                       int64_t cap_rec, int64_t ring_records, uint32_t *rec, uint32_t *gbase, int64_t *n_rec, int64_t *need_slack);
 int isx_encode_planes_mm(const isx_read_planes *reads, const isx_ref_planes *ref, int64_t n_pos, int32_t n_mm_bins, int32_t host_threads, int32_t slack_groups,
                          int64_t cap_rec, int64_t ring_records, uint32_t *rec, uint32_t *gbase, int64_t *n_rec, int64_t *need_slack);
+int isx_encode_planes_ref_words(const isx_read_planes *reads, const isx_ref_planes *ref, int64_t n_pos, int32_t host_threads,
+                                uint64_t *bits, uint32_t *ranks, uint64_t *words, int64_t *n_marked);
 
 int isx_count_read_segs(int64_t n_reads, const uint32_t *cigar, const int64_t *cigar_off, const int64_t *ref_start,
                         const int64_t *clip_lo, const int64_t *clip_hi, int64_t *n_seg);
diff --git a/instrain_amd/_lib.py b/instrain_amd/_lib.py
--- a/instrain_amd/_lib.py
+++ b/instrain_amd/_lib.py
@@ -95,7 +95,8 @@
                 ("lev_mask", C.c_void_p), ("lev_cov", C.c_void_p), ("lev_win_off", C.c_void_p), ("lev_clon", C.c_void_p), ("lev_rare", C.c_void_p),
                 ("lev_sat", C.c_void_p), ("n_lev", C.c_int64), ("n_lev_clon", C.c_int64), ("n_lev_rare", C.c_int64), ("n_lev_sat", C.c_int64),
                 ("lev_mask_bytes", C.c_int32), ("lev_cov_bytes", C.c_int32), ("lev_window", C.c_int32), ("n_lev_windows", C.c_int32),
-                ("lev_min_cov", C.c_int32), ("pad_lev", C.c_int32), ("rows_checksum", C.c_uint64)]
+                ("lev_min_cov", C.c_int32), ("pad_lev", C.c_int32), ("rows_checksum", C.c_uint64),
+                ("tail_ms", C.c_float), ("pad_tail", C.c_int32)]
 
 
 class BamParams(C.Structure):
@@ -161,7 +162,7 @@
            "isx_batch_summarize", "isx_batch_summarize_genomes", "isx_batch_genome_coverage", "isx_snv_level_counts", "isx_ld_level_sums", "isx_compare_coverage", "isx_compare_scaffolds", "isx_compare_fetch_snps",
            "isx_genes_create", "isx_genes_destroy", "isx_genes_sites", "isx_batch_profile_genes", "isx_genes_profile_snvs",
            "isx_pipe_create", "isx_pipe_destroy", "isx_pipe_submit", "isx_pipe_submit_reads", "isx_pipe_stage_reads", "isx_pipe_submit_wire", "isx_wire_bytes", "isx_wire_free", "isx_wire_keep_reference", "isx_pipe_submit_bam", "isx_encode_segs", "isx_encode_segs_ring", "isx_seg_records_needed", "isx_encode_delta", "isx_delta_records_needed", "isx_count_read_segs", "isx_pack_reads", "isx_pipe_collect", "isx_pipe_release", "isx_pipe_fetch_entries", "isx_pipe_fetch_entries_shrunk", "isx_levels_expand", "isx_encode_obs", "isx_encode_obs_ring",
-           "isx_pack_ref_planes", "isx_planes_from_segs", "isx_pack_read_planes", "isx_pipe_submit_planes", "isx_pipe_stage_planes", "isx_encode_planes", "isx_encode_planes_mm", "isx_pipe_set_reference_budget", "isx_host_register", "isx_host_unregister",
+           "isx_pack_ref_planes", "isx_planes_from_segs", "isx_pack_read_planes", "isx_pipe_submit_planes", "isx_pipe_stage_planes", "isx_encode_planes", "isx_encode_planes_mm", "isx_encode_planes_ref_words", "isx_pipe_set_reference_budget", "isx_host_register", "isx_host_unregister",
            "isx_bgzf_index", "isx_bgzf_inflate_device", "isx_bgzf_inflate_host", "isx_bgzf_inflate_fast",
            "isx_bam_open", "isx_bam_close", "isx_bam_close_wait", "isx_bam_set_threads", "isx_bam_ref", "isx_bam_set_priority_reads", "isx_bam_scan", "isx_bam_scan_part",
            "isx_bam_insert_sizes", "isx_bam_set_wanted_refs", "isx_bam_pair_keys", "isx_bam_set_cross_names", "isx_bam_filter_insert_sizes", "isx_bam_filter", "isx_bam_set_r2m", "isx_bam_r2m", "isx_bam_drop_names", "isx_bam_batch_pair_names", "isx_bam_set_mm_cap", "isx_bam_mm_levels", "isx_bam_set_mm_levels", "isx_bam_ref_counts",
@@ -286,6 +287,7 @@
     lib.isx_host_unregister.argtypes = [vp]
     lib.isx_pipe_stage_planes.argtypes = [vp, i64, C.POINTER(RefPlanes), i32, vp, C.POINTER(ReadPlanes), C.POINTER(vp)]
     lib.isx_encode_planes.argtypes = [C.POINTER(ReadPlanes), C.POINTER(RefPlanes), i64, i32, i32, i64, i64, vp, vp, C.POINTER(i64), C.POINTER(i64)]
+    lib.isx_encode_planes_ref_words.argtypes = [C.POINTER(ReadPlanes), C.POINTER(RefPlanes), i64, i32, vp, vp, vp, C.POINTER(i64)]
     lib.isx_encode_planes_mm.argtypes = [C.POINTER(ReadPlanes), C.POINTER(RefPlanes), i64, i32, i32, i32, i64, i64, vp, vp, C.POINTER(i64), C.POINTER(i64)]
     lib.isx_bam_ref.argtypes = [vp, i32, C.POINTER(C.c_char_p), C.POINTER(i64), C.POINTER(i64)]
     lib.isx_bam_copy.argtypes = [vp, vp, vp, vp, vp]
diff --git a/instrain_amd/csrc/isx_internal.h b/instrain_amd/csrc/isx_internal.h
--- a/instrain_amd/csrc/isx_internal.h
+++ b/instrain_amd/csrc/isx_internal.h
@@ -216,6 +216,7 @@
 void launch_pileup(const PileupArgs &a, int block, size_t lds, int grid, int packed, hipStream_t s, hipEvent_t ev_start,
                    hipEvent_t ev_stop);
 void launch_publish_state(const PileupArgs &a, uint32_t epoch, hipStream_t s);
+void launch_ref_expand(const uint64_t *bits, const uint32_t *ranks, const uint64_t *words, uint64_t *out, uint32_t n_words, hipStream_t s);
 void launch_win_order(const uint32_t *win_rec, uint32_t *win_out, int n_win, int W, const isx_snv *snv_raw, isx_snv *snv, const isx_site *sites_raw,
                       isx_site *sites, const uint2 *clon_raw, uint2 *clon, const uint2 *rare_raw, uint2 *rare, uint32_t *scan_state, uint32_t epoch, hipStream_t s);
 void launch_extract_gpos(const uint2 *rec, const uint32_t *rec32, const uint32_t *gbase, uint32_t *gpos, uint16_t *gpos16,
diff --git a/instrain_amd/csrc/isx_pipe.hip b/instrain_amd/csrc/isx_pipe.hip
--- a/instrain_amd/csrc/isx_pipe.hip
+++ b/instrain_amd/csrc/isx_pipe.hip
@@ -86,6 +86,9 @@
     uint64_t rows_checksum = 0;
     hipEvent_t ev_h2d0 = nullptr, ev_h2d1 = nullptr, ev_pass = nullptr, ev_d2h0 = nullptr, ev_d2h1 = nullptr;
     hipEvent_t ev_h2da = nullptr, ev_h2db = nullptr;
+    hipEvent_t ev_h2dc = nullptr, ev_h2dd = nullptr;
+    bool h2d_tail_split = false;
+    float tail_ms = 0.f;
     bool h2d_split = false;
     int64_t ticket = -1;
     BamBatch *dead_batch = nullptr;
@@ -98,6 +101,9 @@
     int encode_passes = 0;
     int64_t h2d_bytes = 0, d2h_bytes = 0;
     uint16_t *d_gpos16 = nullptr;
+    uint8_t *ref_mark = nullptr;
+    uint8_t *d_sparse = nullptr;
+    int64_t ref_words_sent = -1;
 };
 
 static uint64_t bytes_checksum(const void *p, size_t bytes, uint64_t seed)
@@ -214,6 +220,7 @@
     int rb = 2;
     bool segs = false;
     bool drec = false;
+    bool dense_ref = false;
     int64_t dslack = 1;
     uint32_t G = ISX_GROUP16;
     size_t snv_prefix = 0;
@@ -251,6 +258,20 @@
     std::condition_variable cv_stage;
     int64_t next_promise = 0;
     bool stage_stop = false;
+    struct TailJob {
+        Slot *s = nullptr;
+        int64_t ticket = -1, n_pos = 0;
+        int32_t n_splits = 0;
+        bool ref_early = false, early_rec = false, sparse = false;
+        uint8_t *resident = nullptr;
+        size_t ref2_sent = 0, ring_bytes = 0;
+        int rc = 0;
+        std::string err;
+    };
+    std::thread launcher;
+    std::deque<TailJob> launch_q;
+    std::condition_variable cv_launch;
+    bool launch_stop = false;
 };
 
 static int bounce_d2h(isx_pipe *p, void *hdst, const void *dsrc, size_t bytes, hipStream_t st)
@@ -288,6 +309,11 @@
         p->cv_stage.notify_all();
         p->stager.join();
     }
+    if (p->launcher.joinable()) {
+        { std::lock_guard<std::mutex> lk(p->mu); p->launch_stop = true; }
+        p->cv_launch.notify_all();
+        p->launcher.join();
+    }
     if (p->finisher.joinable()) {
         { std::lock_guard<std::mutex> lk(p->mu); p->stop = true; }
         p->cv_work.notify_all();
@@ -319,6 +345,8 @@
         t_batch += now_ms() - t_x; t_x = now_ms();
         if (s.sort_temp) isx_dev_free(s.sort_temp);
         if (s.d_gpos16) isx_dev_free(s.d_gpos16);
+        if (s.d_sparse) isx_dev_free(s.d_sparse);
+        free(s.ref_mark);
         if (s.d_in) isx_dev_free(s.d_in);
         if (s.d_runs) isx_dev_free(s.d_runs);
         t_dev += now_ms() - t_x; t_x = now_ms();
@@ -328,7 +356,7 @@
         host_block_free(s.h_out, s.out_pinned);
         if (s.h_small) isx_pin_free(s.h_small);
         t_pin += now_ms() - t_x;
-        for (hipEvent_t e : {s.ev_h2d0, s.ev_h2d1, s.ev_pass, s.ev_d2h0, s.ev_d2h1, s.ev_h2da, s.ev_h2db}) if (e) (void)hipEventDestroy(e);
+        for (hipEvent_t e : {s.ev_h2d0, s.ev_h2d1, s.ev_pass, s.ev_d2h0, s.ev_d2h1, s.ev_h2da, s.ev_h2db, s.ev_h2dc, s.ev_h2dd}) if (e) (void)hipEventDestroy(e);
     }
     if (pipe_timing)
         fprintf(stderr, "[isx_pipe_destroy] device tables %.1f ms, device arena %.1f ms, pinned staging %.1f ms, total %.1f ms\n", t_batch, t_dev, t_pin, now_ms() - t_f0);
@@ -460,6 +488,12 @@
         HIP_TRY(isx_dev_malloc(reinterpret_cast<void **>(&s.d_runs), s.cap_runs * sizeof(uint2)));
     }
     if (p->ring_half) for (hipEvent_t &e : s.ev_ring) HIP_TRY(hipEventCreateWithFlags(&e, hipEventDisableTiming));
+    if (b->lean && b->M == 1 && p->drec && !p->ring_half && !p->dense_ref) {
+        const size_t cap_words = ref2_bytes(cap_pos) / 8;
+        s.ref_mark = static_cast<uint8_t *>(calloc(cap_words + 64, 1));
+        if (!s.ref_mark) { isx_set_error("out of host memory"); return ISX_ERR_ARG; }
+        HIP_TRY(isx_dev_malloc(reinterpret_cast<void **>(&s.d_sparse), ref2_bytes(cap_pos) + 64));
+    }
     if (prm->enable_linkage && p->rb == 4) HIP_TRY(isx_dev_malloc(reinterpret_cast<void **>(&s.d_gpos16), (size_t)p->cap_rec * sizeof(uint16_t)));
     o = 0;
     s.o_snv = o; o = up(o + p->snv_prefix * sizeof(isx_snv));
@@ -490,7 +524,7 @@
     s.out_pinned = s.out_bytes <= ((size_t)64 << 20) || p->pp.depth > 2;
     { const int hrc = host_block_alloc(reinterpret_cast<void **>(&s.h_out), s.out_bytes, s.out_pinned); if (hrc != ISX_OK) return hrc; }
     if (pipe_timing) fprintf(stderr, "[isx_pipe_create] slot %d: %s results %.1f MB %.1f ms\n", index, s.out_pinned ? "pinned" : "pageable", s.out_bytes / 1e6, now_ms() - t_o0);
-    for (hipEvent_t *e : {&s.ev_h2d0, &s.ev_h2d1, &s.ev_pass, &s.ev_d2h0, &s.ev_d2h1, &s.ev_h2da, &s.ev_h2db}) HIP_TRY(hipEventCreate(e));
+    for (hipEvent_t *e : {&s.ev_h2d0, &s.ev_h2d1, &s.ev_pass, &s.ev_d2h0, &s.ev_d2h1, &s.ev_h2da, &s.ev_h2db, &s.ev_h2dc, &s.ev_h2dd}) HIP_TRY(hipEventCreate(e));
     const size_t n_chunks = (size_t)(p->cap_rec / (p->segs ? (int64_t)p->G : (int64_t)ISX_CHUNK)) + 2;
     s.cmin.resize(n_chunks); s.cmax.resize(n_chunks); s.cany.resize(n_chunks);
     return ISX_OK;
@@ -722,7 +756,41 @@
 }
 
 static int submit_segs_common(isx_pipe *p, int64_t n_pos, const uint8_t *ref, int32_t n_splits, const int64_t *split_bounds,
-                              isxenc::SegJob &J, int64_t *ticket, const isx_ref_planes *rp = nullptr);
+                              isxenc::SegJob &J, int64_t *ticket, const isx_ref_planes *rp = nullptr, int64_t promised = -1);
+static int submit_segs_tail(isx_pipe *p, const isx_pipe::TailJob &job);
+
+static void launch_push(isx_pipe *p, isx_pipe::TailJob &&job)
+{
+    { std::lock_guard<std::mutex> lk(p->mu); p->launch_q.push_back(std::move(job)); }
+    p->cv_launch.notify_one();
+}
+
+static void launcher_main(isx_pipe *p)
+{
+    (void)hipSetDevice(p->ctx->device);
+    for (;;) {
+        isx_pipe::TailJob job;
+        {
+            std::unique_lock<std::mutex> lk(p->mu);
+            p->cv_launch.wait(lk, [&] { return p->launch_stop || !p->launch_q.empty(); });
+            if (p->launch_q.empty()) return;
+            job = std::move(p->launch_q.front());
+            p->launch_q.pop_front();
+        }
+        Slot &s = *job.s;
+        int rc = job.rc;
+        std::string err;
+        err.swap(job.err);
+        if (rc == ISX_OK && (rc = submit_segs_tail(p, job)) != ISX_OK) err = isx_last_error();
+        if (rc != ISX_OK) {
+            (void)isx_wait_stream(H2D(p, s));
+            std::lock_guard<std::mutex> lk(p->mu);
+            s.ticket = job.ticket; s.rc = rc; s.err.swap(err); s.state = 2;
+            p->next_ticket = job.ticket + 1;
+        }
+        p->cv_done.notify_all();
+    }
+}
 
 static void stager_main(isx_pipe *p)
 {
@@ -739,21 +807,19 @@
         if (job.planes) { J.in2 = job.reads; J.n_seg = job.reads.n_seg; }
         else { J.in = job.segs; J.n_seg = job.segs.n_seg; }
         int64_t got = -1;
-        const int rc = submit_segs_common(p, job.n_pos, job.ref, (int32_t)job.bounds.size() - 1, job.bounds.data(), J, &got, job.planes ? &job.rp : nullptr);
+        const int rc = submit_segs_common(p, job.n_pos, job.ref, (int32_t)job.bounds.size() - 1, job.bounds.data(), J, &got, job.planes ? &job.rp : nullptr, job.ticket);
         if (rc != ISX_OK) {
-            Slot &s = p->slots[(size_t)(job.ticket % (int64_t)p->slots.size())];
-            std::string err(isx_last_error());
-            std::lock_guard<std::mutex> lk(p->mu);
-            s.ticket = job.ticket; s.rc = rc; s.err.swap(err); s.state = 2;
-            p->next_ticket = job.ticket + 1;
-        }
-        p->cv_done.notify_all();
+            isx_pipe::TailJob ej;
+            ej.s = &p->slots[(size_t)(job.ticket % (int64_t)p->slots.size())];
+            ej.ticket = job.ticket; ej.rc = rc; ej.err = isx_last_error();
+            launch_push(p, std::move(ej));
+        }
     }
 }
 
 static void drain_stager(isx_pipe *p)
 {
-    if (!p->stager.joinable()) return;
+    if (!p->stager.joinable() && !p->launcher.joinable()) return;
     std::unique_lock<std::mutex> lk(p->mu);
     p->cv_done.wait(lk, [&] { return p->next_ticket == p->next_promise; });
 }
@@ -778,6 +844,7 @@
     isx_pipe *p = new isx_pipe();
     p->ctx = c; p->prm = *prm; p->pp = *pp;
     p->segs = pp->max_segs > 0;
+    { const char *e = getenv("ISX_PIPE_DENSE_REF"); p->dense_ref = e && atoi(e) != 0; }
     p->drec = p->segs && !(prm->layout & ISX_LAYOUT_SEG64_RECORDS) && (prm->n_mm_bins == 1 || (prm->layout & ISX_LAYOUT_MM_DELTA_RECORDS));
     p->rb = p->segs ? (p->drec ? 32 : 64) : ((prm->n_mm_bins == 1 && !(prm->layout & ISX_LAYOUT_NO_SHORT_RECORDS)) ? 2 : 4);
     p->G = p->segs ? (p->drec ? ISX_DREC_GROUP : ISX_SEG_GROUP) : (p->rb == 2 ? ISX_GROUP16 : ISX_GROUP);
@@ -870,6 +937,7 @@
     }
     if (pipe_timing)
         fprintf(stderr, "[isx_pipe_create] thread pool %.1f ms, %d slot(s) %.1f ms\n", t_c1 - t_c0, pp->depth, now_ms() - t_c1);
+    if (p->segs) p->launcher = std::thread(launcher_main, p);
     if (pp->stage_async && p->segs) p->stager = std::thread(stager_main, p);
     *out = p;
     return ISX_OK;
@@ -1158,6 +1226,69 @@
     return ISX_OK;
 }
 
+
+static bool sparse_ref_applies(const isx_pipe *p, const Slot &s, const isx_ref_planes *rp)
+{
+    return s.ref_mark && rp && !(rp->key && (p->ref_cache_budget.load(std::memory_order_relaxed) > 0 || p->ref_cache.count(rp->key)));
+}
+
+static int sparse_ref_begin(isx_pipe *p, Slot &s, int64_t n_pos, const isx_ref_planes *rp, isxenc::SegJob &J, RefStage *out)
+{
+    const double t_r = now_ms();
+    const size_t bn = ((size_t)n_pos + 7) / 8;
+    hipStream_t st = H2D(p, s);
+    const bool any_n = rp->nplane && plane_any(*p->pool, rp->nplane, bn);
+    s.ref_has_n = any_n;
+    J.ref2 = rp->plane2; J.refn = any_n ? rp->nplane : nullptr; J.ref_mark = s.ref_mark;
+    HIP_TRY(hipEventRecord(s.ev_h2d0, st));
+    if (any_n) {
+        uint8_t *dn = s.d_in + s.off_ref + ref2_bytes(n_pos);
+        if (isx_host_is_registered(rp->nplane, bn)) HIP_TRY(hipMemcpyAsync(dn, rp->nplane, bn, hipMemcpyHostToDevice, st));
+        else {
+            uint8_t *hn = s.h_in + s.off_ref + ref2_bytes(n_pos);
+            const size_t piece = (size_t)1 << 20;
+            p->pool->run((int)((bn + piece - 1) / piece), [&](int t) { const size_t a = (size_t)t * piece; memcpy(hn + a, rp->nplane + a, std::min(piece, bn - a)); });
+            HIP_TRY(hipMemcpyAsync(dn, hn, bn, hipMemcpyHostToDevice, st));
+        }
+    }
+    HIP_TRY(hipEventRecord(s.ev_h2da, st));
+    out->early = true;
+    out->host_ms = now_ms() - t_r;
+    return ISX_OK;
+}
+
+static int sparse_ref_finish(isx_pipe *p, Slot &s, int64_t n_pos, const isx_ref_planes *rp, size_t *sent)
+{
+    hipStream_t st = H2D(p, s);
+    const size_t b2 = ((size_t)n_pos + 3) / 4;
+    const int64_t n_words = (int64_t)(ref2_bytes(n_pos) / 8), n64 = (n_words + 63) / 64;
+    uint8_t *h = s.h_in + s.off_ref;
+    uint64_t *bits = reinterpret_cast<uint64_t *>(h);
+    uint32_t *ranks = reinterpret_cast<uint32_t *>(h + (size_t)n64 * 8);
+    const size_t off_words = ((size_t)n64 * 12 + 7) & ~(size_t)7;
+    const int64_t k = isxenc::ref_words_scan(*p->pool, s.ref_mark, n_words, bits, ranks);
+    const size_t sparse_bytes = off_words + (size_t)k * 8;
+    if (sparse_bytes * 4 > b2 * 3) {
+        if (isx_host_is_registered(rp->plane2, b2)) HIP_TRY(hipMemcpyAsync(s.d_in + s.off_ref, rp->plane2, b2, hipMemcpyHostToDevice, st));
+        else {
+            const size_t piece = (size_t)1 << 20;
+            p->pool->run((int)((b2 + piece - 1) / piece), [&](int t) { const size_t a = (size_t)t * piece; memcpy(h + a, rp->plane2 + a, std::min(piece, b2 - a)); });
+            HIP_TRY(hipMemcpyAsync(s.d_in + s.off_ref, h, ref2_bytes(n_pos), hipMemcpyHostToDevice, st));
+        }
+        s.ref_words_sent = -1;
+        *sent = ref2_bytes(n_pos);
+        return ISX_OK;
+    }
+    isxenc::ref_words_gather(*p->pool, bits, ranks, n_words, rp->plane2, b2, reinterpret_cast<uint64_t *>(h + off_words));
+    HIP_TRY(hipMemcpyAsync(s.d_sparse, h, sparse_bytes, hipMemcpyHostToDevice, st));
+    launch_ref_expand(reinterpret_cast<const uint64_t *>(s.d_sparse), reinterpret_cast<const uint32_t *>(s.d_sparse + (size_t)n64 * 8),
+                      reinterpret_cast<const uint64_t *>(s.d_sparse + off_words), reinterpret_cast<uint64_t *>(s.d_in + s.off_ref), (uint32_t)n_words, st);
+    HIP_TRY(hipGetLastError());
+    s.ref_words_sent = k;
+    *sent = sparse_bytes;
+    return ISX_OK;
+}
+
 static int submit_common(isx_pipe *p, int64_t n_pos, const uint8_t *ref, int32_t n_splits, const int64_t *split_bounds,
                          int64_t n_obs, isxenc::EncodeJob &J, int64_t *ticket)
 {
@@ -1249,7 +1380,7 @@
         s.h2d_bytes += (int64_t)(rb + ib);
     }
     HIP_TRY(hipEventRecord(s.ev_h2d1, H2D(p, s)));
-    s.h2d_split = false;
+    s.h2d_split = false; s.tail_ms = 0.f;
 
     return enqueue_pass(p, s, n_pos, ticket);
 }
@@ -1275,16 +1406,27 @@
 }
 
 static int submit_segs_common(isx_pipe *p, int64_t n_pos, const uint8_t *ref, int32_t n_splits, const int64_t *split_bounds,
-                              isxenc::SegJob &J, int64_t *ticket, const isx_ref_planes *rp)
+                              isxenc::SegJob &J, int64_t *ticket, const isx_ref_planes *rp, int64_t promised)
 {
     static const char who[] = "isx_pipe_submit_reads";
     const bool planes_in = J.in2.planes != nullptr || (bool)J.produce_planes || (J.n_seg == 0 && rp != nullptr);
     int rc;
     if ((rc = check_capacity(p, who, n_pos, J.n_seg, p->pp.max_segs, n_splits)) != ISX_OK) return rc;
     if ((rc = check_split_bounds(n_pos, n_splits, split_bounds)) != ISX_OK) return rc;
-    Slot *slot = nullptr;
-    if ((rc = slot_acquire(p, who, &slot)) != ISX_OK) return rc;
-    Slot &s = *slot;
+    const int64_t n_slots = (int64_t)p->slots.size();
+    int64_t my_ticket = promised;
+    {
+        std::lock_guard<std::mutex> lk(p->mu);
+        if (promised < 0) {
+            my_ticket = p->next_promise;
+            if (my_ticket - n_slots >= p->next_ticket || p->slots[(size_t)(my_ticket % n_slots)].state != 0) {
+                isx_set_error(std::string(who) + ": every slot is in use (collect + release the oldest batch first)");
+                return ISX_ERR_STATE;
+            }
+        }
+    }
+    HIP_TRY(hipSetDevice(p->ctx->device));
+    Slot &s = p->slots[(size_t)(my_ticket % n_slots)];
     isx_batch *b = s.b;
     const bool linkage = p->prm.enable_linkage != 0;
 
@@ -1299,13 +1441,17 @@
     RingFeed feed;
     if ((rc = ring_feed_install(p, s, feed, J.ring_groups, J.wave_begin, J.wave_flush)) != ISX_OK) return rc;
     RefStage rs;
+    bool sparse = false;
+    size_t ref2_sent = 0;
     if (planes_in) {
         if (!p->drec) { isx_set_error("bit-plane reads need a pipe whose batches travel as reference-delta records (one mm bin, or ISX_LAYOUT_MM_DELTA_RECORDS)"); return ISX_ERR_STATE; }
-        if ((rc = stage_reference(p, s, n_pos, ref, rp, J, &rs)) != ISX_OK) return rc;
+        sparse = sparse_ref_applies(p, s, rp);
+        if ((rc = sparse ? sparse_ref_begin(p, s, n_pos, rp, J, &rs) : stage_reference(p, s, n_pos, ref, rp, J, &rs)) != ISX_OK) return rc;
     }
     if (p->drec) J.ref = ref;
     const int erc = encode_reads(p, s, J, planes_in, feed);
     const double t_enc = now_ms();
+    if (sparse && (erc != isxenc::SEG_OK || J.n_bases > p->pp.max_obs)) memset(s.ref_mark, 0, ref2_bytes(n_pos) / 8);
     if (feed.err != hipSuccess) { isx_set_error(std::string("isx_pipe_submit_reads: staging ring: ") + hipGetErrorString(feed.err)); return ISX_ERR_HIP; }
     if ((rc = seg_status_error(erc, "isx_pipe_submit_reads: the stream jumps too often for the pipe's record capacity (raise jump_slack)", ISX_ERR_CAPACITY)) != ISX_OK) return rc;
     if (J.n_bases > p->pp.max_obs) { isx_set_error("isx_pipe_submit_reads: more bases than the pipe's max_obs"); return ISX_ERR_CAPACITY; }
@@ -1321,23 +1467,59 @@
         }
         early_rec = true;
     }
+    double sparse_ms = 0.0;
+    if (sparse) {
+        const double t_s = now_ms();
+        if ((rc = sparse_ref_finish(p, s, n_pos, rp, &ref2_sent)) != ISX_OK) return rc;
+        sparse_ms = now_ms() - t_s;
+    } else s.ref_words_sent = -1;
     if (!planes_in) s.ref_has_n = isxenc::pack_ref_planes(*p->pool, ref, n_pos, s.h_in + s.off_ref, s.h_in + s.off_ref + ref2_bytes(n_pos));
     const double t_ref = now_ms();
     memcpy(s.h_in + s.off_bounds, split_bounds, (size_t)(n_splits + 1) * sizeof(int64_t));
 
     b->n_pos = n_pos; b->n_obs = J.n_bases; b->n_splits = n_splits; b->n_rec = (uint64_t)J.n_rec;
     b->n_pairs = (uint64_t)J.max_pair + 1;
-    if ((rc = slot_choose_windows(p, s, p->G, true)) != ISX_OK) return rc;
-    if ((rc = slot_shape_pass(p, s)) != ISX_OK) return rc;
-    slot_bind_inputs(p, s, rs.resident);
+    s.h2d_tail_split = early_rec;
+    if (early_rec) HIP_TRY(hipEventRecord(s.ev_h2dc, H2D(p, s)));
     s.encode_ms = (float)(now_ms() - t0);
     if (pipe_timing)
-        fprintf(stderr, "[isx_pipe_submit_reads] records %.2f ms, reference %.2f ms, bounds + windows %.2f ms; %lld segments, %lld records%s\n",
+        fprintf(stderr, "[isx_pipe_submit_reads] records %.2f ms, reference %.2f ms, bounds %.2f ms; %lld segments, %lld records%s\n",
                 t_enc - t0 - rs.host_ms, t_ref - t_enc + rs.host_ms, now_ms() - t_ref, (long long)J.n_seg, (long long)J.n_rec, planes_in ? " (bit planes)" : "");
+    if (pipe_timing && sparse)
+        fprintf(stderr, "[isx_pipe_submit_reads] reference words %.2f ms: %lld of %lld marked (%.1f %%)%s\n", sparse_ms, (long long)std::max<int64_t>(s.ref_words_sent, 0),
+                (long long)(ref2_bytes(n_pos) / 8), 100.0 * (double)std::max<int64_t>(s.ref_words_sent, 0) / (double)(ref2_bytes(n_pos) / 8), s.ref_words_sent < 0 ? " -> dense plane" : "");
+    isx_pipe::TailJob job;
+    job.s = &s; job.n_pos = n_pos; job.n_splits = n_splits;
+    job.ref_early = rs.early; job.early_rec = early_rec; job.sparse = sparse; job.resident = rs.resident;
+    job.ref2_sent = ref2_sent; job.ring_bytes = feed.bytes;
+    {
+        std::lock_guard<std::mutex> lk(p->mu);
+        if (promised < 0) p->next_promise = my_ticket + 1;
+        job.ticket = my_ticket;
+        p->launch_q.push_back(std::move(job));
+    }
+    p->cv_launch.notify_one();
+    *ticket = my_ticket;
+    return ISX_OK;
+}
+
+static int submit_segs_tail(isx_pipe *p, const isx_pipe::TailJob &job)
+{
+    Slot &s = *job.s;
+    isx_batch *b = s.b;
+    const int64_t n_pos = job.n_pos;
+    const int32_t n_splits = job.n_splits;
+    const bool linkage = p->prm.enable_linkage != 0, ring = p->ring_half > 0, sparse = job.sparse, early_rec = job.early_rec;
+    int rc;
+    const double t_q00 = now_ms();
+    if ((rc = slot_choose_windows(p, s, p->G, false)) != ISX_OK) return rc;
+    if ((rc = slot_shape_pass(p, s)) != ISX_OK) return rc;
+    slot_bind_inputs(p, s, job.resident);
     const double t_q0 = now_ms();
 
-    if (!ring && !rs.early) HIP_TRY(hipEventRecord(s.ev_h2d0, H2D(p, s)));
-    const size_t ref_bytes = ref2_bytes(n_pos) + (s.ref_has_n ? refn_bytes(n_pos) : 0);
+    if (!ring && !job.ref_early) HIP_TRY(hipEventRecord(s.ev_h2d0, H2D(p, s)));
+    if (early_rec) HIP_TRY(hipEventRecord(s.ev_h2dd, H2D(p, s)));
+    const size_t ref_bytes = (sparse ? job.ref2_sent : ref2_bytes(n_pos)) + (s.ref_has_n ? refn_bytes(n_pos) : 0);
     const size_t head = (size_t)(n_splits + 1) * sizeof(int64_t) + s.win.size() * sizeof(uint2) + ref_bytes;
     const size_t gb_bytes = (size_t)(b->n_rec / p->G) * sizeof(uint32_t), rec_bytes = (size_t)b->n_rec * (size_t)p->rb;
     if (s.off_win - s.off_bounds < ((size_t)1 << 20)) {
@@ -1346,11 +1528,11 @@
         HIP_TRY(hipMemcpyAsync(s.d_in + s.off_bounds, s.h_in + s.off_bounds, (size_t)(n_splits + 1) * sizeof(int64_t), hipMemcpyHostToDevice, H2D(p, s)));
         HIP_TRY(hipMemcpyAsync(s.d_in + s.off_win, s.h_in + s.off_win, s.win.size() * sizeof(uint2), hipMemcpyHostToDevice, H2D(p, s)));
     }
-    if (!rs.early) HIP_TRY(hipMemcpyAsync(s.d_in + s.off_ref, s.h_in + s.off_ref, ref_bytes, hipMemcpyHostToDevice, H2D(p, s)));
+    if (!job.ref_early) HIP_TRY(hipMemcpyAsync(s.d_in + s.off_ref, s.h_in + s.off_ref, ref_bytes, hipMemcpyHostToDevice, H2D(p, s)));
     if (!early_rec) HIP_TRY(hipMemcpyAsync(s.d_in + s.off_gbase, s.h_in + s.off_gbase, gb_bytes, hipMemcpyHostToDevice, H2D(p, s)));
-    if (ring) { if (feed.bytes != rec_bytes) { isx_set_error("internal: the staging ring did not carry the whole stream"); return ISX_ERR_STATE; } }
+    if (ring) { if (job.ring_bytes != rec_bytes) { isx_set_error("internal: the staging ring did not carry the whole stream"); return ISX_ERR_STATE; } }
     else if (!early_rec) HIP_TRY(hipMemcpyAsync(s.d_in + s.off_rec, s.h_in + s.off_rec, rec_bytes, hipMemcpyHostToDevice, H2D(p, s)));
-    s.h2d_bytes = (int64_t)(head + gb_bytes + rec_bytes) - (rs.resident ? (int64_t)ref_bytes : 0);
+    s.h2d_bytes = (int64_t)(head + gb_bytes + rec_bytes) - (job.resident ? (int64_t)ref_bytes : 0);
     if (linkage && !p->drec) {
         HIP_TRY(hipMemcpyAsync(s.d_in + s.off_pairs, s.h_in + s.off_pairs, (size_t)b->n_rec * sizeof(uint32_t), hipMemcpyHostToDevice, H2D(p, s)));
         s.h2d_bytes += (int64_t)b->n_rec * 4;
@@ -1358,8 +1540,10 @@
     HIP_TRY(hipEventRecord(s.ev_h2d1, H2D(p, s)));
     s.h2d_split = early_rec;
     const double t_q1 = now_ms();
-    rc = enqueue_pass(p, s, n_pos, ticket);
-    if (pipe_timing) fprintf(stderr, "[isx_pipe_submit_reads] copy-in queue %.2f ms, pass + copy-out queue %.2f ms\n", t_q1 - t_q0, now_ms() - t_q1);
+    int64_t launched = -1;
+    rc = enqueue_pass(p, s, n_pos, &launched);
+    s.tail_ms = (float)(now_ms() - t_q00);
+    if (pipe_timing) fprintf(stderr, "[isx_pipe launcher] windows + pass shape %.2f ms, copy-in queue %.2f ms, pass + copy-out queue %.2f ms\n", t_q0 - t_q00, t_q1 - t_q0, now_ms() - t_q1);
     return rc;
 }
 
@@ -1543,7 +1727,7 @@
     if (w->pairs_bytes) HIP_TRY(hipMemcpyAsync(s.d_in + s.off_pairs, w->h + w->o_pairs, w->pairs_bytes, hipMemcpyHostToDevice, H2D(p, s)));
     HIP_TRY(hipMemcpyAsync(s.d_in + s.off_rec, w->h + w->o_rec, w->rec_bytes, hipMemcpyHostToDevice, H2D(p, s)));
     HIP_TRY(hipEventRecord(s.ev_h2d1, H2D(p, s)));
-    s.h2d_split = false;
+    s.h2d_split = false; s.tail_ms = 0.f;
     s.h2d_bytes = isx_wire_bytes(w);
     s.encode_ms = (float)(now_ms() - t0);
     s.encode_passes = 0;
@@ -1643,6 +1827,7 @@
         if (p->drec && !getenv("ISX_BAM_SEG_WORDS")) J.produce_planes = [q](int64_t first, int64_t count, uint32_t *g, uint8_t *l, uint8_t *m, uint32_t *pr, uint64_t *pl) { bam_batch_emit_planes(q, first, count, g, l, m, pr, pl); };
         else J.produce = [q](int64_t first, int64_t count, uint32_t *g, uint8_t *l, uint8_t *m, uint32_t *pr, uint32_t *b) { bam_batch_emit_segs(q, first, count, g, l, m, pr, b); };
         rc = submit_segs_common(p, n_pos, ref, n_splits, split_bounds, J, ticket);
+        if (rc == ISX_OK) drain_stager(p);
     } else {
         isxenc::EncodeJob J;
         J.obs = nullptr;
@@ -1719,6 +1904,7 @@
     }
     out->batch = b;
     out->encode_ms = s.encode_ms;
+    out->tail_ms = s.tail_ms;
     out->encode_passes = s.encode_passes;
     out->record_bytes = p->rb;
     out->h2d_bytes = s.h2d_bytes; out->d2h_bytes = s.d2h_bytes;
@@ -1727,7 +1913,11 @@
     float ms = 0.f;
     if (s.h2d_split) {
         float m1 = 0.f, m2 = 0.f;
-        if (hipEventElapsedTime(&m1, s.ev_h2d0, s.ev_h2da) == hipSuccess && hipEventElapsedTime(&m2, s.ev_h2db, s.ev_h2d1) == hipSuccess) out->h2d_ms = m1 + m2;
+        if (s.h2d_tail_split) {
+            float m3 = 0.f;
+            if (hipEventElapsedTime(&m1, s.ev_h2d0, s.ev_h2da) == hipSuccess && hipEventElapsedTime(&m2, s.ev_h2db, s.ev_h2dc) == hipSuccess &&
+                hipEventElapsedTime(&m3, s.ev_h2dd, s.ev_h2d1) == hipSuccess) out->h2d_ms = m1 + m2 + m3;
+        } else if (hipEventElapsedTime(&m1, s.ev_h2d0, s.ev_h2da) == hipSuccess && hipEventElapsedTime(&m2, s.ev_h2db, s.ev_h2d1) == hipSuccess) out->h2d_ms = m1 + m2;
     } else if (hipEventElapsedTime(&ms, s.ev_h2d0, s.ev_h2d1) == hipSuccess) out->h2d_ms = ms;
     if (hipEventElapsedTime(&ms, s.ev_d2h0, s.ev_d2h1) == hipSuccess) out->d2h_ms = ms;
     isx_timings t{};
diff --git a/instrain_amd/csrc/isx_refwords.hip b/instrain_amd/csrc/isx_refwords.hip
--- /dev/null
+++ b/instrain_amd/csrc/isx_refwords.hip
@@ -0,0 +1,23 @@
+#include "isx_internal.h"
+
+namespace {
+
+__global__ void __launch_bounds__(256) k_ref_expand(const uint64_t *__restrict__ bits, const uint32_t *__restrict__ ranks,
+                                                    const uint64_t *__restrict__ words, uint64_t *__restrict__ out, uint32_t n_words)
+{
+    const uint32_t j = blockIdx.x * 256u + threadIdx.x;
+    if (j >= n_words) return;
+    const uint64_t m = bits[j >> 6];
+    const uint32_t k = j & 63u;
+    uint64_t w = 0;
+    if ((m >> k) & 1ull) w = words[ranks[j >> 6] + (uint32_t)__popcll(m & (((uint64_t)1 << k) - 1ull))];
+    out[j] = w;
+}
+
+}
+
+void launch_ref_expand(const uint64_t *bits, const uint32_t *ranks, const uint64_t *words, uint64_t *out, uint32_t n_words, hipStream_t s)
+{
+    if (!n_words) return;
+    hipLaunchKernelGGL(k_ref_expand, dim3((n_words + 255u) / 256u), dim3(256), 0, s, bits, ranks, words, out, n_words);
+}
diff --git a/instrain_amd/csrc/seg_encode.cpp b/instrain_amd/csrc/seg_encode.cpp
--- a/instrain_amd/csrc/seg_encode.cpp
+++ b/instrain_amd/csrc/seg_encode.cpp
@@ -726,6 +726,63 @@
     return SEG_OK;
 }
 
+namespace {
+constexpr int64_t REFW_PIECE = (int64_t)1 << 16;
+}
+
+int64_t ref_words_scan(HostPool &pool, uint8_t *mark, int64_t n_words, uint64_t *bits, uint32_t *ranks)
+{
+    const int64_t n64 = (n_words + 63) / 64;
+    const int n_tasks = (int)((n_words + REFW_PIECE - 1) / REFW_PIECE);
+    std::vector<int64_t> cnt((size_t)n_tasks + 1, 0);
+    pool.run(n_tasks, [&](int t) {
+        const int64_t w0 = (int64_t)t * REFW_PIECE, w1 = std::min(n_words, w0 + REFW_PIECE);
+        int64_t tot = 0;
+        for (int64_t j = w0; j < w1; j += 64) {
+            uint64_t m = 0;
+            if (j + 64 <= w1) {
+                for (int q = 0; q < 4; q++) {
+                    const __m128i v = _mm_loadu_si128(reinterpret_cast<const __m128i *>(mark + j + 16 * q));
+                    const uint32_t z = (uint32_t)_mm_movemask_epi8(_mm_cmpeq_epi8(v, _mm_setzero_si128()));
+                    m |= (uint64_t)(~z & 0xFFFFu) << (16 * q);
+                }
+            } else {
+                for (int64_t k = j; k < w1; k++) m |= (uint64_t)(mark[k] != 0) << (k - j);
+            }
+            const uint32_t c = (uint32_t)__builtin_popcountll(m);
+            bits[j >> 6] = m; ranks[j >> 6] = c;
+            tot += c;
+        }
+        memset(mark + w0, 0, (size_t)(w1 - w0));
+        cnt[(size_t)t + 1] = tot;
+    });
+    for (int t = 0; t < n_tasks; t++) cnt[(size_t)t + 1] += cnt[(size_t)t];
+    pool.run(n_tasks, [&](int t) {
+        const int64_t b0 = (int64_t)t * (REFW_PIECE / 64), b1 = std::min(n64, b0 + REFW_PIECE / 64);
+        uint32_t r = (uint32_t)cnt[(size_t)t];
+        for (int64_t i = b0; i < b1; i++) { const uint32_t c = ranks[i]; ranks[i] = r; r += c; }
+    });
+    return cnt[(size_t)n_tasks];
+}
+
+void ref_words_gather(HostPool &pool, const uint64_t *bits, const uint32_t *ranks, int64_t n_words, const uint8_t *plane2, size_t plane2_bytes, uint64_t *words)
+{
+    const int64_t n64 = (n_words + 63) / 64;
+    const int n_tasks = (int)((n_words + REFW_PIECE - 1) / REFW_PIECE);
+    pool.run(n_tasks, [&](int t) {
+        const int64_t b0 = (int64_t)t * (REFW_PIECE / 64), b1 = std::min(n64, b0 + REFW_PIECE / 64);
+        for (int64_t i = b0; i < b1; i++) {
+            uint64_t *o = words + ranks[i];
+            for (uint64_t m = bits[i]; m; m &= m - 1) {
+                const size_t at = ((size_t)i * 64 + (size_t)__builtin_ctzll(m)) * 8;
+                uint64_t w = 0;
+                if (at + 8 <= plane2_bytes) memcpy(&w, plane2 + at, 8);
+                else if (at < plane2_bytes) memcpy(&w, plane2 + at, plane2_bytes - at);
+                *o++ = w;
+            }
+        }
+    });
+}
 
 namespace {
 __attribute__((target("bmi2")))
@@ -1097,6 +1154,48 @@
     if (rc == isxenc::SEG_BAD_POS) { isx_set_error("a segment reaches beyond n_pos"); return ISX_ERR_ARG; }
     if (rc == isxenc::SEG_BAD_LEN) { isx_set_error("a segment's length is not in [1, 150]"); return ISX_ERR_ARG; }
     if (rc == isxenc::SEG_MM_RANGE) { isx_set_error("a segment has mm >= n_mm_bins"); return ISX_ERR_MM_RANGE; }
+    return ISX_OK;
+}
+
+int isx_encode_planes_ref_words(const isx_read_planes *reads, const isx_ref_planes *ref, int64_t n_pos, int32_t host_threads,
+                                uint64_t *bits, uint32_t *ranks, uint64_t *words, int64_t *n_marked)
+{
+    if (!reads || !ref || !ref->plane2 || !bits || !ranks || !words || !n_marked || reads->n_seg < 0 || n_pos <= 0 ||
+        (reads->n_seg && (!reads->gpos || !reads->len || !reads->planes))) {
+        isx_set_error("isx_encode_planes_ref_words: bad argument");
+        return ISX_ERR_ARG;
+    }
+    isxenc::HostPool pool(std::max(1, host_threads), -1, false);
+    const int64_t n_words = ((((n_pos + 3) / 4 + 15) & ~(int64_t)15)) / 8;
+    std::vector<uint8_t> mark((size_t)n_words + 64, 0);
+    isxenc::SegJob J;
+    J.in2 = *reads; J.in2.pair = nullptr; J.n_seg = reads->n_seg; J.n_pos = n_pos; J.n_mm_bins = 1;
+    J.ref2 = ref->plane2; J.refn = ref->nplane; J.ref_mark = mark.data();
+    std::vector<int64_t> exact;
+    std::vector<uint32_t> rec, gbase, cmin, cmax;
+    std::vector<uint8_t> cany;
+    int rc = isxenc::SEG_OK;
+    for (int attempt = 0; attempt < 2; attempt++) {
+        int64_t groups = 0;
+        if (exact.empty()) groups = isxenc::delta_groups_needed(pool, reads->gpos, reads->n_seg, 1);
+        else for (int64_t v : exact) groups += std::max<int64_t>(v, 1);
+        groups = std::max<int64_t>(groups, 1);
+        J.cap_rec = groups * ISX_DREC_GROUP;
+        rec.resize((size_t)J.cap_rec * ISX_DREC_WORDS + 16);
+        gbase.resize((size_t)groups); cmin.resize((size_t)groups); cmax.resize((size_t)groups); cany.resize((size_t)groups);
+        J.rec = reinterpret_cast<uint32_t *>((reinterpret_cast<uintptr_t>(rec.data()) + 63) & ~(uintptr_t)63);
+        J.gbase = gbase.data(); J.cmin = cmin.data(); J.cmax = cmax.data(); J.cany = cany.data();
+        J.slack_groups = 1; J.task_groups = exact.empty() ? nullptr : exact.data();
+        rc = isxenc::encode_planes(pool, J);
+        if (rc != isxenc::SEG_CAPACITY || attempt) break;
+        exact = J.task_need;
+    }
+    if (rc == isxenc::SEG_CAPACITY) { isx_set_error("isx_encode_planes_ref_words: the record stream does not fit"); return ISX_ERR_CAPACITY; }
+    if (rc == isxenc::SEG_BAD_POS) { isx_set_error("a segment reaches beyond n_pos"); return ISX_ERR_ARG; }
+    if (rc == isxenc::SEG_BAD_LEN) { isx_set_error("a segment's length is not in [1, 150]"); return ISX_ERR_ARG; }
+    if (rc != isxenc::SEG_OK) { isx_set_error("isx_encode_planes_ref_words: the record pass failed"); return ISX_ERR_ARG; }
+    *n_marked = isxenc::ref_words_scan(pool, mark.data(), n_words, bits, ranks);
+    isxenc::ref_words_gather(pool, bits, ranks, n_words, ref->plane2, (size_t)((n_pos + 3) / 4), words);
     return ISX_OK;
 }
 
diff --git a/instrain_amd/csrc/seg_encode.h b/instrain_amd/csrc/seg_encode.h
--- a/instrain_amd/csrc/seg_encode.h
+++ b/instrain_amd/csrc/seg_encode.h
@@ -20,6 +20,7 @@
     isx_read_planes in2{};
     std::function<void(int64_t first, int64_t count, uint32_t *gpos, uint8_t *len, uint8_t *mm, uint32_t *pair, uint64_t *planes)> produce_planes;
     const uint8_t *ref2 = nullptr, *refn = nullptr;
+    uint8_t *ref_mark = nullptr;
     int64_t n_seg = 0, n_pos = 0;
     int n_mm_bins = 1;
     bool want_pairs = false;
@@ -51,6 +52,8 @@
 int64_t delta_groups_needed(HostPool &pool, const uint32_t *gpos, int64_t n, int64_t slack_groups);
 int64_t seg_groups_needed(HostPool &pool, const uint32_t *gpos, int64_t n);
 bool pack_ref_planes(HostPool &pool, const uint8_t *ref, int64_t n_pos, uint8_t *plane2, uint8_t *nplane);
+int64_t ref_words_scan(HostPool &pool, uint8_t *mark, int64_t n_words, uint64_t *bits, uint32_t *ranks);
+void ref_words_gather(HostPool &pool, const uint64_t *bits, const uint32_t *ranks, int64_t n_words, const uint8_t *plane2, size_t plane2_bytes, uint64_t *words);
 void planes_from_words(const uint32_t *words, uint32_t len, uint64_t *planes);
 
 }
diff --git a/instrain_amd/csrc/seg_planes.inc b/instrain_amd/csrc/seg_planes.inc
--- a/instrain_amd/csrc/seg_planes.inc
+++ b/instrain_amd/csrc/seg_planes.inc
@@ -66,6 +66,7 @@
     PlaneGroup G;
     G.g = K.ga;
     const uint8_t *const ref2 = J.ref2, *const refn = J.refn;
+    uint8_t *const mark = J.ref_mark;
     const int64_t n_pos = J.n_pos;
     const int64_t safe_pos = n_pos - 200;
     const uint32_t *const gp = K.gp, *const pr = K.pr, *const ga = K.gpos_all;
@@ -196,6 +197,10 @@
         }
         const bool plain = (s0 | s1 | s2) == 0;
         const uint32_t n_exc = (uint32_t)(__builtin_popcountll(ex[0]) + __builtin_popcountll(ex[1]) + __builtin_popcountll(ex[2]));
+        if (__builtin_expect(mark != nullptr && n_exc != 0, 0)) {
+            for (int k = 0; k < 3; k++)
+                for (uint64_t e = ex[k]; e; e &= e - 1) mark[(p + (uint32_t)(64 * k) + (uint32_t)__builtin_ctzll(e)) >> 5] = 1;
+        }
         if (__builtin_expect(n_exc <= 1, 1)) {
             const uint32_t t0 = ISX_TZ64(ex[0]), t1 = ISX_TZ64(ex[1]), t2 = ISX_TZ64(ex[2] | ((uint64_t)1 << 63));
             const uint32_t m0 = 0u - (uint32_t)(ex[0] == 0), m01 = m0 & (0u - (uint32_t)(ex[1] == 0));
diff --git a/instrain_amd/engine.py b/instrain_amd/engine.py
--- a/instrain_amd/engine.py
+++ b/instrain_amd/engine.py
@@ -555,7 +555,7 @@
         sz = {n: getattr(r.sizes, n) for n, _ in Sizes._fields_}
         out = {"sizes": sz, "ticket": r.ticket, "rows_checksum": int(r.rows_checksum),
                "stats": {k: getattr(r, k) for k in ("encode_ms", "h2d_ms", "kernel_ms", "d2h_ms", "collect_wait_ms",
-                                                    "record_bytes", "encode_passes", "h2d_bytes", "d2h_bytes")}}
+                                                    "record_bytes", "encode_passes", "h2d_bytes", "d2h_bytes", "tail_ms")}}
         n_pos = int(r.n_pos)
 
         def view(addr, dtype, n):
@@ -829,6 +829,18 @@
         return rec[:n], gbase[:n // 32], None, slack_groups
 
 
+def encode_planes_ref_words(reads, ref_planes, threads=1):
+    lib = _lib.load()
+    n_words = ((((ref_planes.n_pos + 3) // 4) + 15) & ~15) // 8
+    n64 = (n_words + 63) // 64
+    bits, ranks, words = np.zeros(n64, dtype=np.uint64), np.zeros(n64, dtype=np.uint32), np.zeros(n_words, dtype=np.uint64)
+    n = C.c_int64(0)
+    cr, cf = reads.c(), ref_planes.c()
+    check(lib.isx_encode_planes_ref_words(C.byref(cr), C.byref(cf), ref_planes.n_pos, int(threads), bits.ctypes.data, ranks.ctypes.data,
+                                          words.ctypes.data, C.byref(n)))
+    return bits, ranks, words[:n.value].copy()
+
+
 def dense_cov(res, n_pos=None):
     if "cov16" in res:
         return res["cov16"]
```

Result: slower. 111.5 (-26.3%).
